# iammcy/BFLC-demo

Hardware: AMD Instinct MI355X
Metric: fl_round_wall_clock_ms (lower is better)
Workload: dtype bf16; 1 GPU; model=femnist_cnn, global_batch=4096, img=1x28x28x62cls, parallelism=fl_nodes1, clients=8, update_quota=4, aggregate_top_k=3, samples_per_client=3072, batch_size=1024, partition=dirichlet, byzantine_clients=0

## Files before the change

bflc_amd/models/__init__.py:

```python
from __future__ import annotations

from typing import Tuple

import torch

from bflc_amd.models.base import FlatModel
from bflc_amd.ops import functional as O


class LogReg(FlatModel):

    def specs(self):
        c = self.cfg
        return [("w", (c.n_features, c.n_class), "zeros"),
                ("b", (c.n_class,), "zeros")]

    def forward(self, x):
        return O.linear(x, self.p("w"), self.p("b"))


class MLP(FlatModel):

    HIDDEN = 128

    def specs(self):
        c = self.cfg
        return [("w1", (c.n_features, self.HIDDEN), "kaiming"),
                ("b1", (self.HIDDEN,), "zeros"),
                ("w2", (self.HIDDEN, c.n_class), "xavier"),
                ("b2", (c.n_class,), "zeros")]

    def forward(self, x):
        h = O.linear(x, self.p("w1"), self.p("b1"), relu=True)
        return O.linear(h, self.p("w2"), self.p("b2"))


class FemnistCNN(FlatModel):

    def specs(self):
        c = self.cfg
        return [("c1w", (32, 3, 3, 1), "kaiming"), ("c1b", (32,), "zeros"),
                ("c2w", (64, 3, 3, 32), "kaiming"), ("c2b", (64,), "zeros"),
                ("f1w", (64 * 7 * 7, 128), "kaiming"), ("f1b", (128,), "zeros"),
                ("f2w", (128, c.n_class), "xavier"), ("f2b", (c.n_class,), "zeros")]

    def forward(self, x):
        h = O.conv2d_relu_pool(x, self.p("c1w"), self.p("c1b"), 1, 1)
        h = O.conv2d_relu_pool(h, self.p("c2w"), self.p("c2b"), 1, 1)
        h = h.reshape(h.shape[0], -1)
        h = O.linear(h, self.p("f1w"), self.p("f1b"), relu=True)
        return O.linear(h, self.p("f2w"), self.p("f2b"))


def build_model(cfg, device, compute_dtype=None) -> FlatModel:
    name = cfg.model
    if getattr(cfg, "norm_groups", 0) > 0 and \
            name in ("logreg", "mlp", "femnist_cnn"):
        raise ValueError(
            f"norm_groups={cfg.norm_groups} set for model '{name}', which "
            "has no normalisation layers; it applies to resnet20/resnet50")
    if name == "logreg":
        m = LogReg(cfg, device, compute_dtype)
    elif name == "mlp":
        m = MLP(cfg, device, compute_dtype)
    elif name == "femnist_cnn":
        m = FemnistCNN(cfg, device, compute_dtype)
    elif name in ("resnet20", "resnet50"):
        from bflc_amd.models.resnet import ResNet
        m = ResNet(cfg, device, compute_dtype)
    else:
        raise ValueError(f"unknown model {name}")
    m.init_params(cfg.seed)
    return m


__all__ = ["FlatModel", "LogReg", "MLP", "FemnistCNN", "build_model"]
```

bflc_amd/ops/__init__.py:

```python
from bflc_amd.ops import functional
from bflc_amd.ops.functional import (accuracy, accuracy_t, adam_step_,
                                     axpy_, batchnorm2d, conv2d, conv2d_bn,
                                     conv2d_relu_pool,
                                     global_avgpool, add_relu,
                                     hip_available, hip_ops, linear,
                                     maxpool2d, relu, sgd_step_,
                                     sgdm_step_, grad_clip_coef_,
                                     softmax_cross_entropy, weighted_fedavg)

__all__ = [
    "functional", "linear", "conv2d", "conv2d_bn", "conv2d_relu_pool",
    "batchnorm2d", "relu",
    "add_relu", "maxpool2d", "global_avgpool", "softmax_cross_entropy",
    "accuracy", "accuracy_t", "axpy_", "sgd_step_", "adam_step_",
    "sgdm_step_", "grad_clip_coef_",
    "weighted_fedavg", "hip_ops", "hip_available",
]
```

bflc_amd/ops/functional.py:

```python
from __future__ import annotations

from typing import Optional

import torch
import torch.nn.functional as F

_hip = None
_hip_err: Optional[str] = None


def _load_hip():
    global _hip, _hip_err
    if _hip is not None or _hip_err is not None:
        return _hip
    try:
        from bflc_amd import _hip_ops
        _hip = _hip_ops
    except ImportError as e:
        _hip_err = str(e)
    return _hip


def hip_ops():
    m = _load_hip()
    if m is None:
        raise RuntimeError(
            "bflc_amd._hip_ops (gfx950 HIP kernels) is not built/importable "
            f"({_hip_err}); run `python -m bflc_amd.build`. GPU execution "
            "without the native kernels is disabled by design.")
    return m


def hip_available() -> bool:
    return _load_hip() is not None



class _LinearFn(torch.autograd.Function):

    @staticmethod
    def forward(ctx, x: torch.Tensor, w: torch.Tensor, b: torch.Tensor,
                relu: bool):
        ctx.relu = relu
        if x.is_cuda:
            y = hip_ops().linear_fwd(x, w, b, relu)
        else:
            y = torch.addmm(b, x, w)
            if relu:
                y = torch.relu(y)
        ctx.save_for_backward(x, w, y if relu else None)
        return y

    @staticmethod
    def backward(ctx, dy: torch.Tensor):
        x, w, y = ctx.saved_tensors
        dy = dy.contiguous()
        if ctx.relu:
            dy = hip_ops().relu_bwd(y, dy) if x.is_cuda \
                else dy * (y > 0).to(dy.dtype)
        want_dx = ctx.needs_input_grad[0]
        if x.is_cuda:
            dx, dw, db = hip_ops().linear_bwd(x, w, dy, want_dx)
            if not want_dx:
                dx = None
        else:
            dx = dy @ w.t() if want_dx else None
            dw = x.t() @ dy
            db = dy.sum(0)
        return dx, dw, db, None


def linear(x: torch.Tensor, w: torch.Tensor, b: torch.Tensor,
           relu: bool = False) -> torch.Tensor:
    return _LinearFn.apply(x, w, b, relu)


class _SoftmaxCEFn(torch.autograd.Function):

    @staticmethod
    def forward(ctx, logits: torch.Tensor, target: torch.Tensor):
        if logits.is_cuda:
            loss, probs = hip_ops().softmax_ce_fwd(logits, target)
        else:
            lse = torch.logsumexp(logits.float(), dim=1)
            picked = logits.float().gather(1, target.view(-1, 1)).squeeze(1)
            loss = (lse - picked).mean()
            probs = torch.softmax(logits.float(), dim=1)
        ctx.save_for_backward(probs, target)
        ctx.in_dtype = logits.dtype
        return loss

    @staticmethod
    def backward(ctx, gloss: torch.Tensor):
        probs, target = ctx.saved_tensors
        if probs.is_cuda:
            dlogits = hip_ops().softmax_ce_bwd(probs, target, gloss)
        else:
            n = probs.shape[0]
            dlogits = probs.clone()
            dlogits.scatter_add_(
                1, target.view(-1, 1),
                torch.full((n, 1), -1.0, dtype=probs.dtype))
            dlogits = dlogits * (gloss / n)
        return dlogits.to(ctx.in_dtype), None


def softmax_cross_entropy(logits: torch.Tensor,
                          target: torch.Tensor) -> torch.Tensor:
    return _SoftmaxCEFn.apply(logits, target)


class _ReluFn(torch.autograd.Function):
    @staticmethod
    def forward(ctx, x: torch.Tensor):
        if x.is_cuda:
            y = hip_ops().relu_fwd(x)
        else:
            y = torch.relu(x)
        ctx.save_for_backward(y)
        return y

    @staticmethod
    def backward(ctx, dy: torch.Tensor):
        (y,) = ctx.saved_tensors
        if y.is_cuda:
            return hip_ops().relu_bwd(y, dy.contiguous())
        return dy * (y > 0).to(dy.dtype)


def relu(x: torch.Tensor) -> torch.Tensor:
    return _ReluFn.apply(x)


class _Conv2dFn(torch.autograd.Function):

    @staticmethod
    def forward(ctx, x, w, b, stride: int, padding: int, relu: bool,
                want_col: bool):
        ctx.stride, ctx.padding = stride, padding
        ctx.has_bias = b is not None
        ctx.relu = relu
        if x.is_cuda:
            y, col = hip_ops().conv2d_fwd_col(
                x, w, b if b is not None else
                torch.zeros(w.shape[0], device=x.device, dtype=x.dtype),
                stride, padding, relu, want_col)
            ctx.save_for_backward(x, w, col, y if relu else None)
            return y
        y = F.conv2d(x.permute(0, 3, 1, 2), w.permute(0, 3, 1, 2), b,
                     stride=stride, padding=padding)
        y = y.permute(0, 2, 3, 1).contiguous()
        if relu:
            y = torch.relu(y)
        ctx.save_for_backward(x, w, None, y if relu else None)
        return y

    @staticmethod
    def backward(ctx, dy):
        x, w = ctx.saved_tensors[:2]
        dy = dy.contiguous()
        db_fused = None
        if ctx.relu:
            y = ctx.saved_tensors[3]
            if x.is_cuda and ctx.has_bias and w.shape[0] % 8 == 0:
                dy, db_fused = hip_ops().relu_bwd_colsum(y, dy)
            elif x.is_cuda:
                dy = hip_ops().relu_bwd(y, dy)
            else:
                dy = dy * (y > 0).to(dy.dtype)
        want_dx = ctx.needs_input_grad[0]
        if x.is_cuda:
            col = ctx.saved_tensors[2]
            if col.numel() == 0:
                col = None
            dx, dw, db = hip_ops().conv2d_bwd(
                x, w, dy, ctx.stride, ctx.padding, col,
                ctx.has_bias and db_fused is None, want_dx)
            if not want_dx:
                dx = None
            if db_fused is not None:
                db = db_fused
            elif not ctx.has_bias:
                db = None
        else:
            xn = x.permute(0, 3, 1, 2)
            wn = w.permute(0, 3, 1, 2)
            dyn = dy.permute(0, 3, 1, 2)
            dx = None
            if want_dx:
                dx = torch.nn.grad.conv2d_input(
                    xn.shape, wn, dyn, stride=ctx.stride,
                    padding=ctx.padding)
                dx = dx.permute(0, 2, 3, 1).contiguous()
            dw = torch.nn.grad.conv2d_weight(
                xn, wn.shape, dyn, stride=ctx.stride, padding=ctx.padding)
            dw = dw.permute(0, 2, 3, 1).contiguous()
            db = dy.sum(dim=(0, 1, 2))
        return dx, dw, (db if ctx.has_bias else None), None, None, None, \
            None


def conv2d(x, w, b=None, stride: int = 1, padding: int = 0,
           relu: bool = False) -> torch.Tensor:
    import os
    no_col = os.environ.get("BFLC_CONV_NO_COL", "1") == "1"
    want_col = (not no_col) and torch.is_grad_enabled() and \
        (x.requires_grad or w.requires_grad)
    return _Conv2dFn.apply(x, w, b, stride, padding, relu, want_col)


class _MaxPool2dFn(torch.autograd.Function):
    @staticmethod
    def forward(ctx, x, kernel: int, stride: int, want_idx: bool):
        if x.is_cuda:
            y, idx = hip_ops().maxpool2d_fwd(x, kernel, stride, want_idx)
        else:
            y, idx = F.max_pool2d(x.permute(0, 3, 1, 2), kernel, stride,
                                  return_indices=True)
            y = y.permute(0, 2, 3, 1).contiguous()
        ctx.save_for_backward(idx)
        ctx.in_shape = x.shape
        ctx.kernel, ctx.stride = kernel, stride
        return y

    @staticmethod
    def backward(ctx, dy):
        (idx,) = ctx.saved_tensors
        dy = dy.contiguous()
        if dy.is_cuda:
            dx = hip_ops().maxpool2d_bwd(dy, idx, list(ctx.in_shape),
                                         ctx.kernel, ctx.stride)
        else:
            dx = F.max_unpool2d(dy.permute(0, 3, 1, 2), idx, ctx.kernel,
                                ctx.stride,
                                output_size=ctx.in_shape[1:3])
            dx = dx.permute(0, 2, 3, 1).contiguous()
        return dx, None, None, None


def maxpool2d(x, kernel: int = 2, stride: Optional[int] = None) -> torch.Tensor:
    want_idx = torch.is_grad_enabled() and x.requires_grad
    return _MaxPool2dFn.apply(x, kernel, stride or kernel, want_idx)


class _ConvReluPoolFn(torch.autograd.Function):

    @staticmethod
    def forward(ctx, x, w, b, stride: int, padding: int,
                direct_wgrad: bool):
        ctx.stride, ctx.padding = stride, padding
        ctx.direct_wgrad = direct_wgrad
        ctx.has_bias = b is not None
        bias = b if b is not None else torch.zeros(
            w.shape[0], device=x.device, dtype=x.dtype)
        y, idx = hip_ops().conv2d_relu_pool_fwd_idx(x, w, bias, stride,
                                                    padding)
        ctx.save_for_backward(x, w, y, idx)
        return y

    @staticmethod
    def backward(ctx, dy):
        x, w, y, idx = ctx.saved_tensors
        want_dx = ctx.needs_input_grad[0]
        dx, dw, db = hip_ops().conv2d_relu_pool_bwd(
            x, w, y, idx, dy.contiguous(), ctx.stride, ctx.padding,
            ctx.has_bias, want_dx, ctx.direct_wgrad)
        return (dx if want_dx else None, dw,
                db if ctx.has_bias else None, None, None, None)


def conv2d_relu_pool(x, w, b=None, stride: int = 1,
                     padding: int = 0) -> torch.Tensor:
    import os
    if x.is_cuda and not torch.is_grad_enabled() and \
            os.environ.get("BFLC_FUSED_POOL", "1") == "1":
        bias = b if b is not None else torch.zeros(
            w.shape[0], device=x.device, dtype=x.dtype)
        return hip_ops().conv2d_relu_pool_fwd(x, w, bias, stride, padding)
    if x.is_cuda and torch.is_grad_enabled() and \
            os.environ.get("BFLC_FUSED_POOL_TRAIN", "1") != "0" and \
            hip_ops().conv2d_relu_pool_route(
                list(x.shape), list(w.shape), stride, padding) != "unfused":
        return _ConvReluPoolFn.apply(
            x, w, b, stride, padding,
            os.environ.get("BFLC_THIN_DIRECT_WGRAD", "0") == "1")
    return maxpool2d(conv2d(x, w, b, stride, padding, relu=True), 2)


class _BatchNormFn(torch.autograd.Function):

    @staticmethod
    def forward(ctx, x, gamma, beta, eps: float, relu: bool, residual):
        if x.is_cuda:
            y, mean, invstd = hip_ops().batchnorm_fwd(x, gamma, beta, eps,
                                                      relu, residual)
        else:
            xf = x.float()
            mean = xf.mean(dim=(0, 1, 2))
            var = xf.var(dim=(0, 1, 2), unbiased=False)
            invstd = (var + eps).rsqrt()
            y = (xf - mean) * invstd * gamma.float() + beta.float()
            if residual is not None:
                y = y + residual.float()
            if relu:
                y = torch.relu(y)
            y = y.to(x.dtype)
        ctx.relu = relu
        ctx.has_res = residual is not None
        if relu:
            ctx.save_for_backward(x, gamma, mean, invstd, y)
        else:
            ctx.save_for_backward(x, gamma, mean, invstd)
        return y

    @staticmethod
    def backward(ctx, dy):
        x, gamma, mean, invstd = ctx.saved_tensors[:4]
        yr = ctx.saved_tensors[4] if ctx.relu else None
        dy = dy.contiguous()
        dres = None
        if x.is_cuda:
            if ctx.has_res:
                dres = (hip_ops().add_relu_bwd(yr, dy) if yr is not None
                        else dy)
            dx, dgamma, dbeta = hip_ops().batchnorm_bwd(x, dy, mean, invstd,
                                                        gamma, yr)
        else:
            xf, dyf = x.float(), dy.float()
            if yr is not None:
                dyf = dyf * (yr.float() > 0)
            if ctx.has_res:
                dres = dyf.to(x.dtype)
            n = x.numel() / x.shape[-1]
            xhat = (xf - mean) * invstd
            sdy = dyf.sum(dim=(0, 1, 2))
            sdyx = (dyf * xhat).sum(dim=(0, 1, 2))
            dx = (gamma.float() * invstd) * (dyf - sdy / n - xhat * sdyx / n)
            dx = dx.to(x.dtype)
            dgamma = sdyx.to(x.dtype)
            dbeta = sdy.to(x.dtype)
        return dx, dgamma, dbeta, None, None, dres


class _ConvBNFn(torch.autograd.Function):

    @staticmethod
    def forward(ctx, x, w, gamma, beta, stride, padding, eps, relu,
                residual):
        h = hip_ops()
        ctx.stride, ctx.padding, ctx.relu = stride, padding, relu
        ctx.has_res = residual is not None
        yc, col, psum, psq = h.conv2d_fwd_bn(x, w, stride, padding)
        M = yc.numel() // yc.shape[-1]
        if psum.numel() > 0:
            mean, invstd = h.bn_stats_finalize(psum, psq, float(M), eps)
        else:
            mean, invstd = h.bn_stats(yc, eps)
        y = h.batchnorm_norm(yc, gamma, beta, mean, invstd, relu, residual)
        saved = [x, w, col, yc, gamma, mean, invstd]
        if relu:
            saved.append(y)
        ctx.save_for_backward(*saved)
        return y

    @staticmethod
    def backward(ctx, dy):
        h = hip_ops()
        x, w, col, yc, gamma, mean, invstd = ctx.saved_tensors[:7]
        yr = ctx.saved_tensors[7] if ctx.relu else None
        dy = dy.contiguous()
        dres = None
        if ctx.has_res:
            dres = h.add_relu_bwd(yr, dy) if yr is not None else dy
        dyc, dgamma, dbeta = h.batchnorm_bwd(yc, dy, mean, invstd, gamma,
                                             yr)
        want_dx = ctx.needs_input_grad[0]
        dx, dw, _db = h.conv2d_bwd(x, w, dyc, ctx.stride, ctx.padding,
                                   col if col.numel() > 0 else None,
                                   False, want_dx)
        if not want_dx:
            dx = None
        return (dx, dw, dgamma, dbeta, None, None, None, None, dres)


def conv2d_bn(x, w, gamma, beta, stride: int = 1, padding: int = 0,
              eps: float = 1e-5, relu: bool = True,
              residual=None) -> torch.Tensor:
    if not x.is_cuda:
        return batchnorm2d(conv2d(x, w, None, stride, padding), gamma,
                           beta, eps, relu, residual)
    return _ConvBNFn.apply(x, w, gamma, beta, stride, padding, eps, relu,
                           residual)


def batchnorm2d(x, gamma, beta, eps: float = 1e-5, relu: bool = False,
                residual=None) -> torch.Tensor:
    return _BatchNormFn.apply(x, gamma, beta, eps, relu, residual)


class _GroupNormFn(torch.autograd.Function):

    @staticmethod
    def forward(ctx, x, gamma, beta, groups: int, eps: float, relu: bool,
                residual):
        if x.is_cuda:
            y, mean, rstd = hip_ops().groupnorm_fwd(x, gamma, beta, groups,
                                                    eps, relu, residual)
        else:
            N, H, W, C = x.shape
            if groups <= 0 or C % groups:
                raise ValueError(f"groupnorm: C={C} is not divisible by "
                                 f"groups={groups}")
            xg = x.float().reshape(N, H * W, groups, C // groups)
            mean = xg.mean(dim=(1, 3))
            var = xg.var(dim=(1, 3), unbiased=False)
            rstd = (var + eps).rsqrt()
            xhat = ((xg - mean[:, None, :, None]) * rstd[:, None, :, None]) \
                .reshape(N, H, W, C)
            y = xhat * gamma.float() + beta.float()
            if residual is not None:
                y = y + residual.float()
            if relu:
                y = torch.relu(y)
            y = y.to(x.dtype)
        ctx.groups = groups
        ctx.relu = relu
        ctx.has_res = residual is not None
        if relu:
            ctx.save_for_backward(x, gamma, mean, rstd, y)
        else:
            ctx.save_for_backward(x, gamma, mean, rstd)
        return y

    @staticmethod
    def backward(ctx, dy):
        x, gamma, mean, rstd = ctx.saved_tensors[:4]
        yr = ctx.saved_tensors[4] if ctx.relu else None
        dy = dy.contiguous()
        dres = None
        G = ctx.groups
        if x.is_cuda:
            if ctx.has_res:
                dres = (hip_ops().add_relu_bwd(yr, dy) if yr is not None
                        else dy)
            dx, dgamma, dbeta = hip_ops().groupnorm_bwd(x, dy, mean, rstd,
                                                        gamma, G, yr)
        else:
            N, H, W, C = x.shape
            dyf = dy.float()
            if yr is not None:
                dyf = dyf * (yr.float() > 0)
            if ctx.has_res:
                dres = dyf.to(x.dtype)
            m = H * W * (C // G)
            xg = x.float().reshape(N, H * W, G, C // G)
            xhat = (xg - mean[:, None, :, None]) * rstd[:, None, :, None]
            d = (dyf * gamma.float()).reshape(N, H * W, G, C // G)
            sd = d.sum(dim=(1, 3), keepdim=True)
            sdx = (d * xhat).sum(dim=(1, 3), keepdim=True)
            dx = rstd[:, None, :, None] * (d - sd / m - xhat * sdx / m)
            dx = dx.reshape(N, H, W, C).to(x.dtype)
            xhat = xhat.reshape(N, H, W, C)
            dgamma = (dyf * xhat).sum(dim=(0, 1, 2)).to(x.dtype)
            dbeta = dyf.sum(dim=(0, 1, 2)).to(x.dtype)
        return dx, dgamma, dbeta, None, None, None, dres


def groupnorm2d(x, gamma, beta, groups: int, eps: float = 1e-5,
                relu: bool = False, residual=None) -> torch.Tensor:
    return _GroupNormFn.apply(x, gamma, beta, int(groups), eps, relu,
                              residual)


def conv2d_gn(x, w, gamma, beta, groups: int, stride: int = 1,
              padding: int = 0, eps: float = 1e-5, relu: bool = True,
              residual=None) -> torch.Tensor:
    return groupnorm2d(conv2d(x, w, None, stride, padding), gamma, beta,
                       groups, eps, relu, residual)


def groupnorm_route(H: int, W: int, C: int, groups: int) -> str:
    return hip_ops().groupnorm_route(H, W, C, groups)


class _GlobalAvgPoolFn(torch.autograd.Function):
    @staticmethod
    def forward(ctx, x):
        ctx.hw = (x.shape[1], x.shape[2])
        if x.is_cuda:
            return hip_ops().global_avgpool_fwd(x)
        return x.mean(dim=(1, 2))

    @staticmethod
    def backward(ctx, dy):
        h, w = ctx.hw
        dy = dy.contiguous()
        if dy.is_cuda:
            return hip_ops().global_avgpool_bwd(dy, h, w)
        return (dy / (h * w))[:, None, None, :].expand(-1, h, w, -1) \
            .contiguous()


def global_avgpool(x) -> torch.Tensor:
    return _GlobalAvgPoolFn.apply(x)


class _AddReluFn(torch.autograd.Function):

    @staticmethod
    def forward(ctx, a, b):
        if a.is_cuda:
            y = hip_ops().add_relu_fwd(a, b.contiguous())
        else:
            y = torch.relu(a + b)
        ctx.save_for_backward(y)
        return y

    @staticmethod
    def backward(ctx, dy):
        (y,) = ctx.saved_tensors
        dy = dy.contiguous()
        if y.is_cuda:
            da = hip_ops().add_relu_bwd(y, dy)
        else:
            da = dy * (y > 0).to(dy.dtype)
        return da, da


def add_relu(a, b) -> torch.Tensor:
    return _AddReluFn.apply(a, b)



def accuracy_t(logits: torch.Tensor, target: torch.Tensor) -> torch.Tensor:
    if logits.is_cuda:
        return hip_ops().accuracy_t(logits, target)
    return (logits.argmax(dim=1) == target).float().mean()


def accuracy(logits: torch.Tensor, target: torch.Tensor) -> float:
    return float(accuracy_t(logits, target))


def axpy_(y: torch.Tensor, alpha: float, x: torch.Tensor) -> torch.Tensor:
    if y.is_cuda:
        hip_ops().axpy_(y, x, float(alpha))
        return y
    return y.add_(x, alpha=alpha)


def score_load_(shadow: torch.Tensor, global_flat: torch.Tensor,
                delta: torch.Tensor, lr: float) -> None:
    if shadow.is_cuda:
        hip_ops().score_load_(shadow, global_flat, delta, float(lr))
    else:
        with torch.no_grad():
            shadow.copy_((global_flat - lr * delta).to(shadow.dtype))


def delta_extract_(out: torch.Tensor, global_flat: torch.Tensor,
                   w: torch.Tensor, lr: float) -> None:
    if out.is_cuda:
        hip_ops().delta_extract_(out, global_flat, w, float(lr))
    else:
        with torch.no_grad():
            torch.sub(global_flat, w, out=out)
            out.div_(lr)


def sgd_step_(flat_param: torch.Tensor, flat_grad: torch.Tensor,
              lr: float) -> None:
    if flat_param.is_cuda:
        hip_ops().sgd_step_(flat_param, flat_grad, float(lr))
    else:
        flat_param.add_(flat_grad, alpha=-lr)


def grad_sumsq_geom(n: int):
    return tuple(hip_ops().grad_sumsq_geom(int(n)))


def sgdm_step_geom(n: int):
    return tuple(hip_ops().sgdm_step_geom(int(n)))


def grad_clip_coef_(g: torch.Tensor, clip: float,
                    out: torch.Tensor) -> None:
    if not clip > 0:
        raise ValueError("clip must be > 0")
# ... 72 lines not shown
```

csrc/hip/bindings.cpp:

```cpp
#include <torch/extension.h>

#include <string>
#include <tuple>
#include <vector>

namespace bflc {

void axpy_(torch::Tensor y, torch::Tensor x, double alpha);
void sgd_step_(torch::Tensor p, torch::Tensor g, double lr);
void adam_step_(torch::Tensor p, torch::Tensor g, torch::Tensor m,
                torch::Tensor v, long step, double lr, double beta1,
                double beta2, double eps);
torch::Tensor weighted_fedavg(torch::Tensor deltas, torch::Tensor w);
void sgd_master_(torch::Tensor p, torch::Tensor shadow, torch::Tensor g,
                 double lr);
void adam_master_(torch::Tensor p, torch::Tensor shadow, torch::Tensor g,
                  torch::Tensor m, torch::Tensor v, long step, double lr,
                  double beta1, double beta2, double eps);
void adam_master_graph_(torch::Tensor p, torch::Tensor shadow,
                        torch::Tensor g, torch::Tensor m, torch::Tensor v,
                        torch::Tensor step, torch::Tensor bc, double lr,
                        double beta1, double beta2, double eps);
void refresh_shadow_(torch::Tensor p, torch::Tensor shadow);
void score_load_(torch::Tensor shadow, torch::Tensor global_flat,
                 torch::Tensor delta, double lr);
void delta_extract_(torch::Tensor out, torch::Tensor global_flat,
                    torch::Tensor w, double lr);
torch::Tensor relu_fwd(torch::Tensor x);
torch::Tensor relu_bwd(torch::Tensor y, torch::Tensor dy);
std::tuple<torch::Tensor, torch::Tensor> relu_bwd_colsum(
    const torch::Tensor& y, const torch::Tensor& dy);

std::tuple<long, long, long> grad_sumsq_geom_query(long n);
std::tuple<long, long, long> sgdm_step_geom_query(long n);
void grad_clip_coef_(torch::Tensor g, double clip, torch::Tensor out);
void sgdm_master_dev_(torch::Tensor p, c10::optional<torch::Tensor> shadow,
                      torch::Tensor g, torch::Tensor buf, torch::Tensor p0,
                      torch::Tensor lr_dev, torch::Tensor coef_dev,
                      double momentum, bool nesterov, double wd, double mu);

std::tuple<torch::Tensor, torch::Tensor> softmax_ce_fwd(torch::Tensor logits,
                                                        torch::Tensor target);
torch::Tensor softmax_ce_bwd(torch::Tensor probs, torch::Tensor target,
                             torch::Tensor gloss);

double accuracy(torch::Tensor logits, torch::Tensor target);
torch::Tensor accuracy_t(torch::Tensor logits, torch::Tensor target);

torch::Tensor linear_fwd(torch::Tensor x, torch::Tensor w, torch::Tensor b,
                         bool relu);
torch::Tensor gemm_raw(torch::Tensor A, torch::Tensor B, bool ta, bool tb);
using PlanRow = std::tuple<std::string, long, long, long, long>;
PlanRow gemm_plan_route(long M, long N, long K, bool ta, bool tb);
std::tuple<long, long, long, long> colsum_geom_query(long M, long N);
std::tuple<torch::Tensor, torch::Tensor, torch::Tensor> linear_bwd(
    torch::Tensor x, torch::Tensor w, torch::Tensor dy, bool want_dx);

std::tuple<torch::Tensor, torch::Tensor> conv2d_fwd_col(
    torch::Tensor x, torch::Tensor w, torch::Tensor b, long stride, long pad,
    bool relu, bool want_col);
std::tuple<torch::Tensor, torch::Tensor, torch::Tensor, torch::Tensor>
conv2d_fwd_bn(torch::Tensor x, torch::Tensor w, long stride, long pad);
std::tuple<torch::Tensor, torch::Tensor> bn_stats(torch::Tensor x,
                                                  double eps);
std::tuple<torch::Tensor, torch::Tensor> bn_stats_finalize(
    torch::Tensor psum, torch::Tensor psq, double count, double eps);
torch::Tensor batchnorm_norm(torch::Tensor x, torch::Tensor gamma,
                             torch::Tensor beta, torch::Tensor mean,
                             torch::Tensor invstd, bool relu,
                             c10::optional<torch::Tensor> residual);
torch::Tensor conv2d_fwd(torch::Tensor x, torch::Tensor w, torch::Tensor b,
                         long stride, long pad, bool relu);
std::tuple<torch::Tensor, torch::Tensor, torch::Tensor> conv2d_bwd(
    torch::Tensor x, torch::Tensor w, torch::Tensor dy, long stride,
    long pad, c10::optional<torch::Tensor> col_cache, bool want_db,
    bool want_dx);
std::tuple<torch::Tensor, torch::Tensor> maxpool2d_fwd(torch::Tensor x,
                                                       long kernel,
                                                       long stride,
                                                       bool want_idx);
torch::Tensor maxpool2d_bwd(torch::Tensor dy, torch::Tensor idx,
                            std::vector<long> in_shape, long kernel,
                            long stride);
torch::Tensor conv2d_relu_pool_fwd(torch::Tensor x, torch::Tensor w,
                                   torch::Tensor b, long stride, long pad,
                                   long max_blocks, std::string impl);
std::string conv_fwd_pool_impl(std::vector<long> x_shape,
                               std::vector<long> w_shape, long stride,
                               long pad);
long halo_conv_group_images_query(std::vector<long> x_shape,
                                  std::vector<long> w_shape, long stride,
                                  long pad);
std::string conv2d_relu_pool_route(std::vector<long> x_shape,
                                   std::vector<long> w_shape, long stride,
                                   long pad);
PlanRow conv_plan_route(const std::string& entry, std::vector<long> x_shape,
                        std::vector<long> w_shape, long stride, long pad);
std::tuple<torch::Tensor, torch::Tensor> conv2d_relu_pool_fwd_idx(
    torch::Tensor x, torch::Tensor w, torch::Tensor b, long stride,
    long pad, long max_blocks, std::string impl);
std::tuple<torch::Tensor, torch::Tensor> pool_relu_bwd_colsum(
    torch::Tensor y_pooled, torch::Tensor idx, torch::Tensor dy_pooled,
    std::vector<long> out_shape);
std::tuple<torch::Tensor, torch::Tensor> thin_conv_pool_wgrad(
    torch::Tensor x, torch::Tensor y_pooled, torch::Tensor idx,
    torch::Tensor dy_pooled, long stride, long pad);
std::tuple<torch::Tensor, torch::Tensor> thin_conv_pool_wgrad_fused(
    torch::Tensor x, torch::Tensor y_pooled, torch::Tensor idx,
    torch::Tensor dy_pooled, long stride, long pad);
std::string thin_pool_wgrad_impl(std::vector<long> x_shape,
                                 std::vector<long> w_shape, long stride,
                                 long pad, bool want_dx);
std::string conv2d_relu_pool_bwd_route(std::vector<long> x_shape,
                                       std::vector<long> w_shape,
                                       long stride, long pad, bool want_dx,
                                       bool allow_direct);
std::tuple<torch::Tensor, torch::Tensor, torch::Tensor> conv2d_relu_pool_bwd(
    torch::Tensor x, torch::Tensor w, torch::Tensor y_pooled,
    torch::Tensor idx, torch::Tensor dy_pooled, long stride, long pad,
    bool want_db, bool want_dx, bool allow_direct, std::string dgrad_impl,
    long max_blocks);
std::string pool_dgrad_impl(std::vector<long> x_shape,
                            std::vector<long> w_shape, long stride, long pad,
                            bool want_dx);
long halo_dgrad_group_images_query(std::vector<long> x_shape,
                                   std::vector<long> w_shape, long stride,
                                   long pad);
std::tuple<torch::Tensor, torch::Tensor> halo_pool_dgrad(
    torch::Tensor w, torch::Tensor y_pooled, torch::Tensor idx,
    torch::Tensor dy_pooled, long max_blocks, bool store_plane);

std::tuple<torch::Tensor, torch::Tensor, torch::Tensor> batchnorm_fwd(
    torch::Tensor x, torch::Tensor gamma, torch::Tensor beta, double eps,
    bool relu, c10::optional<torch::Tensor> residual);
std::tuple<torch::Tensor, torch::Tensor, torch::Tensor> batchnorm_bwd(
    torch::Tensor x, torch::Tensor dy, torch::Tensor mean,
    torch::Tensor invstd, torch::Tensor gamma,
    c10::optional<torch::Tensor> y_relu);
torch::Tensor global_avgpool_fwd(torch::Tensor x);
torch::Tensor global_avgpool_bwd(torch::Tensor dy, long H, long W);
torch::Tensor add_relu_fwd(torch::Tensor a, torch::Tensor b);
torch::Tensor add_relu_bwd(torch::Tensor y, torch::Tensor dy);

std::tuple<torch::Tensor, torch::Tensor, torch::Tensor> groupnorm_fwd(
    torch::Tensor x, torch::Tensor gamma, torch::Tensor beta, long groups,
    double eps, bool relu, c10::optional<torch::Tensor> residual);
std::tuple<torch::Tensor, torch::Tensor, torch::Tensor> groupnorm_bwd(
    torch::Tensor x, torch::Tensor dy, torch::Tensor mean, torch::Tensor rstd,
    torch::Tensor gamma, long groups, c10::optional<torch::Tensor> y_relu);
std::string groupnorm_route(long H, long W, long C, long groups);

}

PYBIND11_MODULE(TORCH_EXTENSION_NAME, m) {
  m.doc() = "bflc_amd hand-written gfx950 (CDNA4) HIP kernels";
  m.def("axpy_", &bflc::axpy_, "y += alpha*x (fp32, in place)");
  m.def("sgd_step_", &bflc::sgd_step_, "fused flat SGD");
  m.def("adam_step_", &bflc::adam_step_, "fused flat Adam");
  m.def("weighted_fedavg", &bflc::weighted_fedavg,
        "fixed-order weighted FedAvg reduce");
  m.def("sgd_master_", &bflc::sgd_master_,
        "fused fp32-master SGD + bf16 shadow refresh");
  m.def("adam_master_", &bflc::adam_master_);
  m.def("adam_master_graph_", &bflc::adam_master_graph_,
        "hipGraph-capturable Adam: device step counter + on-device bias "
        "corrections (tick kernel), fp32 master + bf16 shadow");
  m.def("refresh_shadow_", &bflc::refresh_shadow_, "shadow = bf16(master)");
  m.def("score_load_", &bflc::score_load_,
        "shadow = compute_dtype(global - lr*delta): one-pass scoring "
        "candidate load (replaces copy+axpy+set_flat)");
  m.def("delta_extract_", &bflc::delta_extract_,
        "out = (global - w)/lr: one-pass pseudo-gradient extraction");
  m.def("grad_sumsq_geom", &bflc::grad_sumsq_geom_query,
        "sum-of-squares geometry of an n-element gradient: (blocks, "
        "longest lane chain in elements, adds after the lane chain)",
        py::arg("n"));
  m.def("sgdm_step_geom", &bflc::sgdm_step_geom_query,
        "launch of sgdm_master_dev_ at n elements: (blocks, threads, "
        "elements per thread per grid-stride pass)",
        py::arg("n"));
  m.def("grad_clip_coef_", &bflc::grad_clip_coef_,
        "out[0] = min(1, clip / (||g||_2 + 1e-6)), 0 if the norm is not "
        "finite; out[1] = sum(g^2) when out has two elements",
        py::arg("g"), py::arg("clip"), py::arg("out"));
  m.def("sgdm_master_dev_", &bflc::sgdm_master_dev_,
        "fused SGD (momentum / nesterov / weight decay / FedProx / clip "
        "coefficient) on the fp32 master (+ bf16 shadow); lr and coef are "
        "device floats",
        py::arg("p"), py::arg("shadow"), py::arg("g"), py::arg("buf"),
        py::arg("p0"), py::arg("lr_dev"), py::arg("coef_dev"),
        py::arg("momentum"), py::arg("nesterov"), py::arg("wd"),
        py::arg("mu"));
  m.def("relu_fwd", &bflc::relu_fwd);
  m.def("relu_bwd", &bflc::relu_bwd);
  m.def("relu_bwd_colsum", &bflc::relu_bwd_colsum,
        "fused relu backward + bias-grad column sum: (dx, db)");
  m.def("softmax_ce_fwd", &bflc::softmax_ce_fwd,
        "fused softmax cross-entropy fwd (loss, probs)");
  m.def("softmax_ce_bwd", &bflc::softmax_ce_bwd);
  m.def("accuracy", &bflc::accuracy, "fused argmax-compare-reduce");
  m.def("accuracy_t", &bflc::accuracy_t,
        "accuracy as a device tensor (no host sync)");
  m.def("linear_fwd", &bflc::linear_fwd, "MFMA bf16 GEMM + bias (+relu)",
        py::arg("x"), py::arg("w"), py::arg("b"), py::arg("relu") = false);
  m.def("gemm_raw", &bflc::gemm_raw, "raw GEMM (bench/ablation)");
  m.def("gemm_plan_route", &bflc::gemm_plan_route,
        "plan gemm_raw takes: (thin | gemm8p | gemm256 | small, bm, bn, S, "
        "kslice)",
        py::arg("M"), py::arg("N"), py::arg("K"), py::arg("ta"),
        py::arg("tb"));
  m.def("conv_plan_route", &bflc::conv_plan_route,
        "plan of the implicit-GEMM conv entry fwd | fwd_pool | dgrad | "
        "wgrad: (none | gemm256 | small, bm, bn, S, kslice)",
        py::arg("entry"), py::arg("x_shape"), py::arg("w_shape"),
        py::arg("stride"), py::arg("pad"));
  m.def("colsum_geom", &bflc::colsum_geom_query,
        "colsum pass-1 geometry of an [M, N] matrix: (G, cblocks, rows, "
        "chunks)",
        py::arg("M"), py::arg("N"));
  m.def("linear_bwd", &bflc::linear_bwd,
        "(dx, dw, db) - dx empty unless want_dx", py::arg("x"),
        py::arg("w"), py::arg("dy"), py::arg("want_dx") = true);
  m.def("conv2d_fwd", &bflc::conv2d_fwd,
        "NHWC implicit-GEMM convolution (MFMA); inference entry, no col",
        py::arg("x"), py::arg("w"), py::arg("b"), py::arg("stride"),
        py::arg("pad"), py::arg("relu") = false);
  m.def("conv2d_fwd_col", &bflc::conv2d_fwd_col, "(y, col) - col for bwd",
        py::arg("x"), py::arg("w"), py::arg("b"), py::arg("stride"),
        py::arg("pad"), py::arg("relu") = false,
        py::arg("want_col") = true);
  m.def("conv2d_fwd_bn", &bflc::conv2d_fwd_bn,
        "(y, col, psum, psq) - conv with fused epilogue BN stats");
  m.def("bn_stats", &bflc::bn_stats, "(mean, invstd) of x [.., C]");
  m.def("bn_stats_finalize", &bflc::bn_stats_finalize,
        "(mean, invstd) from [chunks][C] partials");
  m.def("batchnorm_norm", &bflc::batchnorm_norm,
        py::arg("x"), py::arg("gamma"), py::arg("beta"), py::arg("mean"),
        py::arg("invstd"), py::arg("relu"),
        py::arg("residual") = py::none(),
        "normalization pass with known stats");
  m.def("conv2d_bwd", &bflc::conv2d_bwd,
        "(dx, dw, db) - db empty unless want_db, dx empty unless "
        "want_dx (first-layer convs need no input gradient)",
        py::arg("x"), py::arg("w"), py::arg("dy"), py::arg("stride"),
        py::arg("pad"), py::arg("col_cache") = py::none(),
        py::arg("want_db") = true, py::arg("want_dx") = true);
  m.def("maxpool2d_fwd", &bflc::maxpool2d_fwd, py::arg("x"),
        py::arg("kernel"), py::arg("stride"),
        py::arg("want_idx") = true);
  m.def("maxpool2d_bwd", &bflc::maxpool2d_bwd);
  m.def("conv2d_relu_pool_fwd", &bflc::conv2d_relu_pool_fwd,
        "grad-free conv + bias + ReLU + 2x2/2 maxpool, pooled in the conv "
        "epilogue where a fused route applies: [N, OH/2, OW/2, Kout]. "
        "max_blocks > 0 caps the halo kernel's grid; impl pins gemm256 | "
        "halo_mfma ('' = conv_fwd_pool_impl's answer)",
        py::arg("x"), py::arg("w"), py::arg("b"), py::arg("stride"),
        py::arg("pad"), py::arg("max_blocks") = 0, py::arg("impl") = "");
  m.def("conv_fwd_pool_impl", &bflc::conv_fwd_pool_impl,
        "what the gemm256_pool route launches: halo_mfma | gemm256",
        py::arg("x_shape"), py::arg("w_shape"), py::arg("stride"),
        py::arg("pad"));
  m.def("halo_conv_group_images", &bflc::halo_conv_group_images_query,
        "images per LDS group of the halo kernel (0: not its geometry)",
        py::arg("x_shape"), py::arg("w_shape"), py::arg("stride"),
        py::arg("pad"));
  m.def("conv2d_relu_pool_route", &bflc::conv2d_relu_pool_route,
        "route conv2d_relu_pool_fwd takes: gemm256_pool | thin_pool | "
        "unfused",
        py::arg("x_shape"), py::arg("w_shape"), py::arg("stride"),
        py::arg("pad"));
  m.def("conv2d_relu_pool_fwd_idx", &bflc::conv2d_relu_pool_fwd_idx,
        "training conv + bias + ReLU + 2x2/2 maxpool: (y_pooled, idx), "
        "same routes and options as conv2d_relu_pool_fwd",
        py::arg("x"), py::arg("w"), py::arg("b"), py::arg("stride"),
        py::arg("pad"), py::arg("max_blocks") = 0, py::arg("impl") = "");
  m.def("pool_relu_bwd_colsum", &bflc::pool_relu_bwd_colsum,
        "unpool + ReLU mask + bias grad in one pass: (dy_full_masked, db)",
        py::arg("y_pooled"), py::arg("idx"), py::arg("dy_pooled"),
        py::arg("out_shape"));
  m.def("thin_conv_pool_wgrad", &bflc::thin_conv_pool_wgrad,
        "direct first-layer (dw, db) from the pooled tensors",
        py::arg("x"), py::arg("y_pooled"), py::arg("idx"),
        py::arg("dy_pooled"), py::arg("stride"), py::arg("pad"));
  m.def("thin_conv_pool_wgrad_fused", &bflc::thin_conv_pool_wgrad_fused,
        "first-layer (dw, db) from the pooled tensors, bitwise the "
        "materialised unpool -> im2col -> split-K GEMM chain",
        py::arg("x"), py::arg("y_pooled"), py::arg("idx"),
        py::arg("dy_pooled"), py::arg("stride"), py::arg("pad"));
  m.def("thin_pool_wgrad_impl", &bflc::thin_pool_wgrad_impl,
        "what the unpool route runs for the thin first layer: "
        "fused_mfma | materialized",
        py::arg("x_shape"), py::arg("w_shape"), py::arg("stride"),
        py::arg("pad"), py::arg("want_dx"));
  m.def("conv2d_relu_pool_bwd_route", &bflc::conv2d_relu_pool_bwd_route,
        "route conv2d_relu_pool_bwd takes: thin_direct | unpool",
        py::arg("x_shape"), py::arg("w_shape"), py::arg("stride"),
        py::arg("pad"), py::arg("want_dx"), py::arg("allow_direct") = true);
  m.def("conv2d_relu_pool_bwd", &bflc::conv2d_relu_pool_bwd,
        "(dx, dw, db) of the fused conv + ReLU + pool from its saved "
        "(x, w, y_pooled, idx). dgrad_impl pins halo_mfma | implicit_gemm "
        "('' = pool_dgrad_impl's answer); max_blocks > 0 caps the halo "
        "kernel's grid",
        py::arg("x"), py::arg("w"), py::arg("y_pooled"), py::arg("idx"),
        py::arg("dy_pooled"), py::arg("stride"), py::arg("pad"),
        py::arg("want_db") = true, py::arg("want_dx") = true,
        py::arg("allow_direct") = true, py::arg("dgrad_impl") = "",
        py::arg("max_blocks") = 0);
  m.def("pool_dgrad_impl", &bflc::pool_dgrad_impl,
        "data gradient the unpool route runs: halo_mfma | implicit_gemm",
        py::arg("x_shape"), py::arg("w_shape"), py::arg("stride"),
        py::arg("pad"), py::arg("want_dx"));
  m.def("halo_dgrad_group_images", &bflc::halo_dgrad_group_images_query,
        "images per LDS group of the halo dgrad kernel (0: not its "
        "geometry)",
        py::arg("x_shape"), py::arg("w_shape"), py::arg("stride"),
        py::arg("pad"));
  m.def("halo_pool_dgrad", &bflc::halo_pool_dgrad,
        "the halo dgrad kernel on its geometry alone: (dx, masked "
        "full-resolution dy plane) from w and the pooled (y, idx, dy); "
        "store_plane = false skips the plane store (0-size plane)",
        py::arg("w"), py::arg("y_pooled"), py::arg("idx"),
        py::arg("dy_pooled"), py::arg("max_blocks") = 0,
        py::arg("store_plane") = true);
  m.def("batchnorm_fwd", &bflc::batchnorm_fwd,
        py::arg("x"), py::arg("gamma"), py::arg("beta"), py::arg("eps"),
        py::arg("relu"), py::arg("residual") = py::none(),
        "(y, mean, invstd) — batch-stats BN, optional fused relu");
  m.def("batchnorm_bwd", &bflc::batchnorm_bwd, "(dx, dgamma, dbeta)",
        py::arg("x"), py::arg("dy"), py::arg("mean"), py::arg("invstd"),
        py::arg("gamma"), py::arg("y_relu") = py::none());
  m.def("global_avgpool_fwd", &bflc::global_avgpool_fwd);
  m.def("global_avgpool_bwd", &bflc::global_avgpool_bwd);
  m.def("add_relu_fwd", &bflc::add_relu_fwd, "fused residual add + relu");
  m.def("add_relu_bwd", &bflc::add_relu_bwd);
  m.def("groupnorm_fwd", &bflc::groupnorm_fwd,
        py::arg("x"), py::arg("gamma"), py::arg("beta"), py::arg("groups"),
        py::arg("eps"), py::arg("relu"), py::arg("residual") = py::none(),
        "(y, mean [N,G], rstd [N,G]) — per-sample GroupNorm, optional "
        "fused residual add + relu");
  m.def("groupnorm_bwd", &bflc::groupnorm_bwd, "(dx, dgamma, dbeta)",
        py::arg("x"), py::arg("dy"), py::arg("mean"), py::arg("rstd"),
        py::arg("gamma"), py::arg("groups"), py::arg("y_relu") = py::none());
  m.def("groupnorm_route", &bflc::groupnorm_route,
        "route groupnorm_fwd/bwd take: slab | split (from H, W, C, groups "
        "only — never N)",
        py::arg("H"), py::arg("W"), py::arg("C"), py::arg("groups"));
}
```

csrc/hip/conv2d.hip:

```cpp

#include "common.h"
#include "gemm_api.h"

namespace bflc {

namespace {

typedef __attribute__((ext_vector_type(8))) __bf16 bf16x8_t;
typedef __attribute__((ext_vector_type(8))) unsigned short u16x8_t;
typedef __attribute__((ext_vector_type(8))) int i32x8_t;
typedef __attribute__((ext_vector_type(4))) float f32x4_t;

__global__ void im2col_nhwc_vec_kernel(const bf16* __restrict__ x,
                                       bf16* __restrict__ col, ConvShape sh,
                                       long total_g) {
  const int c8g = sh.C / 8;
  const int rs = sh.R * sh.S;
  long g = (long)blockIdx.x * blockDim.x + threadIdx.x;
  const long stride = (long)gridDim.x * blockDim.x;
  for (; g < total_g; g += stride) {
    const int c8 = (int)(g % c8g) * 8;
    const int k = (int)((g / c8g) % rs);
    const long m = g / ((long)c8g * rs);
    const int s = k % sh.S, r = k / sh.S;
// ... 654 lines not shown
    for (int t = 0; t < Q; ++t) {
      if (wq == t && my0 < nsteps) {
        if (my0 > 0) acc = accs[frag][lane];
#pragma unroll
        for (int i = 0; i < CH; ++i)
          if (my0 + i < nsteps)
            acc = __builtin_amdgcn_mfma_f32_16x16x32_bf16(
                __builtin_bit_cast(bf16x8_t, av[i]),
                __builtin_bit_cast(bf16x8_t, bv[i]), acc, 0, 0, 0);
        accs[frag][lane] = acc;
      }
      __syncthreads();
    }
  }
  if (wq != 0) return;
  acc = accs[frag][lane];

  if (l15 < 9) {
#pragma unroll
    for (int r = 0; r < 4; ++r) {
      const int row = frag * 16 + l4 * 4 + r;
      if (row >= Kout) continue;
      if (part)
        part[((long)blockIdx.x * Kout + row) * 9 + l15] = acc[r];
      else
        dw[row * 9 + l15] = f2b(acc[r] + 0.f);
    }
  }
}

inline int ew_grid(long n) {
  return (int)std::min<long>((n + 255) / 256, 16384);
}

ConvShape make_shape(const torch::Tensor& x, const torch::Tensor& w,
                     long stride, long pad) {
  ConvShape sh;
  sh.N = (int)x.size(0); sh.H = (int)x.size(1);
  sh.W = (int)x.size(2); sh.C = (int)x.size(3);
  sh.Kout = (int)w.size(0); sh.R = (int)w.size(1); sh.S = (int)w.size(2);
  sh.stride = (int)stride; sh.pad = (int)pad;
  sh.OH = (sh.H + 2 * sh.pad - sh.R) / sh.stride + 1;
  sh.OW = (sh.W + 2 * sh.pad - sh.S) / sh.stride + 1;
  TORCH_CHECK(w.size(3) == sh.C, "conv channel mismatch (NHWC x, KRSC w)");
  return sh;
}

torch::Tensor im2col(const torch::Tensor& x, const ConvShape& sh) {
  if (sh.C % 8 == 0) {
    auto col = torch::empty({sh.M(), sh.RSC()}, x.options());
    const long total_g = sh.M() * sh.R * sh.S * (sh.C / 8);
    hipLaunchKernelGGL(im2col_nhwc_vec_kernel, dim3(ew_grid(total_g)),
                       dim3(256), 0, cur_stream(),
                       (const bf16*)x.data_ptr(), (bf16*)col.data_ptr(), sh,
                       total_g);
    HIP_CHECK(hipGetLastError());
    return col;
  }
  const long rscp = (sh.RSC() + 7) / 8 * 8;
  auto col = torch::empty({sh.M(), rscp}, x.options());
  if (rscp <= 32) {
    const long total_m = sh.M();
    hipLaunchKernelGGL(im2col_nhwc_rowvec_kernel, dim3(ew_grid(total_m)),
                       dim3(256), 0, cur_stream(),
                       (const bf16*)x.data_ptr(), (bf16*)col.data_ptr(), sh,
                       rscp, total_m);
  } else {
    const long total_g = sh.M() * (rscp / 8);
    hipLaunchKernelGGL(im2col_nhwc_gran_kernel, dim3(ew_grid(total_g)),
                       dim3(256), 0, cur_stream(),
                       (const bf16*)x.data_ptr(), (bf16*)col.data_ptr(), sh,
                       rscp, total_g);
  }
  HIP_CHECK(hipGetLastError());
  return col;
}

torch::Tensor pad_w2(const torch::Tensor& w2, long kp) {
  if (kp == w2.size(1)) return w2;
  auto out = torch::zeros({w2.size(0), kp}, w2.options());
  out.slice(1, 0, w2.size(1)).copy_(w2);
  return out;
}

bool is_1x1_s1(const ConvShape& sh) {
  return sh.R == 1 && sh.S == 1 && sh.stride == 1 && sh.pad == 0;
}

int env_gate(const char* name, int dflt) {
  const char* e = getenv(name);
  return e ? atoi(e) : dflt;
}
int wgrad_implicit_max_kout() {
  static int v = env_gate("BFLC_WGRAD_IMPLICIT_MAX_KOUT", 64);
  return v;
}
int dgrad_implicit_max_c() {
  static int v = env_gate("BFLC_DGRAD_IMPLICIT_MAX_C", 128);
  return v;
}

}

std::tuple<torch::Tensor, torch::Tensor> conv2d_fwd_col(
    torch::Tensor x, torch::Tensor w, torch::Tensor b, long stride,
    long pad, bool relu, bool want_col) {
  CHECK_GPU(x); CHECK_CONTIG(x); CHECK_CONTIG(w);
  TORCH_CHECK(x.scalar_type() == at::kBFloat16, "conv: bf16 only");
  auto sh = make_shape(x, w, stride, pad);
  auto w2 = w.view({(long)sh.Kout, sh.RSC()});
  auto bc = b.contiguous();
  auto y = torch::empty({(long)sh.N, (long)sh.OH, (long)sh.OW,
                         (long)sh.Kout}, x.options());
  if (is_1x1_s1(sh)) {
    auto col = x.view({sh.M(), (long)sh.C});
    gemm_bf16_raw(col, w2, y, sh.M(), sh.Kout, sh.RSC(), false, true, &bc,
                  relu, EpStore::kPlain, 0);
    return {y, col};
  }
  if (gemm_conv_fwd_raw(x, w2, y, sh, &bc, relu))
    return {y, torch::empty({0}, x.options())};
  const long kp = (sh.RSC() + 7) / 8 * 8;
  if (!want_col && sh.RSC() <= 16 && kp <= 32) {
    auto w2p = pad_w2(w2, kp);
    if (gemm_thin_conv_raw(x, w2p, y, sh, &bc, relu))
      return {y, torch::empty({0}, x.options())};
  }
  auto col = im2col(x, sh);
  TORCH_CHECK(col.size(1) == kp);
  gemm_bf16_raw(col, pad_w2(w2, kp), y, sh.M(), sh.Kout, kp, false, true,
                &bc, relu, EpStore::kPlain, 0);
  return {y, col};
}

torch::Tensor conv2d_fwd(torch::Tensor x, torch::Tensor w, torch::Tensor b,
                         long stride, long pad, bool relu) {
  return std::get<0>(conv2d_fwd_col(x, w, b, stride, pad, relu, false));
}

std::tuple<torch::Tensor, torch::Tensor, torch::Tensor, torch::Tensor>
conv2d_fwd_bn(torch::Tensor x, torch::Tensor w, long stride, long pad) {
  CHECK_GPU(x); CHECK_CONTIG(x); CHECK_CONTIG(w);
  auto sh = make_shape(x, w, stride, pad);
  auto w2 = w.view({(long)sh.Kout, sh.RSC()});
  auto y = torch::empty({(long)sh.N, (long)sh.OH, (long)sh.OW,
                         (long)sh.Kout}, x.options());
  std::pair<torch::Tensor, torch::Tensor> stats;
  auto none = torch::empty({0}, x.options());
  if (is_1x1_s1(sh)) {
    auto col = x.view({sh.M(), (long)sh.C});
    gemm_bf16_raw(col, w2, y, sh.M(), sh.Kout, sh.RSC(), false, true,
                  nullptr, false, EpStore::kPlain, 0, &stats);
    return {y, col, stats.first.defined() ? stats.first : none,
            stats.second.defined() ? stats.second : none};
  }
  if (gemm_conv_fwd_raw(x, w2, y, sh, nullptr, false, &stats))
    return {y, none, stats.first.defined() ? stats.first : none,
            stats.second.defined() ? stats.second : none};
  auto col = im2col(x, sh);
  const long kp = col.size(1);
  gemm_bf16_raw(col, pad_w2(w2, kp), y, sh.M(), sh.Kout, kp, false, true,
                nullptr, false, EpStore::kPlain, 0, &stats);
  return {y, col, stats.first.defined() ? stats.first : none,
          stats.second.defined() ? stats.second : none};
}

namespace {

torch::Tensor conv_dgrad(const torch::Tensor& x, const torch::Tensor& w,
                         const torch::Tensor& dy2, const ConvShape& sh,
                         bool want_dx) {
  auto w2 = w.view({(long)sh.Kout, sh.RSC()});
  torch::Tensor dx;
  bool dgrad_done = !want_dx;
  if (!want_dx) {
    dx = torch::empty({0}, x.options());
  } else if (is_1x1_s1(sh)) {
    auto wT = transpose_bf16(w2);
    dx = torch::empty_like(x);
    auto dxv = dx.view({sh.M(), (long)sh.C});
    gemm_bf16_raw(dy2, wT, dxv, sh.M(), sh.RSC(), sh.Kout, false, true,
                  nullptr, false, EpStore::kPlain, 0);
    dgrad_done = true;
  } else if (sh.Kout % 8 == 0 && sh.C <= dgrad_implicit_max_c() &&
             sh.C >= 8 && sh.stride == 1) {
    auto wrot2 = w.permute({3, 1, 2, 0}).contiguous()
                     .view({(long)sh.C, (long)sh.R * sh.S * sh.Kout});
    dx = torch::empty_like(x);
    auto dxv = dx.view({(long)sh.N * sh.H * sh.W, (long)sh.C});
    dgrad_done = gemm_conv_dgrad_raw(dy2, wrot2, dxv, sh);
  }
  if (!dgrad_done) {
    auto wT = transpose_bf16(w2);
    auto dcol = torch::empty({sh.M(), sh.RSC()}, x.options());
    gemm_bf16_raw(dy2, wT, dcol, sh.M(), sh.RSC(), sh.Kout, false, true,
                  nullptr, false, EpStore::kPlain, 0);
    dx = torch::empty_like(x);
    if (sh.C % 8 == 0) {
      const long total_g = (long)sh.N * sh.H * sh.W * (sh.C / 8);
      hipLaunchKernelGGL(col2im_nhwc_vec_kernel, dim3(ew_grid(total_g)),
                         dim3(256), 0, cur_stream(),
                         (const bf16*)dcol.data_ptr(),
                         (bf16*)dx.data_ptr(), sh, total_g);
    } else {
      const long total = dx.numel();
      hipLaunchKernelGGL(col2im_nhwc_kernel, dim3(ew_grid(total)), dim3(256),
                         0, cur_stream(), (const bf16*)dcol.data_ptr(),
                         (bf16*)dx.data_ptr(), sh, total);
    }
    HIP_CHECK(hipGetLastError());
  }
  return dx;
}

torch::Tensor conv_wgrad(const torch::Tensor& x, const torch::Tensor& w,
                         const torch::Tensor& dy2, const ConvShape& sh,
                         const c10::optional<torch::Tensor>& col_cache) {
  auto w2 = w.view({(long)sh.Kout, sh.RSC()});
  auto dw = torch::empty_like(w2);
  bool wgrad_done = false;
  if (!is_1x1_s1(sh) && sh.Kout <= wgrad_implicit_max_kout() &&
      !(col_cache.has_value() && col_cache->numel() > 0))
    wgrad_done = gemm_conv_wgrad_raw(dy2, x, dw, sh);
  if (!wgrad_done) {
    auto col = (col_cache.has_value() && col_cache->numel() > 0)
                   ? *col_cache
                   : (is_1x1_s1(sh) ? x.view({sh.M(), (long)sh.C})
                                    : im2col(x, sh));
    const long kp = col.size(1);
    if (kp == sh.RSC()) {
      gemm_bf16_raw(dy2, col, dw, sh.Kout, sh.RSC(), sh.M(), true, false,
                    nullptr, false, EpStore::kPlain, 0);
    } else {
      auto dwp = torch::empty({(long)sh.Kout, kp}, dw.options());
      gemm_bf16_raw(dy2, col, dwp, sh.Kout, kp, sh.M(), true, false,
                    nullptr, false, EpStore::kPlain, 0);
      dw.copy_(dwp.slice(1, 0, sh.RSC()));
    }
  }
  return dw.view(w.sizes());
}

}

std::tuple<torch::Tensor, torch::Tensor, torch::Tensor> conv2d_bwd(
    torch::Tensor x, torch::Tensor w, torch::Tensor dy, long stride,
    long pad, c10::optional<torch::Tensor> col_cache, bool want_db,
    bool want_dx) {
  CHECK_GPU(x); CHECK_CONTIG(x); CHECK_CONTIG(w); CHECK_CONTIG(dy);
  auto sh = make_shape(x, w, stride, pad);
  auto dy2 = dy.view({sh.M(), (long)sh.Kout});
  auto dx = conv_dgrad(x, w, dy2, sh, want_dx);
  auto dw = conv_wgrad(x, w, dy2, sh, col_cache);

  auto db = want_db ? colsum_bf16(dy2)
                    : torch::empty({0}, dy.options());
  return {dx, dw, db};
}

std::tuple<torch::Tensor, torch::Tensor> maxpool2d_fwd(torch::Tensor x,
                                                       long kernel,
                                                       long stride,
                                                       bool want_idx) {
  CHECK_GPU(x); CHECK_CONTIG(x);
  ConvShape sh;
  sh.N = (int)x.size(0); sh.H = (int)x.size(1);
  sh.W = (int)x.size(2); sh.C = (int)x.size(3);
  sh.R = sh.S = (int)kernel; sh.stride = (int)stride; sh.pad = 0;
  sh.Kout = sh.C;
  sh.OH = (sh.H - sh.R) / sh.stride + 1;
  sh.OW = (sh.W - sh.S) / sh.stride + 1;
  auto y = torch::empty({(long)sh.N, (long)sh.OH, (long)sh.OW, (long)sh.C},
                        x.options());
  TORCH_CHECK(sh.R * sh.S <= 255, "maxpool window too large for u8 idx");
  const bool skip_idx = !want_idx && sh.C % 8 == 0;
  auto idx = skip_idx
                 ? torch::empty({0}, y.options().dtype(at::kByte))
                 : torch::empty_like(y, y.options().dtype(at::kByte));
  if (sh.C % 8 == 0) {
    const long total_g = sh.M() * (sh.C / 8);
    hipLaunchKernelGGL(maxpool_nhwc_vec_fwd, dim3(ew_grid(total_g)),
                       dim3(256), 0, cur_stream(),
                       (const bf16*)x.data_ptr(), (bf16*)y.data_ptr(),
                       skip_idx ? nullptr : idx.data_ptr<uint8_t>(), sh,
                       total_g);
  } else {
    const long total = y.numel();
    hipLaunchKernelGGL(maxpool_nhwc_fwd, dim3(ew_grid(total)), dim3(256), 0,
                       cur_stream(), (const bf16*)x.data_ptr(),
                       (bf16*)y.data_ptr(), idx.data_ptr<uint8_t>(), sh,
                       total);
  }
  HIP_CHECK(hipGetLastError());
  return {y, idx};
}

namespace {

enum class PoolRoute { kUnfused, kGemm256, kThin };

PoolRoute pool_route(const ConvShape& sh) {
  if (is_1x1_s1(sh)) return PoolRoute::kUnfused;
  if (gemm_conv_fwd_pool_eligible(sh)) return PoolRoute::kGemm256;
  const long kp = (sh.RSC() + 7) / 8 * 8;
  if (sh.RSC() <= 16 && gemm_thin_conv_pool_eligible(sh, kp))
    return PoolRoute::kThin;
  return PoolRoute::kUnfused;
}

ConvShape make_shape_dims(std::vector<long> xs, std::vector<long> ws,
                          long stride, long pad) {
  TORCH_CHECK(xs.size() == 4 && ws.size() == 4, "NHWC x, KRSC w");
  ConvShape sh;
  sh.N = (int)xs[0]; sh.H = (int)xs[1]; sh.W = (int)xs[2]; sh.C = (int)xs[3];
  sh.Kout = (int)ws[0]; sh.R = (int)ws[1]; sh.S = (int)ws[2];
  sh.stride = (int)stride; sh.pad = (int)pad;
  sh.OH = (sh.H + 2 * sh.pad - sh.R) / sh.stride + 1;
  sh.OW = (sh.W + 2 * sh.pad - sh.S) / sh.stride + 1;
  return sh;
}

}

PlanRow conv_plan_route(const std::string& entry, std::vector<long> x_shape,
                        std::vector<long> w_shape, long stride, long pad) {
  const ConvEntry e = entry == "fwd"        ? ConvEntry::kFwd
                      : entry == "fwd_pool" ? ConvEntry::kFwdPool
                      : entry == "dgrad"    ? ConvEntry::kDgrad
                                            : ConvEntry::kWgrad;
  TORCH_CHECK(e != ConvEntry::kWgrad || entry == "wgrad",
              "conv_plan_route: entry is fwd | fwd_pool | dgrad | wgrad");
  return plan_row(
      gemm_conv_plan(e, make_shape_dims(x_shape, w_shape, stride, pad)));
}

std::string conv2d_relu_pool_route(std::vector<long> x_shape,
                                   std::vector<long> w_shape, long stride,
                                   long pad) {
  switch (pool_route(make_shape_dims(x_shape, w_shape, stride, pad))) {
    case PoolRoute::kGemm256: return "gemm256_pool";
    case PoolRoute::kThin: return "thin_pool";
    default: return "unfused";
  }
}

namespace {

std::tuple<torch::Tensor, torch::Tensor> relu_pool_fwd_impl(
    const torch::Tensor& x, const torch::Tensor& w, const torch::Tensor& b,
    long stride, long pad, bool want_idx, long max_blocks = 0,
    const std::string& impl = "") {
  CHECK_GPU(x); CHECK_CONTIG(x); CHECK_CONTIG(w);
  TORCH_CHECK(x.scalar_type() == at::kBFloat16, "conv: bf16 only");
  auto sh = make_shape(x, w, stride, pad);
  TORCH_CHECK(impl.empty() || impl == "gemm256" || impl == "halo_mfma",
              "conv2d_relu_pool: impl is '' | gemm256 | halo_mfma");
  const HaloMode halo = impl.empty()        ? HaloMode::kAuto
                        : impl == "gemm256" ? HaloMode::kOff
                                            : HaloMode::kForce;
  TORCH_CHECK(halo != HaloMode::kForce || halo_conv_geometry_ok(sh),
              "conv2d_relu_pool: shape outside the halo kernel's geometry");
  const PoolRoute route =
      halo == HaloMode::kForce ? PoolRoute::kGemm256 : pool_route(sh);
  if (route != PoolRoute::kUnfused) {
    auto w2 = w.view({(long)sh.Kout, sh.RSC()});
    auto bc = b.contiguous();
    auto y = torch::empty({(long)sh.N, (long)sh.OH / 2, (long)sh.OW / 2,
                           (long)sh.Kout}, x.options());
    auto idx = want_idx
                   ? torch::empty_like(y, y.options().dtype(at::kByte))
                   : torch::empty({0}, y.options().dtype(at::kByte));
    uint8_t* ip = want_idx ? idx.data_ptr<uint8_t>() : nullptr;
    const bool done =
        route == PoolRoute::kGemm256
            ? gemm_conv_fwd_pool_raw(x, w2, y, sh, &bc, true, ip, halo,
                                     (int)max_blocks)
            : gemm_thin_conv_pool_raw(
                  x, pad_w2(w2, (sh.RSC() + 7) / 8 * 8), y, sh, &bc, true,
                  ip);
    TORCH_CHECK(done, "conv2d_relu_pool: route query and launcher disagree");
    return {y, idx};
  }
  auto y = conv2d_fwd(x, w, b, stride, pad, true);
  return maxpool2d_fwd(y, 2, 2, want_idx);
}

bool thin_wgrad_eligible(const ConvShape& sh) {
  return sh.R == 3 && sh.S == 3 && sh.C == 1 && sh.stride == 1 &&
         sh.OH > 0 && sh.OW > 0 && sh.OH % 2 == 0 && sh.OW % 2 == 0 &&
         sh.Kout <= 64 && sh.Kout % 8 == 0;
}

void check_pooled(const torch::Tensor& y, const torch::Tensor& idx,
                  const torch::Tensor& dy) {
  CHECK_GPU(y); CHECK_GPU(idx); CHECK_GPU(dy);
  CHECK_CONTIG(y); CHECK_CONTIG(idx); CHECK_CONTIG(dy);
  TORCH_CHECK(y.scalar_type() == at::kBFloat16 &&
              dy.scalar_type() == at::kBFloat16 &&
              idx.scalar_type() == at::kByte,
              "pooled backward: bf16 y/dy and u8 idx");
  TORCH_CHECK(y.dim() == 4 && y.sizes() == dy.sizes() &&
              y.sizes() == idx.sizes(),
              "pooled backward: y, idx, dy must share one NHWC shape");
}

bool thin_fused_wgrad_gate() {
  static const bool v = env_gate("BFLC_THIN_FUSED_WGRAD", 1) != 0;
  return v;
}

struct ThinFusedPlan {
  bool ok = false;
  long S = 1, kslice = 0;
  int tbl_pairs = 0;
  long lds = 0;
  int cshift = 0;
};

ThinFusedPlan thin_fused_plan(const ConvShape& sh) {
  ThinFusedPlan t;
  if (!thin_wgrad_eligible(sh) || sh.N <= 0) return t;
  const long Mpix = sh.M();
  const long kp = (sh.RSC() + 7) / 8 * 8;
  const GemmPlan p = gemm_dense_plan(sh.Kout, kp, Mpix, true, false);
  const long lim = 1L << 31;
  if (p.path != GemmPath::kSmall || kp != 16 || Mpix * sh.Kout >= lim ||
      (long)sh.N * sh.H * sh.W >= lim || (long)sh.N * (sh.OH + 2) >= lim)
    return t;
  t.S = p.S;
  t.kslice = p.kslice;
  int rows_max = 0;
  for (long s = 0; s < p.S; ++s) {
    int P0, rows;
    thin_wgrad_window(sh, s * p.kslice,
                      std::min(Mpix, (s + 1) * p.kslice), &P0, &rows);
    rows_max = std::max(rows_max, rows);
  }
  const long xelems = (long)(rows_max + 2) * (sh.OW + 2) + 4;
  const long pairs = (p.kslice / 32 + 1) * 16;
  t.tbl_pairs = (int)pairs;
  t.lds = pairs * 8 + (xelems + 1) / 2 * 4;
  while (t.cshift < 6 && (1 << t.cshift) < sh.OW + 2) ++t.cshift;
  t.ok = t.lds <= kThinFusedMaxLds && xelems <= 32768;
  return t;
}

torch::Tensor pool_relu_bwd_db(const torch::Tensor& y_pooled,
                               const torch::Tensor& idx,
                               const torch::Tensor& dy_pooled,
                               const ConvShape& sh) {
  const long Mpix = sh.M();
  const long N = sh.Kout;
  TORCH_CHECK(Mpix * N < (1L << 31), "pool_relu_bwd_db: 32-bit indices");
  auto db = torch::empty({N}, dy_pooled.options());
  const ColsumGeom g = colsum_geom(Mpix, N);
  auto cpart = torch::empty({g.chunks, N},
                            dy_pooled.options().dtype(at::kFloat));
  hipLaunchKernelGGL(pool_relu_bwd_colsum_part_kernel<false>,
                     dim3(g.cblocks, g.chunks), dim3(256), 0, cur_stream(),
                     (const bf16*)y_pooled.data_ptr(),
                     idx.data_ptr<uint8_t>(),
                     (const bf16*)dy_pooled.data_ptr(), (bf16*)nullptr, Mpix,
                     N, sh.OH, sh.OW, g.G, g.rows, cpart.data_ptr<float>());
  HIP_CHECK(hipGetLastError());
  colsum_finalize(cpart, db);
  return db;
}

}

torch::Tensor conv2d_relu_pool_fwd(torch::Tensor x, torch::Tensor w,
                                   torch::Tensor b, long stride, long pad,
                                   long max_blocks, std::string impl) {
  return std::get<0>(
      relu_pool_fwd_impl(x, w, b, stride, pad, false, max_blocks, impl));
}

std::string conv_fwd_pool_impl(std::vector<long> x_shape,
                               std::vector<long> w_shape, long stride,
                               long pad) {
  const auto sh = make_shape_dims(x_shape, w_shape, stride, pad);
  return pool_route(sh) == PoolRoute::kGemm256 && halo_conv_gate(sh)
             ? "halo_mfma"
             : "gemm256";
}

long halo_conv_group_images_query(std::vector<long> x_shape,
                                  std::vector<long> w_shape, long stride,
                                  long pad) {
  return halo_conv_group_images(
      make_shape_dims(x_shape, w_shape, stride, pad));
}

std::tuple<torch::Tensor, torch::Tensor> conv2d_relu_pool_fwd_idx(
    torch::Tensor x, torch::Tensor w, torch::Tensor b, long stride,
    long pad, long max_blocks, std::string impl) {
  return relu_pool_fwd_impl(x, w, b, stride, pad, true, max_blocks, impl);
}

std::tuple<torch::Tensor, torch::Tensor> pool_relu_bwd_colsum(
    torch::Tensor y_pooled, torch::Tensor idx, torch::Tensor dy_pooled,
    std::vector<long> out_shape) {
  check_pooled(y_pooled, idx, dy_pooled);
  const long n = y_pooled.size(0), PH = y_pooled.size(1),
             PW = y_pooled.size(2), N = y_pooled.size(3);
  TORCH_CHECK(N % 8 == 0, "pool_relu_bwd_colsum: C % 8 required");
  TORCH_CHECK(out_shape.size() == 4 && out_shape[0] == n &&
              out_shape[1] == 2 * PH && out_shape[2] == 2 * PW &&
              out_shape[3] == N,
              "pool_relu_bwd_colsum: out_shape must be [N, 2*PH, 2*PW, C]");
  const long M = n * PH * PW * 4;
  auto dx = torch::empty({n, 2 * PH, 2 * PW, N}, dy_pooled.options());
  auto db = torch::empty({N}, dy_pooled.options());
  const ColsumGeom g = colsum_geom(M, N);
  auto part = torch::empty({g.chunks, N},
                           dy_pooled.options().dtype(at::kFloat));
  if (M > 0) {
    hipLaunchKernelGGL(pool_relu_bwd_colsum_part_kernel<true>,
                       dim3(g.cblocks, g.chunks), dim3(256), 0, cur_stream(),
                       (const bf16*)y_pooled.data_ptr(),
                       idx.data_ptr<uint8_t>(),
                       (const bf16*)dy_pooled.data_ptr(),
                       (bf16*)dx.data_ptr(), M, N, (int)(2 * PH),
                       (int)(2 * PW), g.G, g.rows, part.data_ptr<float>());
    HIP_CHECK(hipGetLastError());
  }
  colsum_finalize(part, db);
  return {dx, db};
}

std::tuple<torch::Tensor, torch::Tensor> thin_conv_pool_wgrad(
    torch::Tensor x, torch::Tensor y_pooled, torch::Tensor idx,
    torch::Tensor dy_pooled, long stride, long pad) {
  CHECK_GPU(x); CHECK_CONTIG(x);
  TORCH_CHECK(x.scalar_type() == at::kBFloat16 && x.dim() == 4,
              "thin_conv_pool_wgrad: bf16 NHWC x");
  check_pooled(y_pooled, idx, dy_pooled);
  const auto sh = make_shape_dims(
      x.sizes().vec(), {y_pooled.size(3), 3, 3, x.size(3)}, stride, pad);
  TORCH_CHECK(thin_wgrad_eligible(sh),
              "thin_conv_pool_wgrad: 3x3, C == 1, stride 1, even OH/OW, "
              "Kout % 8 == 0 and Kout <= 64 only");
  TORCH_CHECK(y_pooled.size(0) == sh.N && y_pooled.size(1) == sh.OH / 2 &&
              y_pooled.size(2) == sh.OW / 2,
              "thin_conv_pool_wgrad: pooled shape does not match x");
  const long MP = sh.M() / 4;
  const int N = sh.Kout;
  const int G = N / 8, PL = 256 / G;
  const long rows = std::max<long>(PL, (MP + 511) / 512);
  const int chunks = (int)std::max<long>(1, (MP + rows - 1) / rows);
  auto part = torch::empty({(long)chunks, (long)N, (long)kWgradAcc},
                           x.options().dtype(at::kFloat));
  auto dw = torch::empty({(long)N, 3, 3, 1}, x.options());
  auto db = torch::empty({(long)N}, x.options());
  hipLaunchKernelGGL(thin_conv_pool_wgrad_part_kernel, dim3(chunks),
                     dim3(256), 0, cur_stream(), (const bf16*)x.data_ptr(),
                     (const bf16*)y_pooled.data_ptr(),
                     idx.data_ptr<uint8_t>(),
                     (const bf16*)dy_pooled.data_ptr(), sh, MP, G, rows,
                     part.data_ptr<float>());
  HIP_CHECK(hipGetLastError());
  hipLaunchKernelGGL(thin_conv_pool_wgrad_final_kernel,
                     dim3(ceil_div((long)N * kWgradAcc, 4)), dim3(256), 0,
                     cur_stream(), part.data_ptr<float>(), chunks, N,
                     (bf16*)dw.data_ptr(), (bf16*)db.data_ptr());
  HIP_CHECK(hipGetLastError());
  return {dw, db};
}

std::tuple<torch::Tensor, torch::Tensor> thin_conv_pool_wgrad_fused(
    torch::Tensor x, torch::Tensor y_pooled, torch::Tensor idx,
    torch::Tensor dy_pooled, long stride, long pad) {
  CHECK_GPU(x); CHECK_CONTIG(x);
  TORCH_CHECK(x.scalar_type() == at::kBFloat16 && x.dim() == 4,
              "thin_conv_pool_wgrad_fused: bf16 NHWC x");
  check_pooled(y_pooled, idx, dy_pooled);
  const auto sh = make_shape_dims(
      x.sizes().vec(), {y_pooled.size(3), 3, 3, x.size(3)}, stride, pad);
  const ThinFusedPlan t = thin_fused_plan(sh);
  TORCH_CHECK(t.ok,
              "thin_conv_pool_wgrad_fused: 3x3, C == 1, stride 1, even "
              "OH/OW, Kout % 8 == 0 and Kout <= 64, on the small-tile "
              "split-K plan, only");
  TORCH_CHECK(y_pooled.size(0) == sh.N && y_pooled.size(1) == sh.OH / 2 &&
              y_pooled.size(2) == sh.OW / 2,
              "thin_conv_pool_wgrad_fused: pooled shape does not match x");
  const long Mpix = sh.M();
  const int N = sh.Kout;
  auto dw = torch::empty({(long)N, 3, 3, 1}, x.options());
  torch::Tensor db;

  torch::Tensor part;
  if (t.S > 1)
    part = torch::empty({t.S, (long)N, 9}, x.options().dtype(at::kFloat));
  const int frags = (N + 15) / 16;
  auto* kern = frags <= 2 ? thin_pool_wgrad_mfma_kernel<4>
                          : thin_pool_wgrad_mfma_kernel<2>;
  hipLaunchKernelGGL(kern, dim3((unsigned)t.S),
                     dim3(frags * (frags <= 2 ? 4 : 2) * 64), (size_t)t.lds,
                     cur_stream(), (const unsigned short*)x.data_ptr(),
                     (const unsigned short*)y_pooled.data_ptr(),
                     idx.data_ptr<uint8_t>(),
                     (const unsigned short*)dy_pooled.data_ptr(), sh, Mpix,
                     t.kslice, t.cshift, t.tbl_pairs,
                     t.S > 1 ? part.data_ptr<float>() : nullptr,
                     (bf16*)dw.data_ptr());
  HIP_CHECK(hipGetLastError());
  if (t.S > 1) {
    auto dw2 = dw.view({(long)N, 9});
    splitk_reduce_plain(part, dw2);
  }

  db = pool_relu_bwd_db(y_pooled, idx, dy_pooled, sh);
  return {dw, db};
}

std::string thin_pool_wgrad_impl(std::vector<long> x_shape,
                                 std::vector<long> w_shape, long stride,
                                 long pad, bool want_dx) {
  const auto sh = make_shape_dims(x_shape, w_shape, stride, pad);
  return !want_dx && thin_fused_wgrad_gate() && thin_fused_plan(sh).ok
             ? "fused_mfma"
             : "materialized";
}

std::string conv2d_relu_pool_bwd_route(std::vector<long> x_shape,
                                       std::vector<long> w_shape,
                                       long stride, long pad, bool want_dx,
                                       bool allow_direct) {
  const auto sh = make_shape_dims(x_shape, w_shape, stride, pad);
  return allow_direct && !want_dx && thin_wgrad_eligible(sh) ? "thin_direct"
                                                             : "unpool";
}

namespace {

std::tuple<torch::Tensor, torch::Tensor> halo_pool_dgrad_impl(
    const torch::Tensor& x_like, const torch::Tensor& w,
    const torch::Tensor& y_pooled, const torch::Tensor& idx,
    const torch::Tensor& dy_pooled, const ConvShape& sh, long max_blocks,
    bool store_plane = true) {
  auto dyf = store_plane
                 ? torch::empty({(long)sh.N, (long)sh.OH, (long)sh.OW,
                                 (long)sh.Kout}, dy_pooled.options())
                 : torch::empty({0}, dy_pooled.options());
  auto dx = torch::empty({(long)sh.N, (long)sh.H, (long)sh.W, (long)sh.C},
                         x_like.options());
  halo_pool_dgrad_launch(w, y_pooled, idx, dy_pooled,
                         store_plane ? &dyf : nullptr, dx, sh,
                         (int)max_blocks);
  return {dx, dyf};
}

}

std::string pool_dgrad_impl(std::vector<long> x_shape,
                            std::vector<long> w_shape, long stride, long pad,
                            bool want_dx) {
  const auto sh = make_shape_dims(x_shape, w_shape, stride, pad);
  return want_dx && halo_dgrad_gate(sh) ? "halo_mfma" : "implicit_gemm";
}

long halo_dgrad_group_images_query(std::vector<long> x_shape,
                                   std::vector<long> w_shape, long stride,
                                   long pad) {
  return halo_dgrad_group_images(
      make_shape_dims(x_shape, w_shape, stride, pad));
}

std::tuple<torch::Tensor, torch::Tensor> halo_pool_dgrad(
    torch::Tensor w, torch::Tensor y_pooled, torch::Tensor idx,
    torch::Tensor dy_pooled, long max_blocks, bool store_plane) {
  CHECK_GPU(w); CHECK_CONTIG(w);
  TORCH_CHECK(w.scalar_type() == at::kBFloat16 && w.dim() == 4,
              "halo_pool_dgrad: bf16 KRSC w");
  check_pooled(y_pooled, idx, dy_pooled);
  const auto sh = make_shape_dims(
      {y_pooled.size(0), 2 * y_pooled.size(1), 2 * y_pooled.size(2),
       w.size(3)},
      w.sizes().vec(), 1, 1);
  TORCH_CHECK(y_pooled.size(3) == sh.Kout && halo_dgrad_geometry_ok(sh),
              "halo_pool_dgrad: shape outside the halo kernel's geometry");
  return halo_pool_dgrad_impl(dy_pooled, w, y_pooled, idx, dy_pooled, sh,
                              max_blocks, store_plane);
}

std::tuple<torch::Tensor, torch::Tensor, torch::Tensor> conv2d_relu_pool_bwd(
    torch::Tensor x, torch::Tensor w, torch::Tensor y_pooled,
    torch::Tensor idx, torch::Tensor dy_pooled, long stride, long pad,
    bool want_db, bool want_dx, bool allow_direct, std::string dgrad_impl,
    long max_blocks) {
  CHECK_GPU(x); CHECK_CONTIG(x); CHECK_CONTIG(w);
  const auto sh = make_shape(x, w, stride, pad);
  TORCH_CHECK(sh.OH % 2 == 0 && sh.OW % 2 == 0 &&
              y_pooled.dim() == 4 && y_pooled.size(0) == sh.N &&
              y_pooled.size(1) == sh.OH / 2 &&
              y_pooled.size(2) == sh.OW / 2 && y_pooled.size(3) == sh.Kout,
              "conv2d_relu_pool_bwd: pooled shape does not match the conv");
  TORCH_CHECK(dgrad_impl.empty() || dgrad_impl == "halo_mfma" ||
                  dgrad_impl == "implicit_gemm",
              "conv2d_relu_pool_bwd: dgrad_impl is '' | halo_mfma | "
              "implicit_gemm");
  const bool force_halo = dgrad_impl == "halo_mfma";
  TORCH_CHECK(!force_halo || (want_dx && halo_dgrad_geometry_ok(sh) &&
                              sh.M() * sh.Kout < (1L << 31)),
              "conv2d_relu_pool_bwd: shape outside the halo dgrad kernel's "
              "geometry");
  auto none = torch::empty({0}, x.options());
  if (allow_direct && !want_dx && thin_wgrad_eligible(sh)) {
    auto [dw, db] = thin_conv_pool_wgrad(x, y_pooled, idx, dy_pooled,
                                         stride, pad);
    return {none, dw.view(w.sizes()), want_db ? db : none};
  }
  if (!want_dx && thin_fused_wgrad_gate() && thin_fused_plan(sh).ok) {
    auto [dw, db] = thin_conv_pool_wgrad_fused(x, y_pooled, idx, dy_pooled,
                                               stride, pad);
    return {none, dw.view(w.sizes()), want_db ? db : none};
  }
  if (force_halo ||
      (dgrad_impl.empty() && want_dx && halo_dgrad_gate(sh))) {
    check_pooled(y_pooled, idx, dy_pooled);
    auto db = want_db ? pool_relu_bwd_db(y_pooled, idx, dy_pooled, sh) : none;
    auto [dx, dyf] = halo_pool_dgrad_impl(x, w, y_pooled, idx, dy_pooled, sh,
                                          max_blocks);
    auto dy2 = dyf.view({sh.M(), (long)sh.Kout});
    auto dw = conv_wgrad(x, w, dy2, sh, c10::nullopt);
    return {dx, dw, db};
  }
  auto [dyf, db] = pool_relu_bwd_colsum(
      y_pooled, idx, dy_pooled,
      {(long)sh.N, (long)sh.OH, (long)sh.OW, (long)sh.Kout});
  auto [dx, dw, db_unused] =
      conv2d_bwd(x, w, dyf, stride, pad, c10::nullopt, false, want_dx);
  (void)db_unused;
  return {dx, dw, want_db ? db : none};
}

torch::Tensor maxpool2d_bwd(torch::Tensor dy, torch::Tensor idx,
                            std::vector<long> in_shape, long kernel,
                            long stride) {
  CHECK_GPU(dy); CHECK_CONTIG(dy); CHECK_CONTIG(idx);
  TORCH_CHECK(idx.numel() == dy.numel(),
              "maxpool2d_bwd: argmax mask missing/size-mismatched (the "
              "forward ran with want_idx=false?)");
  ConvShape sh;
  sh.N = (int)in_shape[0]; sh.H = (int)in_shape[1];
  sh.W = (int)in_shape[2]; sh.C = (int)in_shape[3];
  sh.R = sh.S = (int)kernel; sh.stride = (int)stride; sh.pad = 0;
  sh.Kout = sh.C;
  sh.OH = (int)dy.size(1); sh.OW = (int)dy.size(2);
  auto dx = torch::empty({(long)sh.N, (long)sh.H, (long)sh.W, (long)sh.C},
                         dy.options());
  if (sh.C % 8 == 0) {
    const long total_g = (long)sh.N * sh.H * sh.W * (sh.C / 8);
    hipLaunchKernelGGL(maxpool_nhwc_vec_bwd, dim3(ew_grid(total_g)),
                       dim3(256), 0, cur_stream(),
                       (const bf16*)dy.data_ptr(), idx.data_ptr<uint8_t>(),
                       (bf16*)dx.data_ptr(), sh, total_g);
  } else {
    const long total = dx.numel();
    hipLaunchKernelGGL(maxpool_nhwc_bwd, dim3(ew_grid(total)), dim3(256), 0,
                       cur_stream(), (const bf16*)dy.data_ptr(),
                       idx.data_ptr<uint8_t>(), (bf16*)dx.data_ptr(), sh,
                       total);
  }
  HIP_CHECK(hipGetLastError());
  return dx;
}

}
```

csrc/hip/gemm_api.h:

```cpp
#pragma once

#include <torch/extension.h>

#include <string>
#include <tuple>

#include "gemm_plan.h"

namespace bflc {

#if defined(__HIPCC__) || defined(__HIP__)
#define BFLC_HD __host__ __device__
#else
#define BFLC_HD
#endif

struct ConvShape {
  int N, C, H, W, Kout, R, S, stride, pad, OH, OW;
  BFLC_HD long M() const { return (long)N * OH * OW; }
  BFLC_HD long RSC() const { return (long)R * S * C; }
};

enum class EpStore : int {
  kPlain = 0,
  kConvNCHW = 1,
};

void gemm_bf16_raw(const torch::Tensor& A, const torch::Tensor& B,
                   torch::Tensor& C, long M, long N, long K, bool ta, bool tb,
                   const torch::Tensor* bias, bool relu, EpStore store,
                   long ohw,
                   std::pair<torch::Tensor, torch::Tensor>* bn_stats
                   = nullptr);

using PlanRow = std::tuple<std::string, long, long, long, long>;
inline PlanRow plan_row(const GemmPlan& p) {
  return {gemm_path_name(p.path), p.bm, p.bn, p.S, p.kslice};
}
PlanRow gemm_plan_route(long M, long N, long K, bool ta, bool tb);
GemmPlan gemm_dense_plan(long M, long N, long K, bool ta, bool tb);
void splitk_reduce_plain(const torch::Tensor& part, torch::Tensor& out);

enum class ConvEntry { kFwd, kFwdPool, kDgrad, kWgrad };
GemmPlan gemm_conv_plan(ConvEntry e, const ConvShape& sh);

bool gemm_thin_conv_raw(const torch::Tensor& x, const torch::Tensor& w2p,
                        torch::Tensor& y, const ConvShape& sh,
                        const torch::Tensor* bias, bool relu);

bool gemm_conv_fwd_raw(const torch::Tensor& x, const torch::Tensor& w2,
                       torch::Tensor& y, const ConvShape& sh,
                       const torch::Tensor* bias, bool relu,
                       std::pair<torch::Tensor, torch::Tensor>* bn_stats
                       = nullptr);

bool gemm_conv_fwd_pool_eligible(const ConvShape& sh);
enum class HaloMode { kAuto, kOff, kForce };
bool gemm_conv_fwd_pool_raw(const torch::Tensor& x, const torch::Tensor& w2,
                            torch::Tensor& y, const ConvShape& sh,
                            const torch::Tensor* bias, bool relu,
                            uint8_t* idx = nullptr,
                            HaloMode halo = HaloMode::kAuto,
                            int max_blocks = 0);

bool halo_conv_geometry_ok(const ConvShape& sh);
int halo_conv_group_images(const ConvShape& sh);
bool halo_conv_gate(const ConvShape& sh);
void halo_conv_fwd_pool_launch(const torch::Tensor& x,
                               const torch::Tensor& w2, torch::Tensor& y,
                               const ConvShape& sh, const torch::Tensor* bias,
                               bool relu, uint8_t* idx, int max_blocks);
bool halo_dgrad_geometry_ok(const ConvShape& sh);
int halo_dgrad_group_images(const ConvShape& sh);
bool halo_dgrad_gate(const ConvShape& sh);
void halo_pool_dgrad_launch(const torch::Tensor& w,
                            const torch::Tensor& y_pooled,
                            const torch::Tensor& idx,
                            const torch::Tensor& dy_pooled,
                            torch::Tensor* dyf, torch::Tensor& dx,
                            const ConvShape& sh, int max_blocks);
bool gemm_thin_conv_pool_eligible(const ConvShape& sh, long KT);
bool gemm_thin_conv_pool_raw(const torch::Tensor& x,
                             const torch::Tensor& w2p, torch::Tensor& y,
                             const ConvShape& sh, const torch::Tensor* bias,
                             bool relu, uint8_t* idx = nullptr);

bool gemm_conv_dgrad_raw(const torch::Tensor& dy, const torch::Tensor& wrot2,
                         torch::Tensor& dx, const ConvShape& sh);

bool gemm_conv_wgrad_raw(const torch::Tensor& dy2, const torch::Tensor& x,
                         torch::Tensor& dw, const ConvShape& sh);

torch::Tensor colsum_bf16(const torch::Tensor& X);
void colsum_finalize(const torch::Tensor& part, torch::Tensor& out);
std::tuple<torch::Tensor, torch::Tensor> relu_bwd_colsum(
    const torch::Tensor& y, const torch::Tensor& dy);

torch::Tensor transpose_bf16(const torch::Tensor& X);

}
```

csrc/hip/gemm_bf16.hip:

```cpp

#include "common.h"
#include "gemm_api.h"

namespace bflc {

namespace {

typedef __attribute__((ext_vector_type(8))) __bf16 bf16x8_t;
typedef __attribute__((ext_vector_type(8))) unsigned short u16x8_t;
typedef __attribute__((ext_vector_type(2))) unsigned short u16x2_t;
typedef __attribute__((ext_vector_type(4))) float f32x4_t;

constexpr int BK = 32;
constexpr int BKP = BK + 8;

template <int BM, int BN, int WR, int WC, bool TA, bool TB,
          int CMODE = 0>
__launch_bounds__(WR * WC * 64)
__global__ void gemm_kernel(const bf16* __restrict__ A,
                            const bf16* __restrict__ B,
                            bf16* __restrict__ C, float* __restrict__ Cpart,
                            const bf16* __restrict__ bias, long M, long N,
                            long K, long kslice, int relu, int store_mode,
                            long ohw, int vecA, int vecB, ConvShape csh,
                            float* __restrict__ bn_psum = nullptr,
                            float* __restrict__ bn_psq = nullptr) {
  constexpr int THREADS = WR * WC * 64;
  constexpr int FM = BM / WR / 16;
  constexpr int FN = BN / WC / 16;

  __shared__ bf16 As[BM][BKP];
  __shared__ bf16 Bs[BN][BKP];
  auto swz = [](int row, int k) { return k ^ (row & 24); };

  const int ntn = (int)((N + BN - 1) / BN);
  const int ntm = (int)((M + BM - 1) / BM);
  const int nwg = ntm * ntn;
  int bid = blockIdx.x;
  {
    const int nxcd = 8;
    const int q = nwg / nxcd, r = nwg % nxcd;
    const int xcd = bid % nxcd, idx = bid / nxcd;
    bid = (xcd < r ? xcd * (q + 1) : r * (q + 1) + (xcd - r) * q) + idx;
  }
  const long tile_m = (long)(bid / ntn) * BM;
  const long tile_n = (long)(bid % ntn) * BN;

  const long k_begin = (long)blockIdx.y * kslice;
  const long k_end = min(K, k_begin + kslice);

  const int tid = threadIdx.x;
  const int wave = tid / 64, lane = tid % 64;
  const int wm0 = (wave / WC) * (BM / WR);
  const int wn0 = (wave % WC) * (BN / WC);
  const int l15 = lane & 15, l4 = lane >> 4;

  f32x4_t acc[FM][FN] = {};

  constexpr int AGI =
      (CMODE == 1 || CMODE == 2)
          ? ((BM * BK / 8) + THREADS - 1) / THREADS : 1;
  long cv_nbase[AGI];
  int cv_i0[AGI], cv_j0[AGI];
  bool cv_mok[AGI];
  int st_c8[AGI], st_rr[AGI], st_ss[AGI];
  if (CMODE == 1 || CMODE == 2) {
    constexpr int GROUPS = (BM * BK) / 8;
#pragma unroll
    for (int i = 0; i < AGI; ++i) {
      const int g = tid + i * THREADS;
      const int m = g / (BK / 8);
      const int k8 = (g % (BK / 8)) * 8;
      const long gm = tile_m + m;
      cv_mok[i] = g < GROUPS && gm < M;
      const long gmc = cv_mok[i] ? gm : 0;
      if (CMODE == 1) {
        const int ow = (int)(gmc % csh.OW);
        const int oh = (int)((gmc / csh.OW) % csh.OH);
        const int nn = (int)(gmc / ((long)csh.OW * csh.OH));
        cv_i0[i] = oh * csh.stride - csh.pad;
        cv_j0[i] = ow * csh.stride - csh.pad;
        cv_nbase[i] = (long)nn * csh.H;
      } else {
        const int iw = (int)(gmc % csh.W);
        const int ih = (int)((gmc / csh.W) % csh.H);
        const int nn = (int)(gmc / ((long)csh.W * csh.H));
        cv_i0[i] = ih + csh.pad;
        cv_j0[i] = iw + csh.pad;
        cv_nbase[i] = (long)nn * csh.OH;
      }
      const int inner = CMODE == 1 ? csh.C : csh.Kout;
      const long gk0 = k_begin + k8;
      const int rs = (int)(gk0 / inner);
      st_c8[i] = (int)(gk0 - (long)rs * inner);
      st_rr[i] = rs / csh.S;
      st_ss[i] = rs - st_rr[i] * csh.S;
    }
  }

  constexpr int BGI =
      CMODE == 3 ? ((BN * BK / 8) + THREADS - 1) / THREADS
      : (CMODE == 4 ? ((BN * BK / 16) + THREADS - 1) / THREADS : 1);
  int cv3_rr[BGI], cv3_ss[BGI], cv3_c8[BGI];
  int st3_ow[BGI], st3_oh[BGI];
  long st3_nb[BGI];
  if (CMODE == 3 || CMODE == 4) {
#pragma unroll
    for (int i = 0; i < BGI; ++i) {
      const int g = tid + i * THREADS;
      const int n8 = (g % (BN / 8)) * 8;
      const long gn = tile_n + n8;
      const long gnc = gn + 8 <= N ? gn : 0;
      const int rs = (int)(gnc / csh.C);
      cv3_c8[i] = (int)(gnc - (long)rs * csh.C);
      cv3_rr[i] = rs / csh.S;
      cv3_ss[i] = rs - cv3_rr[i] * csh.S;
      const int k = (CMODE == 4 ? 2 : 1) * (g / (BN / 8));
      const long gm0 = k_begin + k;
      st3_ow[i] = (int)(gm0 % csh.OW);
      st3_oh[i] = (int)((gm0 / csh.OW) % csh.OH);
      st3_nb[i] = (long)(gm0 / ((long)csh.OW * csh.OH)) * csh.H;
    }
  }

  const bf16 zero = f2b(0.f);
  for (long k0 = k_begin; k0 < k_end; k0 += BK) {
    if (CMODE == 1 || CMODE == 2) {
      constexpr int GROUPS = (BM * BK) / 8;
#pragma unroll
      for (int i = 0; i < AGI; ++i) {
        const int g = tid + i * THREADS;
        if (GROUPS % THREADS != 0 && g >= GROUPS) break;
        const int m = g / (BK / 8), k8 = (g % (BK / 8)) * 8;
        const long gk = k0 + k8;
        bool ok = cv_mok[i] && gk < k_end;
        long src = 0;
        if (ok && CMODE == 1) {
          const int ih = cv_i0[i] + st_rr[i];
          const int iw = cv_j0[i] + st_ss[i];
          ok = ih >= 0 && ih < csh.H && iw >= 0 && iw < csh.W;
          src = ((cv_nbase[i] + ih) * csh.W + iw) * csh.C + st_c8[i];
        } else if (ok) {
          const int oh_num = cv_i0[i] - st_rr[i];
          const int ow_num = cv_j0[i] - st_ss[i];
          const int oh = oh_num / csh.stride;
          const int ow = ow_num / csh.stride;
          ok = oh_num >= 0 && ow_num >= 0 &&
               oh_num % csh.stride == 0 && ow_num % csh.stride == 0 &&
               oh < csh.OH && ow < csh.OW;
          src = ((cv_nbase[i] + oh) * csh.OW + ow) * csh.Kout + st_c8[i];
        }
        if (ok) {
          *reinterpret_cast<bf16x8_t*>(&As[m][swz(m, k8)]) =
              *reinterpret_cast<const bf16x8_t*>(&A[src]);
        } else {
          u16x8_t z = {};
          *reinterpret_cast<bf16x8_t*>(&As[m][swz(m, k8)]) =
              *reinterpret_cast<const bf16x8_t*>(&z);
        }
        {
          const int inner = CMODE == 1 ? csh.C : csh.Kout;
          int c8n = st_c8[i] + BK;
          while (c8n >= inner) {
            c8n -= inner;
            if (++st_ss[i] == csh.S) { st_ss[i] = 0; ++st_rr[i]; }
          }
          st_c8[i] = c8n;
        }
      }
    } else if (vecA) {
      constexpr int GROUPS = (BM * BK) / 8;
#pragma unroll
      for (int i = 0; i < (GROUPS + THREADS - 1) / THREADS; ++i) {
        const int g = tid + i * THREADS;
        if (GROUPS % THREADS != 0 && g >= GROUPS) break;
        if (!TA) {
          const int m = g / (BK / 8), k8 = (g % (BK / 8)) * 8;
          const long gm = tile_m + m, gk = k0 + k8;
          if (gm < M && gk + 8 <= k_end) {
            *reinterpret_cast<bf16x8_t*>(&As[m][swz(m, k8)]) =
                *reinterpret_cast<const bf16x8_t*>(&A[gm * K + gk]);
          } else {
#pragma unroll
            for (int j = 0; j < 8; ++j)
              As[m][swz(m, k8) + j] = (gm < M && gk + j < k_end)
                                  ? A[gm * K + gk + j] : zero;
          }
        } else {
          const int k = g / (BM / 8), m8 = (g % (BM / 8)) * 8;
          const long gm = tile_m + m8, gk = k0 + k;
          if (gk < k_end && gm + 8 <= M) {
            const u16x8_t v =
                *reinterpret_cast<const u16x8_t*>(&A[gk * M + gm]);
#pragma unroll
            for (int j = 0; j < 8; ++j)
              *reinterpret_cast<unsigned short*>(
                  &As[m8 + j][swz(m8 + j, k)]) = v[j];
          } else {
#pragma unroll
            for (int j = 0; j < 8; ++j)
              As[m8 + j][swz(m8 + j, k)] =
                  (gk < k_end && gm + j < M) ? A[gk * M + gm + j] : zero;
          }
        }
      }
    } else {
#pragma unroll
      for (int i = 0; i < (BM * BK) / THREADS; ++i) {
        int idx = tid + i * THREADS;
        int m = idx / BK, k = idx % BK;
        long gm = tile_m + m, gk = k0 + k;
        As[m][swz(m, k)] = (gm < M && gk < k_end)
                       ? (TA ? A[gk * M + gm] : A[gm * K + gk]) : zero;
      }
    }
    if (CMODE == 4) {
      constexpr int GROUPS = (BN * BK) / 16;
#pragma unroll
      for (int i = 0; i < BGI; ++i) {
        const int g = tid + i * THREADS;
        if (GROUPS % THREADS != 0 && g >= GROUPS) break;
        const int k2 = g / (BN / 8), n8 = (g % (BN / 8)) * 8;
        const int k = 2 * k2;
        const long gn = tile_n + n8;
        const long gm0 = k0 + k;
        const bool okn = gn + 8 <= N;
        u16x8_t v0 = {}, v1 = {};
        if (okn && gm0 < k_end) {
          const int ih = st3_oh[i] * csh.stride - csh.pad + cv3_rr[i];
          const int iw = st3_ow[i] * csh.stride - csh.pad + cv3_ss[i];
          if (ih >= 0 && ih < csh.H && iw >= 0 && iw < csh.W)
            v0 = *reinterpret_cast<const u16x8_t*>(
                &B[((st3_nb[i] + ih) * csh.W + iw) * csh.C + cv3_c8[i]]);
        }
        if (okn && gm0 + 1 < k_end) {
          int ow1 = st3_ow[i] + 1, oh1 = st3_oh[i];
          long nb1 = st3_nb[i];
          if (ow1 == csh.OW) {
            ow1 = 0;
            if (++oh1 == csh.OH) { oh1 = 0; nb1 += csh.H; }
          }
          const int ih = oh1 * csh.stride - csh.pad + cv3_rr[i];
          const int iw = ow1 * csh.stride - csh.pad + cv3_ss[i];
          if (ih >= 0 && ih < csh.H && iw >= 0 && iw < csh.W)
            v1 = *reinterpret_cast<const u16x8_t*>(
                &B[((nb1 + ih) * csh.W + iw) * csh.C + cv3_c8[i]]);
        }
#pragma unroll
        for (int j = 0; j < 8; ++j) {
          u16x2_t w2v;
          w2v[0] = v0[j];
          w2v[1] = v1[j];
          *reinterpret_cast<u16x2_t*>(
              &Bs[n8 + j][swz(n8 + j, k)]) = w2v;
        }
        {
          int ow = st3_ow[i] + BK;
          while (ow >= csh.OW) {
            ow -= csh.OW;
            if (++st3_oh[i] == csh.OH) { st3_oh[i] = 0; st3_nb[i] += csh.H; }
          }
          st3_ow[i] = ow;
        }
      }
    } else if (CMODE == 3) {
      constexpr int GROUPS = (BN * BK) / 8;
#pragma unroll
      for (int i = 0; i < (GROUPS + THREADS - 1) / THREADS; ++i) {
        const int g = tid + i * THREADS;
        if (GROUPS % THREADS != 0 && g >= GROUPS) break;
        const int k = g / (BN / 8), n8 = (g % (BN / 8)) * 8;
        const long gn = tile_n + n8;
        const long gm = k0 + k;
        bool ok = gm < k_end && gn + 8 <= N;
        u16x8_t v = {};
        if (ok) {
          const int ih = st3_oh[i] * csh.stride - csh.pad + cv3_rr[i];
          const int iw = st3_ow[i] * csh.stride - csh.pad + cv3_ss[i];
          if (ih >= 0 && ih < csh.H && iw >= 0 && iw < csh.W)
            v = *reinterpret_cast<const u16x8_t*>(
                &B[((st3_nb[i] + ih) * csh.W + iw) * csh.C + cv3_c8[i]]);
        }
#pragma unroll
        for (int j = 0; j < 8; ++j)
          *reinterpret_cast<unsigned short*>(
              &Bs[n8 + j][swz(n8 + j, k)]) = v[j];
        {
          int ow = st3_ow[i] + BK;
          while (ow >= csh.OW) {
            ow -= csh.OW;
            if (++st3_oh[i] == csh.OH) { st3_oh[i] = 0; st3_nb[i] += csh.H; }
          }
          st3_ow[i] = ow;
        }
      }
    } else if (vecB) {
      constexpr int GROUPS = (BN * BK) / 8;
#pragma unroll
      for (int i = 0; i < (GROUPS + THREADS - 1) / THREADS; ++i) {
        const int g = tid + i * THREADS;
        if (GROUPS % THREADS != 0 && g >= GROUPS) break;
        if (TB) {
          const int n = g / (BK / 8), k8 = (g % (BK / 8)) * 8;
          const long gn = tile_n + n, gk = k0 + k8;
          if (gn < N && gk + 8 <= k_end) {
// ... 843 lines not shown
      }
      if (bias) v += b2f(bias[col]);
      if (relu) v = fmaxf(v, 0.f);
      const float f = b2f(f2b(v));
      if (f > best) { best = f; bi = r; }
    }
    C[o] = f2b(best);
    if (idx) idx[o] = (uint8_t)bi;
  }
}

void launch_splitk_reduce_pool(const float* part, long S, long M, long N,
                               bf16* c, const bf16* bias, int relu,
                               uint8_t* idx) {
  const long totalp = M * N / 4;
  const int blocks = (int)std::min<long>((totalp + 255) / 256, 16384);
  hipLaunchKernelGGL(splitk_reduce_pool_kernel, dim3(blocks), dim3(256), 0,
                     cur_stream(), part, (int)S, M, N, c, bias, relu,
                     splitk_reduce_is_vec(M, N) ? 1 : 0, idx);
  HIP_CHECK(hipGetLastError());
}

void launch_splitk_reduce(const float* part, long S, long M, long N,
                          bf16* c, const bf16* bias, int relu,
                          EpStore store, long ohw) {
  const long total = M * N;
  if (store == EpStore::kPlain && splitk_reduce_is_vec(M, N)) {
    const long total4 = total / 4;
    const int blocks = (int)std::min<long>((total4 + 255) / 256, 16384);
    hipLaunchKernelGGL(splitk_reduce_vec_kernel, dim3(blocks), dim3(256),
                       0, cur_stream(), part, (int)S, M, N, c, bias, relu);
  } else {
    const int blocks = (int)std::min<long>((total + 31) / 32, 16384);
    hipLaunchKernelGGL(splitk_reduce_kernel, dim3(blocks), dim3(256), 0,
                       cur_stream(), part, (int)S, M, N, c, bias, relu,
                       (int)store, ohw);
  }
  HIP_CHECK(hipGetLastError());
}

__global__ void colsum_part_vec_kernel(const bf16* __restrict__ X, long M,
                                       long N, int G, long chunk_rows,
                                       float* __restrict__ part) {
  const int gi = threadIdx.x % G, rl = threadIdx.x / G;
  const int RL = (int)blockDim.x / G;
  const long c8 = ((long)blockIdx.x * G + gi) * 8;
  const long r0 = (long)blockIdx.y * chunk_rows;
  const long r1 = min(M, r0 + chunk_rows);
  float sj[8] = {};
  if (c8 < N)
    for (long m = r0 + rl; m < r1; m += RL) {
      const bf16x8_t v = *reinterpret_cast<const bf16x8_t*>(&X[m * N + c8]);
#pragma unroll
      for (int j = 0; j < 8; ++j) sj[j] += b2f(v[j]);
    }
  __shared__ float rs[256][8];
#pragma unroll
  for (int j = 0; j < 8; ++j) rs[threadIdx.x][j] = sj[j];
  __syncthreads();
  for (int h = RL >> 1; h > 0; h >>= 1) {
    if (rl < h) {
#pragma unroll
      for (int j = 0; j < 8; ++j)
        rs[rl * G + gi][j] += rs[(rl + h) * G + gi][j];
    }
    __syncthreads();
  }
  if (rl == 0 && c8 < N) {
#pragma unroll
    for (int j = 0; j < 8; ++j)
      part[(long)blockIdx.y * N + c8 + j] = rs[gi][j];
  }
}

__global__ void relu_bwd_colsum_part_vec_kernel(
    const bf16* __restrict__ y, const bf16* __restrict__ dy,
    bf16* __restrict__ dx, long M, long N, int G, long chunk_rows,
    float* __restrict__ part) {
  const int gi = threadIdx.x % G, rl = threadIdx.x / G;
  const int RL = (int)blockDim.x / G;
  const long c8 = ((long)blockIdx.x * G + gi) * 8;
  const long r0 = (long)blockIdx.y * chunk_rows;
  const long r1 = min(M, r0 + chunk_rows);
  float sj[8] = {};
  if (c8 < N)
    for (long m = r0 + rl; m < r1; m += RL) {
      const bf16x8_t yv =
          *reinterpret_cast<const bf16x8_t*>(&y[m * N + c8]);
      bf16x8_t gv = *reinterpret_cast<const bf16x8_t*>(&dy[m * N + c8]);
#pragma unroll
      for (int j = 0; j < 8; ++j) {
        if (!(b2f(yv[j]) > 0.f)) gv[j] = f2b(0.f);
        sj[j] += b2f(gv[j]);
      }
      *reinterpret_cast<bf16x8_t*>(&dx[m * N + c8]) = gv;
    }
  __shared__ float rs[256][8];
#pragma unroll
  for (int j = 0; j < 8; ++j) rs[threadIdx.x][j] = sj[j];
  __syncthreads();
  for (int h = RL >> 1; h > 0; h >>= 1) {
    if (rl < h) {
#pragma unroll
      for (int j = 0; j < 8; ++j)
        rs[rl * G + gi][j] += rs[(rl + h) * G + gi][j];
    }
    __syncthreads();
  }
  if (rl == 0 && c8 < N) {
#pragma unroll
    for (int j = 0; j < 8; ++j)
      part[(long)blockIdx.y * N + c8 + j] = rs[gi][j];
  }
}

__global__ void colsum_part_kernel(const bf16* __restrict__ X, long M, long N,
                                   long chunk_rows,
                                   float* __restrict__ part) {
  const long col = (long)blockIdx.x * 32 + (threadIdx.x & 31);
  const int rlane = threadIdx.x >> 5;
  const int chunk = blockIdx.y;
  const long r0 = (long)chunk * chunk_rows;
  const long r1 = min(M, r0 + chunk_rows);
  float acc = 0.f;
  if (col < N)
    for (long m = r0 + rlane; m < r1; m += 8) acc += b2f(X[m * N + col]);
  __shared__ float red[8][33];
  red[rlane][threadIdx.x & 31] = acc;
  __syncthreads();
  if (rlane == 0 && col < N) {
    float t = 0.f;
#pragma unroll
    for (int r = 0; r < 8; ++r) t += red[r][threadIdx.x & 31];
    part[(long)chunk * N + col] = t;
  }
}

__global__ void colsum_final_vec_kernel(const float* __restrict__ part,
                                        int chunks, long N, int G,
                                        bf16* __restrict__ out) {
  const int gi = threadIdx.x % G, kl = threadIdx.x / G;
  const int KL = (int)blockDim.x / G;
  const long c4 = ((long)blockIdx.x * G + gi) * 4;
  float sj[4] = {};
  if (c4 < N)
    for (int k = kl; k < chunks; k += KL) {
      const float4 a =
          *reinterpret_cast<const float4*>(&part[(long)k * N + c4]);
      sj[0] += a.x; sj[1] += a.y; sj[2] += a.z; sj[3] += a.w;
    }
  __shared__ float rs[256][4];
#pragma unroll
  for (int j = 0; j < 4; ++j) rs[threadIdx.x][j] = sj[j];
  __syncthreads();
  for (int h = KL >> 1; h > 0; h >>= 1) {
    if (kl < h) {
#pragma unroll
      for (int j = 0; j < 4; ++j)
        rs[kl * G + gi][j] += rs[(kl + h) * G + gi][j];
    }
    __syncthreads();
  }
  if (kl == 0 && c4 < N) {
#pragma unroll
    for (int j = 0; j < 4; ++j) out[c4 + j] = f2b(rs[gi][j]);
  }
}

__global__ void colsum_final_kernel(const float* __restrict__ part,
                                    int chunks, long N,
                                    bf16* __restrict__ out) {
  const int clane = threadIdx.x >> 5;
  const int elane = threadIdx.x & 31;
  const long col = (long)blockIdx.x * 32 + elane;
  float acc = 0.f;
  if (col < N)
    for (int c = clane; c < chunks; c += 8) acc += part[(long)c * N + col];
  __shared__ float red[8][33];
  red[clane][elane] = acc;
  __syncthreads();
  if (clane == 0 && col < N) {
    float v = 0.f;
#pragma unroll
    for (int r = 0; r < 8; ++r) v += red[r][elane];
    out[col] = f2b(v);
  }
}

typedef __attribute__((ext_vector_type(8))) float f32x8v_t;
typedef __attribute__((ext_vector_type(2))) float f32x2v_t;
typedef uint8_t u8x8_t __attribute__((ext_vector_type(8)));

template <int KT>
__global__ __launch_bounds__(256) void gemm_thin_kernel(
    const bf16* __restrict__ A, const bf16* __restrict__ B,
    bf16* __restrict__ C, const bf16* __restrict__ bias, long M, int N,
    int relu) {
  __shared__ float Bl[32 * 64];
  __shared__ float bl[64];
  for (int i = threadIdx.x; i < N * KT; i += blockDim.x)
    Bl[(i % KT) * 64 + i / KT] = b2f(B[i]);
  for (int i = threadIdx.x; i < N; i += blockDim.x)
    bl[i] = bias ? b2f(bias[i]) : 0.f;
  __syncthreads();
  long m = (long)blockIdx.x * blockDim.x + threadIdx.x;
  const long stride = (long)gridDim.x * blockDim.x;
  for (; m < M; m += stride) {
    f32x2v_t a2[KT];
    const bf16* arow = &A[m * KT];
#pragma unroll
    for (int k8 = 0; k8 < KT; k8 += 8) {
      const bf16x8_t v = *reinterpret_cast<const bf16x8_t*>(&arow[k8]);
#pragma unroll
      for (int j = 0; j < 8; ++j) {
        const float f = b2f(v[j]);
        a2[k8 + j] = f32x2v_t{f, f};
      }
    }
    for (int n8 = 0; n8 < N; n8 += 8) {
      f32x8v_t acc = *reinterpret_cast<const f32x8v_t*>(&bl[n8]);
      f32x2v_t* acc2 = reinterpret_cast<f32x2v_t*>(&acc);
#pragma unroll
      for (int k = 0; k < KT; ++k) {
        const f32x8v_t bv =
            *reinterpret_cast<const f32x8v_t*>(&Bl[k * 64 + n8]);
        const f32x2v_t* bv2 = reinterpret_cast<const f32x2v_t*>(&bv);
#pragma unroll
        for (int p = 0; p < 4; ++p) acc2[p] += bv2[p] * a2[k];
      }
      bf16x8_t out;
#pragma unroll
      for (int j = 0; j < 8; ++j) {
        float v = acc[j];
        if (relu && v < 0.f) v = 0.f;
        out[j] = f2b(v);
      }
      *reinterpret_cast<bf16x8_t*>(&C[m * N + n8]) = out;
    }
  }
}

template <int KT>
__global__ __launch_bounds__(256) void gemm_thin_conv_kernel(
    const bf16* __restrict__ X, const bf16* __restrict__ B,
    bf16* __restrict__ C, const bf16* __restrict__ bias, ConvShape sh,
    long M, int N, int relu) {
  __shared__ float Bl[32 * 64];
  __shared__ float bl[64];
  for (int i = threadIdx.x; i < N * KT; i += blockDim.x)
    Bl[(i % KT) * 64 + i / KT] = b2f(B[i]);
  for (int i = threadIdx.x; i < N; i += blockDim.x)
    bl[i] = bias ? b2f(bias[i]) : 0.f;
  __syncthreads();
  const int OW = sh.OW, OHW = sh.OH * sh.OW;
  long m = (long)blockIdx.x * blockDim.x + threadIdx.x;
  const long stride = (long)gridDim.x * blockDim.x;
  for (; m < M; m += stride) {
    const int n = (int)(m / OHW);
    const int rem = (int)(m % OHW);
    const int oh = rem / OW, ow = rem % OW;
    const int ih0 = oh * sh.stride - sh.pad;
    const int iw0 = ow * sh.stride - sh.pad;
    f32x2v_t a2[KT];
#pragma unroll
    for (int t = 0; t < KT; ++t) a2[t] = f32x2v_t{0.f, 0.f};
    int t = 0;
    for (int r = 0; r < sh.R; ++r) {
      const int ih = ih0 + r;
      const bool okh = ih >= 0 && ih < sh.H;
      for (int s = 0; s < sh.S; ++s) {
        const int iw = iw0 + s;
        const bool ok = okh && iw >= 0 && iw < sh.W;
        const long base =
            (((long)n * sh.H + ih) * sh.W + iw) * sh.C;
        for (int c = 0; c < sh.C; ++c, ++t) {
          const float f = ok ? b2f(X[base + c]) : 0.f;
          a2[t] = f32x2v_t{f, f};
        }
      }
    }
    for (int n8 = 0; n8 < N; n8 += 8) {
      f32x8v_t acc = *reinterpret_cast<const f32x8v_t*>(&bl[n8]);
      f32x2v_t* acc2 = reinterpret_cast<f32x2v_t*>(&acc);
#pragma unroll
      for (int k = 0; k < KT; ++k) {
        const f32x8v_t bv =
            *reinterpret_cast<const f32x8v_t*>(&Bl[k * 64 + n8]);
        const f32x2v_t* bv2 = reinterpret_cast<const f32x2v_t*>(&bv);
#pragma unroll
        for (int p = 0; p < 4; ++p) acc2[p] += bv2[p] * a2[k];
      }
      bf16x8_t out;
#pragma unroll
      for (int j = 0; j < 8; ++j) {
        float v = acc[j];
        if (relu && v < 0.f) v = 0.f;
        out[j] = f2b(v);
      }
      *reinterpret_cast<bf16x8_t*>(&C[m * N + n8]) = out;
    }
  }
}

template <int KT, bool IDX>
__global__ __launch_bounds__(256) void gemm_thin_conv_pool_kernel(
    const bf16* __restrict__ X, const bf16* __restrict__ B,
    bf16* __restrict__ C, uint8_t* __restrict__ idx,
    const bf16* __restrict__ bias, ConvShape sh, long MP, int N, int relu) {
  __shared__ float Bl[32 * 64];
  __shared__ float bl[64];
  for (int i = threadIdx.x; i < N * KT; i += blockDim.x)
    Bl[(i % KT) * 64 + i / KT] = b2f(B[i]);
  for (int i = threadIdx.x; i < N; i += blockDim.x)
    bl[i] = bias ? b2f(bias[i]) : 0.f;
  __syncthreads();
  const int PW = sh.OW >> 1, PHW = (sh.OH >> 1) * PW;
  long mp = (long)blockIdx.x * blockDim.x + threadIdx.x;
  const long stride = (long)gridDim.x * blockDim.x;
  for (; mp < MP; mp += stride) {
    const int n = (int)(mp / PHW);
    const int rem = (int)(mp % PHW);
    const int ih0 = (rem / PW) * 2 - sh.pad;
    const int iw0 = (rem % PW) * 2 - sh.pad;
    f32x2v_t pd[4][4];
#pragma unroll
    for (int r = 0; r < 4; ++r) {
      const int ih = ih0 + r;
      const bool okh = ih >= 0 && ih < sh.H;
#pragma unroll
      for (int s = 0; s < 4; ++s) {
        const int iw = iw0 + s;
        const bool ok = okh && iw >= 0 && iw < sh.W;
        const float f =
            ok ? b2f(X[((long)n * sh.H + ih) * sh.W + iw]) : 0.f;
        pd[r][s] = f32x2v_t{f, f};
      }
    }
    const f32x2v_t zero2 = {0.f, 0.f};
    for (int n8 = 0; n8 < N; n8 += 8) {
      f32x8v_t acc[4];
#pragma unroll
      for (int q = 0; q < 4; ++q)
        acc[q] = *reinterpret_cast<const f32x8v_t*>(&bl[n8]);
#pragma unroll
      for (int k = 0; k < KT; ++k) {
        const f32x8v_t bv =
            *reinterpret_cast<const f32x8v_t*>(&Bl[k * 64 + n8]);
        const f32x2v_t* bv2 = reinterpret_cast<const f32x2v_t*>(&bv);
#pragma unroll
        for (int q = 0; q < 4; ++q) {
          const f32x2v_t a =
              k < 9 ? pd[(q >> 1) + k / 3][(q & 1) + k % 3] : zero2;
          f32x2v_t* acc2 = reinterpret_cast<f32x2v_t*>(&acc[q]);
#pragma unroll
          for (int p = 0; p < 4; ++p) acc2[p] += bv2[p] * a;
        }
      }
      float best[8];
      int bi[8];
#pragma unroll
      for (int j = 0; j < 8; ++j) { best[j] = -INFINITY; bi[j] = 0; }
#pragma unroll
      for (int q = 0; q < 4; ++q) {
#pragma unroll
        for (int j = 0; j < 8; ++j) {
          float v = acc[q][j];
          if (relu && v < 0.f) v = 0.f;
          const float f = b2f(f2b(v));
          if (f > best[j]) {
            best[j] = f;
            if (IDX) bi[j] = q;
          }
        }
      }
      bf16x8_t out;
#pragma unroll
      for (int j = 0; j < 8; ++j) out[j] = f2b(best[j]);
      *reinterpret_cast<bf16x8_t*>(&C[mp * N + n8]) = out;
      if (IDX) {
        u8x8_t oidx;
#pragma unroll
        for (int j = 0; j < 8; ++j) oidx[j] = (uint8_t)bi[j];
        *reinterpret_cast<u8x8_t*>(&idx[mp * N + n8]) = oidx;
      }
    }
  }
}

static_assert(BK == kSmallBK && BK2 == kDbufBK,
              "gemm_plan.h slices K in the kernels' steps");

template <int V>
using ic = std::integral_constant<int, V>;

template <class F>
void dispatch_bool(bool b, F&& f) {
  if (b) f(std::true_type{});
  else f(std::false_type{});
}

template <class F>
void dispatch_thin(long K, F&& f) {
  switch (K) {
    case 8: f(ic<8>{}); break;
    case 16: f(ic<16>{}); break;
    case 24: f(ic<24>{}); break;
    default: f(ic<32>{}); break;
  }
}

template <class F>
void dispatch_small(const GemmPlan& p, F&& f) {
  switch (p.bm * 1000 + p.bn) {
    case 128128: f(ic<128>{}, ic<128>{}, ic<2>{}, ic<2>{}); break;
    case 128064: f(ic<128>{}, ic<64>{}, ic<2>{}, ic<2>{}); break;
    case 128032: f(ic<128>{}, ic<32>{}, ic<2>{}, ic<2>{}); break;
    case  64128: f(ic<64>{}, ic<128>{}, ic<2>{}, ic<2>{}); break;
    case  64064: f(ic<64>{}, ic<64>{}, ic<2>{}, ic<2>{}); break;
    case  64032: f(ic<64>{}, ic<32>{}, ic<2>{}, ic<2>{}); break;
    case  32128: f(ic<32>{}, ic<128>{}, ic<1>{}, ic<4>{}); break;
    case  32064: f(ic<32>{}, ic<64>{}, ic<1>{}, ic<4>{}); break;
    case  32032: f(ic<32>{}, ic<32>{}, ic<2>{}, ic<1>{}); break;
    default: TORCH_CHECK(false, "no tile config for ", p.bm, "x", p.bn);
  }
}

template <class F>
void dispatch_dbuf(const GemmPlan& p, F&& f) {
  switch (p.bm * 1000 + p.bn) {
    case 256256: f(ic<256>{}, ic<256>{}); break;
    case 256128: f(ic<256>{}, ic<128>{}); break;
    case 256064: f(ic<256>{}, ic<64>{}); break;
    case 128256: f(ic<128>{}, ic<256>{}); break;
    case 128128: f(ic<128>{}, ic<128>{}); break;
    case 128064: f(ic<128>{}, ic<64>{}); break;
    case  64256: f(ic<64>{}, ic<256>{}); break;
    case  64128: f(ic<64>{}, ic<128>{}); break;
    case  64064: f(ic<64>{}, ic<64>{}); break;
    default: TORCH_CHECK(false, "no dbuf tile config for ", p.bm, "x", p.bn);
  }
}

struct SplitKPart {
  torch::Tensor buf;
  float* ptr = nullptr;
};

SplitKPart alloc_splitk_part(const GemmPlan& p, long M, long N,
                             const torch::Tensor& like) {
  SplitKPart part;
  if (p.S > 1) {
    part.buf = torch::empty({p.S, M, N}, like.options().dtype(at::kFloat));
    part.ptr = part.buf.data_ptr<float>();
  }
  return part;
}

struct BnStatsPtrs {
  float* sum = nullptr;
  float* sq = nullptr;
};

BnStatsPtrs alloc_bn_stats(std::pair<torch::Tensor, torch::Tensor>* out,
                           bool want, const GemmPlan& p, long M, long N,
                           const torch::Tensor& like) {
  BnStatsPtrs st;
  if (out && want) {
    const long chunks = (M + p.bm - 1) / p.bm;
    const auto opt = like.options().dtype(at::kFloat);
    out->first = torch::empty({chunks, N}, opt);
    out->second = torch::empty({chunks, N}, opt);
    st.sum = out->first.data_ptr<float>();
    st.sq = out->second.data_ptr<float>();
  }
  return st;
}

int wgrad_small_gate() {
  static const int v = [] {
    const char* e = getenv("BFLC_WGRAD_SMALL");
    return e ? atoi(e) : 0;
  }();
  return v;
}

bool narrow_dbuf_gate() {
  static const bool v = [] {
    const char* e = getenv("BFLC_NARROW_DBUF");
    return e && e[0] == '1';
  }();
  return v;
}

struct GemmDims { long M, N, K; };

GemmDims conv_gemm_dims(ConvEntry e, const ConvShape& sh) {
  if (e == ConvEntry::kWgrad) return {sh.Kout, sh.RSC(), sh.M()};
  if (e == ConvEntry::kDgrad)
    return {(long)sh.N * sh.H * sh.W, sh.C, (long)sh.R * sh.S * sh.Kout};
  return {sh.M(), sh.Kout, sh.RSC()};
}

void launch_colsum_final(const float* part, int chunks, long N, bf16* out) {
  if (N % 4 == 0) {
    const int G4 = colsum_final_g4(N);
    hipLaunchKernelGGL(colsum_final_vec_kernel,
                       dim3(ceil_div(N / 4, (long)G4)), dim3(256), 0,
                       cur_stream(), part, chunks, N, G4, out);
  } else {
    hipLaunchKernelGGL(colsum_final_kernel, dim3(ceil_div(N, 32)),
                       dim3(256), 0, cur_stream(), part, chunks, N, out);
  }
  HIP_CHECK(hipGetLastError());
}

}

bool gemm_thin_conv_pool_eligible(const ConvShape& sh, long KT) {
  return sh.R == 3 && sh.S == 3 && sh.C == 1 && sh.stride == 1 &&
         sh.OH % 2 == 0 && sh.OW % 2 == 0 && KT == 16 &&
         sh.Kout <= 64 && sh.Kout % 8 == 0 && sh.M() >= 65536;
}

bool gemm_thin_conv_pool_raw(const torch::Tensor& x,
                             const torch::Tensor& w2p, torch::Tensor& y,
                             const ConvShape& sh, const torch::Tensor* bias,
                             bool relu, uint8_t* idx) {
  const long KT = w2p.size(1);
  if (!gemm_thin_conv_pool_eligible(sh, KT)) return false;
  const long MP = sh.M() / 4;
  const bf16* bs = bias ? (const bf16*)bias->data_ptr() : nullptr;
  const int blocks = (int)std::min<long>((MP + 255) / 256, 16384);
  dispatch_bool(idx != nullptr, [&](auto want_idx) {
    hipLaunchKernelGGL(
        (gemm_thin_conv_pool_kernel<16, decltype(want_idx)::value>),
        dim3(blocks), dim3(256), 0, cur_stream(), (const bf16*)x.data_ptr(),
        (const bf16*)w2p.data_ptr(), (bf16*)y.data_ptr(), idx, bs, sh, MP,
        (int)sh.Kout, relu ? 1 : 0);
  });
  HIP_CHECK(hipGetLastError());
  return true;
}

bool gemm_thin_conv_raw(const torch::Tensor& x, const torch::Tensor& w2p,
                        torch::Tensor& y, const ConvShape& sh,
                        const torch::Tensor* bias, bool relu) {
  const long M = sh.M();
  const long KT = w2p.size(1);
  const long N = sh.Kout;
  if (KT > 32 || KT % 8 != 0 || N > 64 || N % 8 != 0 || M < 65536)
    return false;
  const bf16* bs = bias ? (const bf16*)bias->data_ptr() : nullptr;
  const int blocks = (int)std::min<long>((M + 255) / 256, 16384);
  dispatch_thin(KT, [&](auto kt) {
    hipLaunchKernelGGL((gemm_thin_conv_kernel<decltype(kt)::value>),
                       dim3(blocks), dim3(256), 0, cur_stream(),
                       (const bf16*)x.data_ptr(),
                       (const bf16*)w2p.data_ptr(), (bf16*)y.data_ptr(),
                       bs, sh, M, (int)N, relu ? 1 : 0);
  });
  HIP_CHECK(hipGetLastError());
  return true;
}

torch::Tensor transpose_bf16(const torch::Tensor& X) {
  const long R = X.size(0), C = X.size(1);
  auto out = torch::empty({C, R}, X.options());
  dim3 grid((unsigned)ceil_div(C, 64), (unsigned)ceil_div(R, 64));
  hipLaunchKernelGGL(transpose_bf16_kernel, grid, dim3(256), 0, cur_stream(),
                     (const bf16*)X.data_ptr(), (bf16*)out.data_ptr(), R, C);
  HIP_CHECK(hipGetLastError());
  return out;
}

void gemm_bf16_raw(const torch::Tensor& A, const torch::Tensor& B,
                   torch::Tensor& C, long M, long N, long K, bool ta, bool tb,
                   const torch::Tensor* bias, bool relu, EpStore store,
                   long ohw,
                   std::pair<torch::Tensor, torch::Tensor>* bn_stats) {
  TORCH_CHECK(A.scalar_type() == at::kBFloat16 &&
              B.scalar_type() == at::kBFloat16, "gemm: bf16 only");
  CHECK_GPU(A); CHECK_GPU(B); CHECK_CONTIG(A); CHECK_CONTIG(B);
  const bf16* a = (const bf16*)A.data_ptr();
  const bf16* b = (const bf16*)B.data_ptr();
  bf16* c = (bf16*)C.data_ptr();
  const bf16* bs = bias ? (const bf16*)bias->data_ptr() : nullptr;
  const int relu_i = relu ? 1 : 0, sm = (int)store;

  const GemmPlan p =
      plan_dense(M, N, K, ta, tb, store == EpStore::kPlain,
                 bn_stats != nullptr, wgrad_small_gate());
  if (p.path == GemmPath::kThin) {
    dispatch_thin(K, [&](auto kt) {
      hipLaunchKernelGGL((gemm_thin_kernel<decltype(kt)::value>),
                         dim3((unsigned)p.tiles), dim3(256), 0, cur_stream(),
                         a, b, c, bs, M, (int)N, relu_i);
    });
    HIP_CHECK(hipGetLastError());
    return;
  }

  const SplitKPart part = alloc_splitk_part(p, M, N, A);
  const dim3 grid((unsigned)p.tiles, (unsigned)p.S);
  if (p.path == GemmPath::kSmall) {
    const int vecA = ta ? (M % 8 == 0) : (K % 8 == 0);
    const int vecB = tb ? (K % 8 == 0) : (N % 8 == 0);
    dispatch_small(p, [&](auto bm, auto bn, auto wr, auto wc) {
      constexpr int BMv = decltype(bm)::value, BNv = decltype(bn)::value;
      constexpr int WRv = decltype(wr)::value, WCv = decltype(wc)::value;
      dispatch_bool(ta, [&](auto tav) {
        dispatch_bool(tb, [&](auto tbv) {
          hipLaunchKernelGGL(
              (gemm_kernel<BMv, BNv, WRv, WCv, decltype(tav)::value,
                           decltype(tbv)::value>),
              grid, dim3(WRv * WCv * 64), 0, cur_stream(), a, b, c, part.ptr,
              bs, M, N, K, p.kslice, relu_i, sm, ohw, vecA, vecB,
              ConvShape{});
        });
      });
    });
  } else {
    torch::Tensor At, Bt;
    if (ta) { At = transpose_bf16(A); a = (const bf16*)At.data_ptr(); }
    if (!tb) { Bt = transpose_bf16(B); b = (const bf16*)Bt.data_ptr(); }
    const BnStatsPtrs st = alloc_bn_stats(
        bn_stats, p.S == 1 && store == EpStore::kPlain, p, M, N, A);
    if (p.path == GemmPath::kGemm8p)
      hipLaunchKernelGGL(gemm8p_kernel, grid, dim3(512), 0, cur_stream(), a,
                         b, c, part.ptr, bs, M, N, K, p.kslice, relu_i,
                         st.sum, st.sq);
    else
      dispatch_dbuf(p, [&](auto bm, auto bn) {
        hipLaunchKernelGGL(
            (gemm256_kernel<decltype(bm)::value, decltype(bn)::value>), grid,
            dim3(512), 0, cur_stream(), a, b, c, part.ptr, bs, M, N, K,
            p.kslice, relu_i, sm, ohw, ConvShape{}, st.sum, st.sq);
      });
  }
  HIP_CHECK(hipGetLastError());
  if (p.S > 1)
    launch_splitk_reduce(part.ptr, p.S, M, N, c, bs, relu_i, store, ohw);
}

PlanRow gemm_plan_route(long M, long N, long K, bool ta, bool tb) {
  return plan_row(plan_dense(M, N, K, ta, tb, true, false,
                             wgrad_small_gate()));
}

GemmPlan gemm_dense_plan(long M, long N, long K, bool ta, bool tb) {
  return plan_dense(M, N, K, ta, tb, true, false, wgrad_small_gate());
}

void splitk_reduce_plain(const torch::Tensor& part, torch::Tensor& out) {
  launch_splitk_reduce(part.data_ptr<float>(), part.size(0), part.size(1),
                       part.size(2), (bf16*)out.data_ptr(), nullptr, 0,
                       EpStore::kPlain, 0);
}

std::tuple<long, long, long, long> colsum_geom_query(long M, long N) {
  const ColsumGeom g = colsum_geom(M, N);
  return {g.G, g.cblocks, g.rows, g.chunks};
}

torch::Tensor colsum_bf16(const torch::Tensor& X) {
  CHECK_GPU(X); CHECK_CONTIG(X);
  long M = X.size(0), N = X.size(1);
  auto out = torch::empty({N}, X.options());
  const ColsumGeom g = colsum_geom(M, N);
  auto part = torch::empty({g.chunks, N}, X.options().dtype(at::kFloat));
  if (N % 8 == 0) {
    hipLaunchKernelGGL(colsum_part_vec_kernel, dim3(g.cblocks, g.chunks),
                       dim3(256), 0, cur_stream(),
                       (const bf16*)X.data_ptr(), M, N, g.G, g.rows,
                       part.data_ptr<float>());
  } else {
    hipLaunchKernelGGL(colsum_part_kernel, dim3(g.cblocks, g.chunks),
                       dim3(256), 0, cur_stream(),
                       (const bf16*)X.data_ptr(), M, N, g.rows,
                       part.data_ptr<float>());
  }
  HIP_CHECK(hipGetLastError());
  launch_colsum_final(part.data_ptr<float>(), g.chunks, N,
                      (bf16*)out.data_ptr());
  return out;
}

void colsum_finalize(const torch::Tensor& part, torch::Tensor& out) {
  launch_colsum_final(part.data_ptr<float>(), (int)part.size(0),
                      part.size(1), (bf16*)out.data_ptr());
}

std::tuple<torch::Tensor, torch::Tensor> relu_bwd_colsum(
    const torch::Tensor& y, const torch::Tensor& dy) {
  CHECK_GPU(y); CHECK_GPU(dy); CHECK_CONTIG(y); CHECK_CONTIG(dy);
  const long N = dy.size(-1);
  const long M = dy.numel() / N;
  TORCH_CHECK(N % 8 == 0, "relu_bwd_colsum: N % 8 required");
  TORCH_CHECK(y.numel() == dy.numel());
  auto dx = torch::empty_like(dy);
  auto out = torch::empty({N}, dy.options());
  const ColsumGeom g = colsum_geom(M, N);
  auto part = torch::empty({g.chunks, N}, dy.options().dtype(at::kFloat));
  hipLaunchKernelGGL(relu_bwd_colsum_part_vec_kernel,
                     dim3(g.cblocks, g.chunks), dim3(256), 0, cur_stream(),
                     (const bf16*)y.data_ptr(), (const bf16*)dy.data_ptr(),
                     (bf16*)dx.data_ptr(), M, N, g.G, g.rows,
                     part.data_ptr<float>());
  HIP_CHECK(hipGetLastError());
  launch_colsum_final(part.data_ptr<float>(), g.chunks, N,
                      (bf16*)out.data_ptr());
  return {dx, out};
}

GemmPlan gemm_conv_plan(ConvEntry e, const ConvShape& sh) {
  const GemmDims d = conv_gemm_dims(e, sh);
  if (e == ConvEntry::kWgrad)
    return sh.C % 8 == 0 ? plan_small(d.M, d.N, d.K) : GemmPlan{};
  const int inner = e == ConvEntry::kDgrad ? sh.Kout : sh.C;
  if (inner % 8 != 0 || d.M < 48) return {};
  if (e == ConvEntry::kFwdPool &&
      (d.N % 64 != 0 || d.N < 64 || sh.OH % 2 != 0 || sh.OW % 2 != 0))
    return {};
  return plan_conv(d.M, d.N, d.K, narrow_dbuf_gate());
}

namespace {

template <int CMODE>
bool conv_implicit_gemm(const torch::Tensor& x, const torch::Tensor& w2,
                        torch::Tensor& y, const ConvShape& sh,
                        const torch::Tensor* bias, bool relu,
                        std::pair<torch::Tensor, torch::Tensor>* bn_stats
                        = nullptr, bool pool = false,
                        uint8_t* pool_idx = nullptr,
                        HaloMode halo = HaloMode::kAuto,
                        int max_blocks = 0) {
  const ConvEntry e = CMODE == 2 ? ConvEntry::kDgrad
                                 : (pool ? ConvEntry::kFwdPool
                                         : ConvEntry::kFwd);
  const GemmPlan p = gemm_conv_plan(e, sh);
  if (p.path == GemmPath::kNone || (pool && bn_stats)) return false;
  if constexpr (CMODE == 1) {
    if (pool && halo != HaloMode::kOff && halo_conv_gate(sh)) {
      halo_conv_fwd_pool_launch(x, w2, y, sh, bias, relu, pool_idx,
                                max_blocks);
      return true;
    }
  }
  const GemmDims d = conv_gemm_dims(e, sh);
  const long M = d.M, N = d.N, K = d.K;
  const bf16* a = (const bf16*)x.data_ptr();
  const bf16* b = (const bf16*)w2.data_ptr();
  bf16* c = (bf16*)y.data_ptr();
  const bf16* bs = bias ? (const bf16*)bias->data_ptr() : nullptr;
  const int relu_i = relu ? 1 : 0, plain = (int)EpStore::kPlain;
  const SplitKPart part = alloc_splitk_part(p, M, N, x);
  const dim3 grid((unsigned)p.tiles, (unsigned)p.S);
  const BnStatsPtrs st =
      alloc_bn_stats(bn_stats, CMODE == 1 && p.S == 1, p, M, N, x);
  if (p.path == GemmPath::kSmall) {
    dispatch_small(p, [&](auto bm, auto bn, auto wr, auto wc) {
      constexpr int BMv = decltype(bm)::value, BNv = decltype(bn)::value;
      constexpr int WRv = decltype(wr)::value, WCv = decltype(wc)::value;
      hipLaunchKernelGGL(
          (gemm_kernel<BMv, BNv, WRv, WCv, false, true, CMODE>), grid,
          dim3(WRv * WCv * 64), 0, cur_stream(), a, b, c, part.ptr, bs, M,
          N, K, p.kslice, relu_i, plain, 0, 0, 1, sh, st.sum, st.sq);
    });
  } else if (p.bn == 32) {
    auto launchn = [&](auto bm) {
      hipLaunchKernelGGL((gemm256_kernel<decltype(bm)::value, 32, CMODE>),
                         grid, dim3(512), 0, cur_stream(), a, b, c, part.ptr,
                         bs, M, N, K, p.kslice, relu_i, plain, 0, sh,
                         st.sum, st.sq);
    };
    if (p.bm == 128) launchn(ic<128>{});
    else launchn(ic<64>{});
  } else {
    dispatch_dbuf(p, [&](auto bm, auto bn) {
      constexpr int BMv = decltype(bm)::value, BNv = decltype(bn)::value;
      if constexpr (CMODE == 1) {
        if (pool && pool_idx && p.S == 1) {
          hipLaunchKernelGGL((gemm256_kernel<BMv, BNv, 1, 2>), grid,
                             dim3(512), 0, cur_stream(), a, b, c, part.ptr,
                             bs, M, N, K, p.kslice, relu_i, plain, 0, sh,
                             st.sum, st.sq, pool_idx);
          return;
        }
        if (pool) {
          hipLaunchKernelGGL((gemm256_kernel<BMv, BNv, 1, 1>), grid,
                             dim3(512), 0, cur_stream(), a, b, c, part.ptr,
                             bs, M, N, K, p.kslice, relu_i, plain, 0, sh,
                             st.sum, st.sq);
          return;
        }
      }
      hipLaunchKernelGGL((gemm256_kernel<BMv, BNv, CMODE>), grid, dim3(512),
                         0, cur_stream(), a, b, c, part.ptr, bs, M, N, K,
                         p.kslice, relu_i, plain, 0, sh, st.sum, st.sq);
    });
  }
  HIP_CHECK(hipGetLastError());
  if (p.S > 1 && pool)
    launch_splitk_reduce_pool(part.ptr, p.S, M, N, c, bs, relu_i, pool_idx);
  else if (p.S > 1)
    launch_splitk_reduce(part.ptr, p.S, M, N, c, bs, relu_i,
                         EpStore::kPlain, 0);
  return true;
}

}

bool gemm_conv_fwd_raw(const torch::Tensor& x, const torch::Tensor& w2,
                       torch::Tensor& y, const ConvShape& sh,
                       const torch::Tensor* bias, bool relu,
                       std::pair<torch::Tensor, torch::Tensor>* bn_stats) {
  return conv_implicit_gemm<1>(x, w2, y, sh, bias, relu, bn_stats);
}

bool gemm_conv_fwd_pool_eligible(const ConvShape& sh) {
  return gemm_conv_plan(ConvEntry::kFwdPool, sh).path != GemmPath::kNone;
}

bool gemm_conv_fwd_pool_raw(const torch::Tensor& x, const torch::Tensor& w2,
                            torch::Tensor& y, const ConvShape& sh,
                            const torch::Tensor* bias, bool relu,
                            uint8_t* idx, HaloMode halo, int max_blocks) {
  if (halo == HaloMode::kForce) {
    halo_conv_fwd_pool_launch(x, w2, y, sh, bias, relu, idx, max_blocks);
    return true;
  }
  return conv_implicit_gemm<1>(x, w2, y, sh, bias, relu, nullptr, true, idx,
                               halo, max_blocks);
}

bool gemm_conv_dgrad_raw(const torch::Tensor& dy, const torch::Tensor& wrot2,
                         torch::Tensor& dx, const ConvShape& sh) {
  return conv_implicit_gemm<2>(dy, wrot2, dx, sh, nullptr, false);
}

// ... 77 lines not shown
```

csrc/hip/halo_conv.hip:

```cpp
#include "common.h"
#include "gemm_api.h"

#include <cstdlib>

namespace bflc {

namespace {

typedef __attribute__((ext_vector_type(8))) __bf16 bf16x8_t;
typedef __attribute__((ext_vector_type(4))) unsigned int u32x4_t;
typedef __attribute__((ext_vector_type(4))) float f32x4_t;

constexpr int kHaloThreads = 256;
constexpr int kHaloWC = 1;
constexpr int kHaloPF = 8;
constexpr int kHaloMinBlocks = 2;
constexpr long kHaloLdsBudget = 80 * 1024;

struct Magic { unsigned long long m; };
inline Magic make_magic(unsigned d) { return {0xFFFFFFFFull / d + 1}; }
__device__ __forceinline__ unsigned mdiv(unsigned n, Magic g) {
  return (unsigned)(((unsigned long long)n * g.m) >> 32);
}

struct HaloParams {
  int N, H, W, PH, PW;
  int G;
  int pitch;
  int img_lds;
  int hw4;
  int phw;
  Magic m_hw4, m_w, m_phw, m_pw;
};

template <int POOLV>
__launch_bounds__(kHaloThreads, kHaloMinBlocks * (kHaloThreads / 256))
__global__ void halo_conv_pool_kernel(const unsigned char* __restrict__ x,
                                      const bf16* __restrict__ w2,
                                      const bf16* __restrict__ bias,
                                      bf16* __restrict__ y,
                                      uint8_t* __restrict__ pool_idx,
                                      int relu, HaloParams p) {
  extern __shared__ __align__(16) unsigned char smem[];
  constexpr int WR = kHaloThreads / 64 / kHaloWC;
  constexpr int FN = 4 / kHaloWC;
  constexpr int WN = FN * 16;
  constexpr int KOUT = 64, KW = 9 * 32;

  const int tid = threadIdx.x;
  const int lane = tid & 63;
  const int l15 = lane & 15, l4 = lane >> 4;
  const int wave = __builtin_amdgcn_readfirstlane(tid >> 6);
  const int wr = wave / kHaloWC, wc = wave % kHaloWC;

  const int buf_bytes = p.G * p.img_lds;
  const int ngroups = (p.N + p.G - 1) / p.G;

  {
    const u32x4_t z = {0u, 0u, 0u, 0u};
    for (int o = tid * 16; o < 2 * buf_bytes; o += kHaloThreads * 16)
      *reinterpret_cast<u32x4_t*>(smem + o) = z;
  }

  bf16x8_t bfr[9][FN];
#pragma unroll
  for (int t = 0; t < 9; ++t)
#pragma unroll
    for (int fn = 0; fn < FN; ++fn)
      bfr[t][fn] = *reinterpret_cast<const bf16x8_t*>(
          &w2[(long)(wc * WN + fn * 16 + l15) * KW + t * 32 + l4 * 8]);
  float bv[FN];
#pragma unroll
  for (int fn = 0; fn < FN; ++fn)
    bv[fn] = bias ? b2f(bias[wc * WN + fn * 16 + l15]) : 0.f;

  int st_off[kHaloPF];
#pragma unroll
  for (int i = 0; i < kHaloPF; ++i) {
    const unsigned gi = tid + i * kHaloThreads;
    const unsigned img = mdiv(gi, p.m_hw4);
    const unsigned rem = gi - img * p.hw4;
    const unsigned pix = rem >> 2, ch = rem & 3;
    const unsigned py = mdiv(pix, p.m_w), px = pix - py * p.W;
    st_off[i] = (int)(img * p.img_lds + (py + 1) * p.pitch + (px + 1) * 64 +
                      ch * 16);
  }
  u32x4_t pf[kHaloPF];
  auto fetch = [&](int g) __attribute__((always_inline)) {
    const int gc = min(p.G, p.N - g * p.G);
    const int ngr = gc * p.hw4;
    const unsigned char* src = x + (long)g * p.G * p.hw4 * 16;
#pragma unroll
    for (int i = 0; i < kHaloPF; ++i) {
      const int gi = tid + i * kHaloThreads;
      if (gi < ngr)
        pf[i] = *reinterpret_cast<const u32x4_t*>(src + (long)gi * 16);
    }
    return ngr;
  };
  auto stage = [&](int buf, int ngr) __attribute__((always_inline)) {
#pragma unroll
    for (int i = 0; i < kHaloPF; ++i) {
      const int gi = tid + i * kHaloThreads;
      if (gi < ngr)
        *reinterpret_cast<u32x4_t*>(smem + buf * buf_bytes + st_off[i]) =
            pf[i];
    }
  };

  int g = blockIdx.x;
  if (g >= ngroups) return;
  {
    const int ngr = fetch(g);
    __syncthreads();
    stage(0, ngr);
  }
  __syncthreads();

  int cur = 0;
  for (; g < ngroups; g += gridDim.x) {
    const int gnext = g + gridDim.x;
    const bool has_next = gnext < ngroups;
    int ngr_next = 0;
    if (has_next) ngr_next = fetch(gnext);

    const int gc = min(p.G, p.N - g * p.G);
    const int npp = gc * p.phw;
    const int ntiles = (npp + 3) >> 2;
    const long pp0 = (long)g * p.G * p.phw;
    const unsigned char* lbuf = smem + cur * buf_bytes;

    for (int mt = wr; mt < ntiles; mt += WR) {
      const int pp = mt * 4 + (l15 >> 2);
      const int q = l15 & 3;
      const unsigned ppc = pp < npp ? pp : 0;
      const unsigned img = mdiv(ppc, p.m_phw);
      const unsigned rem = ppc - img * p.phw;
      const unsigned ph = mdiv(rem, p.m_pw), pw = rem - ph * p.PW;
      const unsigned char* a0 = lbuf + img * p.img_lds +
                                (2 * ph + (q >> 1)) * p.pitch +
                                (2 * pw + (q & 1)) * 64 + l4 * 16;
      const unsigned char* a1 = a0 + p.pitch;
      const unsigned char* a2 = a1 + p.pitch;

      f32x4_t acc[FN] = {};
#pragma unroll
      for (int t = 0; t < 9; ++t) {
        const int r = t / 3, s = t - r * 3;
        const unsigned char* ar = r == 0 ? a0 : (r == 1 ? a1 : a2);
        const bf16x8_t af =
            *reinterpret_cast<const bf16x8_t*>(ar + s * 64);
#pragma unroll
        for (int fn = 0; fn < FN; ++fn)
          acc[fn] = __builtin_amdgcn_mfma_f32_16x16x32_bf16(
              af, bfr[t][fn], acc[fn], 0, 0, 0);
      }
      {
        const u32x4_t zu = {0u, 0u, 0u, 0u};
        const bf16x8_t z = *reinterpret_cast<const bf16x8_t*>(&zu);
#pragma unroll
        for (int fn = 0; fn < FN; ++fn)
          acc[fn] = __builtin_amdgcn_mfma_f32_16x16x32_bf16(
              z, z, acc[fn], 0, 0, 0);
      }

      const int opp = mt * 4 + l4;
      if (opp < npp) {
#pragma unroll
        for (int fn = 0; fn < FN; ++fn) {
          const int col = wc * WN + fn * 16 + l15;
          float best = -INFINITY;
          int bi = 0;
#pragma unroll
          for (int r = 0; r < 4; ++r) {
            float v = acc[fn][r] + bv[fn];
            if (relu) v = fmaxf(v, 0.f);
            const float f = b2f(f2b(v));
            if (f > best) {
              best = f;
              if (POOLV == 2) bi = r;
            }
          }
          y[(pp0 + opp) * KOUT + col] = f2b(best);
          if (POOLV == 2) pool_idx[(pp0 + opp) * KOUT + col] = (uint8_t)bi;
        }
      }
    }

    if (has_next) stage(cur ^ 1, ngr_next);
    __syncthreads();
    cur ^= 1;
  }
}

bool halo_conv_env_gate() {
  static const bool v = [] {
    const char* e = getenv("BFLC_HALO_CONV");
    return (e ? atoi(e) : 1) != 0;
  }();
  return v;
}

struct HaloGeom {
  bool ok = false;
  int G = 0, pitch = 0, img_lds = 0;
};

HaloGeom halo_geom(const ConvShape& sh) {
  HaloGeom g;
  if (sh.C != 32 || sh.R != 3 || sh.S != 3 || sh.stride != 1 ||
      sh.pad != 1 || sh.Kout != 64 || sh.N <= 0 || sh.OH <= 0 ||
      sh.OW <= 0 || sh.OH % 2 != 0 || sh.OW % 2 != 0)
    return g;
  g.pitch = (sh.W + 2) * 64 + 32;
  const long img = (long)(sh.H + 2) * g.pitch;
  const long by_lds = kHaloLdsBudget / (2 * img);
  const long by_pf =
      (long)kHaloPF * kHaloThreads / ((long)sh.H * sh.W * 4);
  const long G = std::min(by_lds, by_pf);
  if (G < 1) return g;
  g.G = (int)G;
  g.img_lds = (int)img;
  g.ok = true;
  return g;
}

constexpr int kDgPF = 2;
constexpr int kDgWPitch = 72;
constexpr long kDgWBytes = 9L * 32 * kDgWPitch * 2;

struct DgradParams {
  int N, H, W, PW;
  int G;
  int WP;
  int img_pix;
  int hw;
  int pgr;
  Magic m_pgr8, m_pw, m_hw, m_w;
};

typedef __attribute__((ext_vector_type(8))) unsigned short u16x8_t;
typedef __attribute__((ext_vector_type(2))) unsigned int u32x2_t;

__device__ __forceinline__ int dg_lds_off(int pix, int slot) {
  return pix * 128 + ((slot ^ ((pix >> 1) & 7)) << 4);
}

template <bool PLANE>
__launch_bounds__(kHaloThreads, kHaloMinBlocks * (kHaloThreads / 256))
__global__ void halo_pool_dgrad_kernel(const bf16* __restrict__ w,
                                       const unsigned char* __restrict__ yp,
                                       const unsigned char* __restrict__ idx,
                                       const unsigned char* __restrict__ dyp,
                                       unsigned char* __restrict__ dyf,
                                       bf16* __restrict__ dx, DgradParams p) {
  extern __shared__ __align__(16) unsigned char smem[];
  constexpr int WR = kHaloThreads / 64;
  constexpr int FN = 2, C = 32;

  const int tid = threadIdx.x;
  const int lane = tid & 63;
  const int l15 = lane & 15, l4 = lane >> 4;
  const int wave = __builtin_amdgcn_readfirstlane(tid >> 6);

  const int buf_bytes = p.G * p.img_pix * 128;
  const int ngroups = (p.N + p.G - 1) / p.G;
  int g = blockIdx.x;
  if (g >= ngroups) return;

  int st_pix[kDgPF], st_gl[kDgPF];
#pragma unroll
  for (int i = 0; i < kDgPF; ++i) {
    const unsigned gi = tid + i * kHaloThreads;
    const unsigned pp = gi >> 3;
    const unsigned img = mdiv(pp, p.m_pgr8);
    const unsigned rem = pp - img * (p.pgr >> 3);
    const unsigned ph = mdiv(rem, p.m_pw), pw = rem - ph * p.PW;
    st_pix[i] = (int)(img * p.img_pix + (2 * ph + 1) * p.WP + 2 * pw + 1);
    st_gl[i] = (int)((img * p.hw + 2 * ph * p.W + 2 * pw) * 8 + (gi & 7));
  }
  u32x4_t pf_dy[kDgPF], pf_y[kDgPF];
  u32x2_t pf_ix[kDgPF];
  auto fetch = [&](int gg) __attribute__((always_inline)) {
    const int gc = min(p.G, p.N - gg * p.G);
    const int ngr = gc * p.pgr;
    const long base = (long)gg * p.G * p.pgr;
#pragma unroll
    for (int i = 0; i < kDgPF; ++i) {
      const int gi = tid + i * kHaloThreads;
      if (gi < ngr) {
        pf_dy[i] =
            *reinterpret_cast<const u32x4_t*>(dyp + (base + gi) * 16);
        pf_y[i] = *reinterpret_cast<const u32x4_t*>(yp + (base + gi) * 16);
        pf_ix[i] = *reinterpret_cast<const u32x2_t*>(idx + (base + gi) * 8);
      }
    }
    return ngr;
  };
  auto stage = [&](int buf, int gg, int ngr) __attribute__((always_inline)) {
    unsigned char* lbuf = smem + buf * buf_bytes;
    unsigned char* gbase = dyf + (long)gg * p.G * p.hw * 128;
    const bf16 zero = f2b(0.f);
#pragma unroll
    for (int i = 0; i < kDgPF; ++i) {
      const int gi = tid + i * kHaloThreads;
      if (gi < ngr) {
        const bf16x8_t dv = __builtin_bit_cast(bf16x8_t, pf_dy[i]);
        const bf16x8_t yv = __builtin_bit_cast(bf16x8_t, pf_y[i]);
        const unsigned long long iv =
            __builtin_bit_cast(unsigned long long, pf_ix[i]);
        const int slot = gi & 7;
#pragma unroll
        for (int q = 0; q < 4; ++q) {
          bf16x8_t gv;
#pragma unroll
          for (int j = 0; j < 8; ++j) {
            float a = 0.f;
            if ((int)((iv >> (8 * j)) & 0xff) == q) a += b2f(dv[j]);
            gv[j] = f2b(a);
            if (!(b2f(yv[j]) > 0.f)) gv[j] = zero;
          }
          const int pix = st_pix[i] + (q >> 1) * p.WP + (q & 1);
          *reinterpret_cast<bf16x8_t*>(lbuf + dg_lds_off(pix, slot)) = gv;
          if (PLANE) {
            const long go = st_gl[i] + ((q >> 1) * p.W + (q & 1)) * 8;
            *reinterpret_cast<bf16x8_t*>(gbase + go * 16) = gv;
          }
        }
      }
    }
  };

  int ngr0 = fetch(g);

  {
    unsigned short* wt = reinterpret_cast<unsigned short*>(smem);
    const unsigned short* wg = reinterpret_cast<const unsigned short*>(w);
    const int kout = lane;
    u16x8_t wv[9];
#pragma unroll
    for (int i = 0; i < 9; ++i) {
      const int q = wave + i * WR;
      wv[i] = *reinterpret_cast<const u16x8_t*>(&wg[kout * 288 + q * 8]);
    }
#pragma unroll
    for (int i = 0; i < 9; ++i) {
      const int q = wave + i * WR;
#pragma unroll
      for (int j = 0; j < 8; ++j) wt[(q * 8 + j) * kDgWPitch + kout] = wv[i][j];
    }
  }
  __syncthreads();
  bf16x8_t bfr[9][2][FN];
  {
    const unsigned short* wt = reinterpret_cast<const unsigned short*>(smem);
#pragma unroll
    for (int t = 0; t < 9; ++t)
#pragma unroll
      for (int h = 0; h < 2; ++h)
#pragma unroll
        for (int fn = 0; fn < FN; ++fn)
          bfr[t][h][fn] = *reinterpret_cast<const bf16x8_t*>(
              &wt[(t * 32 + fn * 16 + l15) * kDgWPitch + h * 32 + l4 * 8]);
  }
  __syncthreads();

  {
    const u32x4_t z = {0u, 0u, 0u, 0u};
    for (int o = tid * 16; o < 2 * buf_bytes; o += kHaloThreads * 16)
      *reinterpret_cast<u32x4_t*>(smem + o) = z;
  }
  __syncthreads();
  stage(0, g, ngr0);
  __syncthreads();

  int cur = 0;
  for (; g < ngroups; g += gridDim.x) {
    const int gnext = g + gridDim.x;
    const bool has_next = gnext < ngroups;
    int ngr_next = 0;
    if (has_next) ngr_next = fetch(gnext);

    const int gc = min(p.G, p.N - g * p.G);
    const int npix = gc * p.hw;
    const int ntiles = (npix + 15) >> 4;
    const long m0 = (long)g * p.G * p.hw;
    const unsigned char* lbuf = smem + cur * buf_bytes;

    for (int mt = wave; mt < ntiles; mt += WR) {
      const int m = mt * 16 + l15;
      const unsigned mc = m < npix ? m : 0;
      const unsigned img = mdiv(mc, p.m_hw);
      const unsigned rem = mc - img * p.hw;
      const unsigned ih = mdiv(rem, p.m_w), iw = rem - ih * p.W;
      const int pix0 =
          (int)(img * p.img_pix + (ih + 2) * p.WP + iw + 2);

      f32x4_t acc[FN] = {};
#pragma unroll
      for (int t = 0; t < 9; ++t) {
        const int r = t / 3, s = t - r * 3;
        const int off = dg_lds_off(pix0 - r * p.WP - s, l4);
#pragma unroll
        for (int h = 0; h < 2; ++h) {
          const bf16x8_t af =
              *reinterpret_cast<const bf16x8_t*>(lbuf + (off ^ (h << 6)));
#pragma unroll
          for (int fn = 0; fn < FN; ++fn)
            acc[fn] = __builtin_amdgcn_mfma_f32_16x16x32_bf16(
                af, bfr[t][h][fn], acc[fn], 0, 0, 0);
        }
      }

#pragma unroll
      for (int r = 0; r < 4; ++r) {
        const int row = mt * 16 + l4 * 4 + r;
        if (row < npix) {
#pragma unroll
          for (int fn = 0; fn < FN; ++fn)
            dx[(m0 + row) * C + fn * 16 + l15] = f2b(acc[fn][r] + 0.f);
        }
      }
    }

    if (has_next) stage(cur ^ 1, gnext, ngr_next);
    __syncthreads();
    cur ^= 1;
  }
}

bool halo_dgrad_env_gate() {
  static const bool v = [] {
    const char* e = getenv("BFLC_HALO_DGRAD");
    return (e ? atoi(e) : 1) != 0;
  }();
  return v;
}

struct DgradGeom {
  bool ok = false;
  int G = 0;
  long img_lds = 0;
};

DgradGeom dgrad_geom(const ConvShape& sh) {
  DgradGeom g;
  if (sh.C != 32 || sh.R != 3 || sh.S != 3 || sh.stride != 1 ||
      sh.pad != 1 || sh.Kout != 64 || sh.N <= 0 || sh.OH <= 0 ||
      sh.OW <= 0 || sh.OH % 2 != 0 || sh.OW % 2 != 0)
    return g;
  g.img_lds = (long)(sh.OH + 2) * (sh.OW + 2) * 128;
  const long by_lds = kHaloLdsBudget / (2 * g.img_lds);
  const long by_pf =
      (long)kDgPF * kHaloThreads / ((long)(sh.OH / 2) * (sh.OW / 2) * 8);
  const long G = std::min(by_lds, by_pf);
  if (G < 1) return g;
  g.G = (int)G;
  g.ok = true;
  return g;
}

}

bool halo_dgrad_geometry_ok(const ConvShape& sh) { return dgrad_geom(sh).ok; }

int halo_dgrad_group_images(const ConvShape& sh) { return dgrad_geom(sh).G; }

bool halo_dgrad_gate(const ConvShape& sh) {
  if (!halo_dgrad_env_gate() || !dgrad_geom(sh).ok) return false;
  if (sh.M() * sh.Kout >= (1L << 31)) return false;
  const GemmPlan p = gemm_conv_plan(ConvEntry::kDgrad, sh);
  return p.path != GemmPath::kNone && p.S == 1;
}

void halo_pool_dgrad_launch(const torch::Tensor& w,
                            const torch::Tensor& y_pooled,
                            const torch::Tensor& idx,
                            const torch::Tensor& dy_pooled,
                            torch::Tensor* dyf, torch::Tensor& dx,
                            const ConvShape& sh, int max_blocks) {
  const DgradGeom g = dgrad_geom(sh);
  TORCH_CHECK(g.ok, "halo dgrad: shape outside the kernel's geometry");
  TORCH_CHECK((long)sh.N * sh.OH * sh.OW < (1L << 31), "halo dgrad: N");
  DgradParams p;
  p.N = sh.N; p.H = sh.OH; p.W = sh.OW; p.PW = sh.OW / 2;
  p.G = g.G;
  p.WP = sh.OW + 2;
  p.img_pix = (sh.OH + 2) * (sh.OW + 2);
  p.hw = sh.OH * sh.OW;
  p.pgr = (sh.OH / 2) * (sh.OW / 2) * 8;
  p.m_pgr8 = make_magic((unsigned)(p.pgr / 8));
  p.m_pw = make_magic((unsigned)p.PW);
  p.m_hw = make_magic((unsigned)p.hw);
  p.m_w = make_magic((unsigned)p.W);
  const size_t lds =
      (size_t)std::max<long>(2L * g.G * g.img_lds, kDgWBytes);
  const int groups = (sh.N + g.G - 1) / g.G;
  int blocks = std::min(groups, kHaloMinBlocks * kNumCU);
  if (max_blocks > 0) blocks = std::min(blocks, max_blocks);
  static const bool attr_set = [] {
    HIP_CHECK(hipFuncSetAttribute(
        (const void*)halo_pool_dgrad_kernel<true>,
        hipFuncAttributeMaxDynamicSharedMemorySize, (int)kHaloLdsBudget));
    HIP_CHECK(hipFuncSetAttribute(
        (const void*)halo_pool_dgrad_kernel<false>,
        hipFuncAttributeMaxDynamicSharedMemorySize, (int)kHaloLdsBudget));
    return true;
  }();
  (void)attr_set;
  auto* kern = dyf ? halo_pool_dgrad_kernel<true>
                   : halo_pool_dgrad_kernel<false>;
  hipLaunchKernelGGL(kern, dim3((unsigned)blocks),
                     dim3(kHaloThreads), lds, cur_stream(),
                     (const bf16*)w.data_ptr(),
                     (const unsigned char*)y_pooled.data_ptr(),
                     (const unsigned char*)idx.data_ptr(),
                     (const unsigned char*)dy_pooled.data_ptr(),
                     dyf ? (unsigned char*)dyf->data_ptr() : nullptr,
                     (bf16*)dx.data_ptr(), p);
  HIP_CHECK(hipGetLastError());
}

bool halo_conv_geometry_ok(const ConvShape& sh) { return halo_geom(sh).ok; }

int halo_conv_group_images(const ConvShape& sh) { return halo_geom(sh).G; }

bool halo_conv_gate(const ConvShape& sh) {
  if (!halo_conv_env_gate() || !halo_geom(sh).ok) return false;
  const GemmPlan p = gemm_conv_plan(ConvEntry::kFwdPool, sh);
  return p.path == GemmPath::kGemm256 && p.S == 1;
}

void halo_conv_fwd_pool_launch(const torch::Tensor& x,
                               const torch::Tensor& w2, torch::Tensor& y,
                               const ConvShape& sh, const torch::Tensor* bias,
                               bool relu, uint8_t* idx, int max_blocks) {
  const HaloGeom g = halo_geom(sh);
  TORCH_CHECK(g.ok, "halo conv: shape outside the kernel's geometry");
  TORCH_CHECK((long)sh.N * sh.H * sh.W * 64 < (1L << 40), "halo conv: N");
  HaloParams p;
  p.N = sh.N; p.H = sh.H; p.W = sh.W;
  p.PH = sh.OH / 2; p.PW = sh.OW / 2;
  p.G = g.G; p.pitch = g.pitch; p.img_lds = g.img_lds;
  p.hw4 = sh.H * sh.W * 4;
  p.phw = p.PH * p.PW;
  p.m_hw4 = make_magic((unsigned)p.hw4);
  p.m_w = make_magic((unsigned)p.W);
  p.m_phw = make_magic((unsigned)p.phw);
  p.m_pw = make_magic((unsigned)p.PW);
  const size_t lds = (size_t)2 * g.G * g.img_lds;
  const int groups = (sh.N + g.G - 1) / g.G;
  int blocks = std::min(groups, kHaloMinBlocks * kNumCU);
  if (max_blocks > 0) blocks = std::min(blocks, max_blocks);
  auto* kern = idx ? halo_conv_pool_kernel<2> : halo_conv_pool_kernel<1>;
  static const bool attr_set = [] {
    HIP_CHECK(hipFuncSetAttribute(
        (const void*)halo_conv_pool_kernel<1>,
        hipFuncAttributeMaxDynamicSharedMemorySize, (int)kHaloLdsBudget));
    HIP_CHECK(hipFuncSetAttribute(
        (const void*)halo_conv_pool_kernel<2>,
        hipFuncAttributeMaxDynamicSharedMemorySize, (int)kHaloLdsBudget));
    return true;
  }();
  (void)attr_set;
  hipLaunchKernelGGL(kern, dim3((unsigned)blocks), dim3(kHaloThreads), lds,
                     cur_stream(), (const unsigned char*)x.data_ptr(),
                     (const bf16*)w2.data_ptr(),
                     bias ? (const bf16*)bias->data_ptr() : nullptr,
                     (bf16*)y.data_ptr(), idx, relu ? 1 : 0, p);
  HIP_CHECK(hipGetLastError());
}

}
```

Baseline: 5.065 ms/round.

## Fuse both conv-ReLU-pool layers of FemnistCNN into one halo stack kernel

```diff
diff --git a/bflc_amd/models/__init__.py b/bflc_amd/models/__init__.py
--- a/bflc_amd/models/__init__.py
+++ b/bflc_amd/models/__init__.py
@@ -45,8 +45,8 @@
                 ("f2w", (128, c.n_class), "xavier"), ("f2b", (c.n_class,), "zeros")]
 
     def forward(self, x):
-        h = O.conv2d_relu_pool(x, self.p("c1w"), self.p("c1b"), 1, 1)
-        h = O.conv2d_relu_pool(h, self.p("c2w"), self.p("c2b"), 1, 1)
+        h = O.conv_relu_pool_stack(x, self.p("c1w"), self.p("c1b"),
+                                   self.p("c2w"), self.p("c2b"))
         h = h.reshape(h.shape[0], -1)
         h = O.linear(h, self.p("f1w"), self.p("f1b"), relu=True)
         return O.linear(h, self.p("f2w"), self.p("f2b"))
diff --git a/bflc_amd/ops/__init__.py b/bflc_amd/ops/__init__.py
--- a/bflc_amd/ops/__init__.py
+++ b/bflc_amd/ops/__init__.py
@@ -2,6 +2,7 @@
 from bflc_amd.ops.functional import (accuracy, accuracy_t, adam_step_,
                                      axpy_, batchnorm2d, conv2d, conv2d_bn,
                                      conv2d_relu_pool,
+                                     conv_relu_pool_stack,
                                      global_avgpool, add_relu,
                                      hip_available, hip_ops, linear,
                                      maxpool2d, relu, sgd_step_,
@@ -10,7 +11,7 @@
 
 __all__ = [
     "functional", "linear", "conv2d", "conv2d_bn", "conv2d_relu_pool",
-    "batchnorm2d", "relu",
+    "conv_relu_pool_stack", "batchnorm2d", "relu",
     "add_relu", "maxpool2d", "global_avgpool", "softmax_cross_entropy",
     "accuracy", "accuracy_t", "axpy_", "sgd_step_", "adam_step_",
     "sgdm_step_", "grad_clip_coef_",
diff --git a/bflc_amd/ops/functional.py b/bflc_amd/ops/functional.py
--- a/bflc_amd/ops/functional.py
+++ b/bflc_amd/ops/functional.py
@@ -285,6 +285,18 @@
             x, w, b, stride, padding,
             os.environ.get("BFLC_THIN_DIRECT_WGRAD", "0") == "1")
     return maxpool2d(conv2d(x, w, b, stride, padding, relu=True), 2)
+
+
+def conv_relu_pool_stack(x, w1, b1, w2, b2) -> torch.Tensor:
+    import os
+    if x.is_cuda and not torch.is_grad_enabled() and \
+            os.environ.get("BFLC_FUSED_POOL", "1") == "1" and \
+            b1 is not None and b2 is not None and \
+            hip_ops().conv_relu_pool_stack_route(
+                list(x.shape), list(w1.shape), list(w2.shape)) == "halo_stack":
+        return hip_ops().conv_relu_pool_stack_fwd(x, w1, b1, w2, b2, 0, "")
+    h = conv2d_relu_pool(x, w1, b1, 1, 1)
+    return conv2d_relu_pool(h, w2, b2, 1, 1)
 
 
 class _BatchNormFn(torch.autograd.Function):
diff --git a/csrc/hip/bindings.cpp b/csrc/hip/bindings.cpp
--- a/csrc/hip/bindings.cpp
+++ b/csrc/hip/bindings.cpp
@@ -88,6 +88,16 @@
 std::string conv_fwd_pool_impl(std::vector<long> x_shape,
                                std::vector<long> w_shape, long stride,
                                long pad);
+torch::Tensor conv_relu_pool_stack_fwd(torch::Tensor x, torch::Tensor w1,
+                                       torch::Tensor b1, torch::Tensor w2,
+                                       torch::Tensor b2, long max_blocks,
+                                       std::string impl);
+std::string conv_relu_pool_stack_route(std::vector<long> x_shape,
+                                       std::vector<long> w1_shape,
+                                       std::vector<long> w2_shape);
+long halo_stack_group_images_query(std::vector<long> x_shape,
+                                   std::vector<long> w1_shape,
+                                   std::vector<long> w2_shape);
 long halo_conv_group_images_query(std::vector<long> x_shape,
                                   std::vector<long> w_shape, long stride,
                                   long pad);
@@ -264,6 +274,19 @@
         "images per LDS group of the halo kernel (0: not its geometry)",
         py::arg("x_shape"), py::arg("w_shape"), py::arg("stride"),
         py::arg("pad"));
+  m.def("conv_relu_pool_stack_fwd", &bflc::conv_relu_pool_stack_fwd,
+        "grad-free conv3x3 + ReLU + pool twice (stride 1, pad 1): "
+        "[N, H/4, W/4, Kout2]. impl pins two_call | halo_stack (geometry "
+        "only; '' = conv_relu_pool_stack_route's answer); max_blocks > 0 "
+        "caps the halo kernels' grids",
+        py::arg("x"), py::arg("w1"), py::arg("b1"), py::arg("w2"),
+        py::arg("b2"), py::arg("max_blocks") = 0, py::arg("impl") = "");
+  m.def("conv_relu_pool_stack_route", &bflc::conv_relu_pool_stack_route,
+        "what conv_relu_pool_stack_fwd runs: halo_stack | two_call",
+        py::arg("x_shape"), py::arg("w1_shape"), py::arg("w2_shape"));
+  m.def("halo_stack_group_images", &bflc::halo_stack_group_images_query,
+        "images per LDS group of the stack kernel (0: not its geometry)",
+        py::arg("x_shape"), py::arg("w1_shape"), py::arg("w2_shape"));
   m.def("conv2d_relu_pool_route", &bflc::conv2d_relu_pool_route,
         "route conv2d_relu_pool_fwd takes: gemm256_pool | thin_pool | "
         "unfused",
diff --git a/csrc/hip/conv2d.hip b/csrc/hip/conv2d.hip
--- a/csrc/hip/conv2d.hip
+++ b/csrc/hip/conv2d.hip
@@ -980,9 +980,7 @@
 PoolRoute pool_route(const ConvShape& sh) {
   if (is_1x1_s1(sh)) return PoolRoute::kUnfused;
   if (gemm_conv_fwd_pool_eligible(sh)) return PoolRoute::kGemm256;
-  const long kp = (sh.RSC() + 7) / 8 * 8;
-  if (sh.RSC() <= 16 && gemm_thin_conv_pool_eligible(sh, kp))
-    return PoolRoute::kThin;
+  if (gemm_thin_conv_pool_eligible(sh)) return PoolRoute::kThin;
   return PoolRoute::kUnfused;
 }
 
@@ -1053,9 +1051,7 @@
         route == PoolRoute::kGemm256
             ? gemm_conv_fwd_pool_raw(x, w2, y, sh, &bc, true, ip, halo,
                                      (int)max_blocks)
-            : gemm_thin_conv_pool_raw(
-                  x, pad_w2(w2, (sh.RSC() + 7) / 8 * 8), y, sh, &bc, true,
-                  ip);
+            : gemm_thin_conv_pool_raw(x, w2, y, sh, &bc, true, ip);
     TORCH_CHECK(done, "conv2d_relu_pool: route query and launcher disagree");
     return {y, idx};
   }
@@ -1168,6 +1164,80 @@
                                   long pad) {
   return halo_conv_group_images(
       make_shape_dims(x_shape, w_shape, stride, pad));
+}
+
+namespace {
+
+struct StackShapes { ConvShape sh1, sh2; };
+
+StackShapes stack_shapes(const std::vector<long>& xs,
+                         const std::vector<long>& w1s,
+                         const std::vector<long>& w2s) {
+  StackShapes s;
+  s.sh1 = make_shape_dims(xs, w1s, 1, 1);
+  s.sh2 = make_shape_dims({xs[0], s.sh1.OH / 2, s.sh1.OW / 2, w1s[0]}, w2s,
+                          1, 1);
+  return s;
+}
+
+bool stack_gate(const StackShapes& s) {
+  return pool_route(s.sh1) == PoolRoute::kThin &&
+         pool_route(s.sh2) == PoolRoute::kGemm256 &&
+         halo_stack_gate(s.sh1, s.sh2);
+}
+
+}
+
+std::string conv_relu_pool_stack_route(std::vector<long> x_shape,
+                                       std::vector<long> w1_shape,
+                                       std::vector<long> w2_shape) {
+  TORCH_CHECK(w2_shape.size() == 4 && w1_shape.size() == 4 &&
+              w2_shape[3] == w1_shape[0],
+              "conv stack: w2's channels are w1's outputs");
+  return stack_gate(stack_shapes(x_shape, w1_shape, w2_shape))
+             ? "halo_stack"
+             : "two_call";
+}
+
+long halo_stack_group_images_query(std::vector<long> x_shape,
+                                   std::vector<long> w1_shape,
+                                   std::vector<long> w2_shape) {
+  const StackShapes s = stack_shapes(x_shape, w1_shape, w2_shape);
+  return halo_stack_group_images(s.sh1, s.sh2);
+}
+
+torch::Tensor conv_relu_pool_stack_fwd(torch::Tensor x, torch::Tensor w1,
+                                       torch::Tensor b1, torch::Tensor w2,
+                                       torch::Tensor b2, long max_blocks,
+                                       std::string impl) {
+  CHECK_GPU(x); CHECK_CONTIG(x); CHECK_CONTIG(w1); CHECK_CONTIG(w2);
+  TORCH_CHECK(x.scalar_type() == at::kBFloat16 &&
+              w1.scalar_type() == at::kBFloat16 &&
+              w2.scalar_type() == at::kBFloat16 &&
+              b1.scalar_type() == at::kBFloat16 &&
+              b2.scalar_type() == at::kBFloat16, "conv: bf16 only");
+  TORCH_CHECK(impl.empty() || impl == "two_call" || impl == "halo_stack",
+              "conv_relu_pool_stack: impl is '' | two_call | halo_stack");
+  TORCH_CHECK(x.dim() == 4 && w1.dim() == 4 && w2.dim() == 4 &&
+              w2.size(3) == w1.size(0),
+              "conv stack: NHWC x, KRSC weights, w2's channels w1's outputs");
+  const StackShapes s = stack_shapes(x.sizes().vec(), w1.sizes().vec(),
+                                     w2.sizes().vec());
+  const bool pinned = impl == "halo_stack";
+  TORCH_CHECK(!pinned || halo_stack_geometry_ok(s.sh1, s.sh2),
+              "conv_relu_pool_stack: shape outside the stack kernel's "
+              "geometry");
+  if (pinned || (impl.empty() && stack_gate(s))) {
+    auto b1c = b1.contiguous(), b2c = b2.contiguous();
+    auto y = torch::empty({(long)s.sh2.N, (long)s.sh2.OH / 2,
+                           (long)s.sh2.OW / 2, (long)s.sh2.Kout},
+                          x.options());
+    halo_stack_launch(x, w1, b1c, w2, b2c, y, s.sh1, s.sh2, (int)max_blocks);
+    return y;
+  }
+  auto h = std::get<0>(relu_pool_fwd_impl(x, w1, b1, 1, 1, false));
+  return std::get<0>(
+      relu_pool_fwd_impl(h, w2, b2, 1, 1, false, max_blocks, ""));
 }
 
 std::tuple<torch::Tensor, torch::Tensor> conv2d_relu_pool_fwd_idx(
diff --git a/csrc/hip/gemm_api.h b/csrc/hip/gemm_api.h
--- a/csrc/hip/gemm_api.h
+++ b/csrc/hip/gemm_api.h
@@ -70,6 +70,14 @@
                                const torch::Tensor& w2, torch::Tensor& y,
                                const ConvShape& sh, const torch::Tensor* bias,
                                bool relu, uint8_t* idx, int max_blocks);
+bool halo_stack_geometry_ok(const ConvShape& sh1, const ConvShape& sh2);
+int halo_stack_group_images(const ConvShape& sh1, const ConvShape& sh2);
+bool halo_stack_gate(const ConvShape& sh1, const ConvShape& sh2);
+void halo_stack_launch(const torch::Tensor& x, const torch::Tensor& w1,
+                       const torch::Tensor& b1, const torch::Tensor& w2,
+                       const torch::Tensor& b2, torch::Tensor& y,
+                       const ConvShape& sh1, const ConvShape& sh2,
+                       int max_blocks);
 bool halo_dgrad_geometry_ok(const ConvShape& sh);
 int halo_dgrad_group_images(const ConvShape& sh);
 bool halo_dgrad_gate(const ConvShape& sh);
@@ -79,9 +87,9 @@
                             const torch::Tensor& dy_pooled,
                             torch::Tensor* dyf, torch::Tensor& dx,
                             const ConvShape& sh, int max_blocks);
-bool gemm_thin_conv_pool_eligible(const ConvShape& sh, long KT);
+bool gemm_thin_conv_pool_eligible(const ConvShape& sh);
 bool gemm_thin_conv_pool_raw(const torch::Tensor& x,
-                             const torch::Tensor& w2p, torch::Tensor& y,
+                             const torch::Tensor& w2, torch::Tensor& y,
                              const ConvShape& sh, const torch::Tensor* bias,
                              bool relu, uint8_t* idx = nullptr);
 
diff --git a/csrc/hip/gemm_bf16.hip b/csrc/hip/gemm_bf16.hip
--- a/csrc/hip/gemm_bf16.hip
+++ b/csrc/hip/gemm_bf16.hip
@@ -1,6 +1,7 @@
 
 #include "common.h"
 #include "gemm_api.h"
+#include "thin_pool_chain.h"
 
 namespace bflc {
 
@@ -1450,15 +1451,15 @@
   }
 }
 
-template <int KT, bool IDX>
+template <bool IDX>
 __global__ __launch_bounds__(256) void gemm_thin_conv_pool_kernel(
     const bf16* __restrict__ X, const bf16* __restrict__ B,
     bf16* __restrict__ C, uint8_t* __restrict__ idx,
     const bf16* __restrict__ bias, ConvShape sh, long MP, int N, int relu) {
-  __shared__ float Bl[32 * 64];
-  __shared__ float bl[64];
-  for (int i = threadIdx.x; i < N * KT; i += blockDim.x)
-    Bl[(i % KT) * 64 + i / KT] = b2f(B[i]);
+  __shared__ __align__(32) float Bl[9 * 64];
+  __shared__ __align__(32) float bl[64];
+  for (int i = threadIdx.x; i < N * 9; i += blockDim.x)
+    Bl[(i % 9) * 64 + i / 9] = b2f(B[i]);
   for (int i = threadIdx.x; i < N; i += blockDim.x)
     bl[i] = bias ? b2f(bias[i]) : 0.f;
   __syncthreads();
@@ -1470,7 +1471,7 @@
     const int rem = (int)(mp % PHW);
     const int ih0 = (rem / PW) * 2 - sh.pad;
     const int iw0 = (rem % PW) * 2 - sh.pad;
-    f32x2v_t pd[4][4];
+    thin::f32x2 pd[4][4];
 #pragma unroll
     for (int r = 0; r < 4; ++r) {
       const int ih = ih0 + r;
@@ -1481,56 +1482,15 @@
         const bool ok = okh && iw >= 0 && iw < sh.W;
         const float f =
             ok ? b2f(X[((long)n * sh.H + ih) * sh.W + iw]) : 0.f;
-        pd[r][s] = f32x2v_t{f, f};
-      }
-    }
-    const f32x2v_t zero2 = {0.f, 0.f};
+        pd[r][s] = thin::f32x2{f, f};
+      }
+    }
     for (int n8 = 0; n8 < N; n8 += 8) {
-      f32x8v_t acc[4];
-#pragma unroll
-      for (int q = 0; q < 4; ++q)
-        acc[q] = *reinterpret_cast<const f32x8v_t*>(&bl[n8]);
-#pragma unroll
-      for (int k = 0; k < KT; ++k) {
-        const f32x8v_t bv =
-            *reinterpret_cast<const f32x8v_t*>(&Bl[k * 64 + n8]);
-        const f32x2v_t* bv2 = reinterpret_cast<const f32x2v_t*>(&bv);
-#pragma unroll
-        for (int q = 0; q < 4; ++q) {
-          const f32x2v_t a =
-              k < 9 ? pd[(q >> 1) + k / 3][(q & 1) + k % 3] : zero2;
-          f32x2v_t* acc2 = reinterpret_cast<f32x2v_t*>(&acc[q]);
-#pragma unroll
-          for (int p = 0; p < 4; ++p) acc2[p] += bv2[p] * a;
-        }
-      }
-      float best[8];
-      int bi[8];
-#pragma unroll
-      for (int j = 0; j < 8; ++j) { best[j] = -INFINITY; bi[j] = 0; }
-#pragma unroll
-      for (int q = 0; q < 4; ++q) {
-#pragma unroll
-        for (int j = 0; j < 8; ++j) {
-          float v = acc[q][j];
-          if (relu && v < 0.f) v = 0.f;
-          const float f = b2f(f2b(v));
-          if (f > best[j]) {
-            best[j] = f;
-            if (IDX) bi[j] = q;
-          }
-        }
-      }
-      bf16x8_t out;
-#pragma unroll
-      for (int j = 0; j < 8; ++j) out[j] = f2b(best[j]);
-      *reinterpret_cast<bf16x8_t*>(&C[mp * N + n8]) = out;
-      if (IDX) {
-        u8x8_t oidx;
-#pragma unroll
-        for (int j = 0; j < 8; ++j) oidx[j] = (uint8_t)bi[j];
-        *reinterpret_cast<u8x8_t*>(&idx[mp * N + n8]) = oidx;
-      }
+      thin::bf16x8 out;
+      thin::u8x8 oidx;
+      thin::conv_pool_chain<IDX>(pd, &Bl[n8], 64, &bl[n8], relu, out, oidx);
+      *reinterpret_cast<thin::bf16x8*>(&C[mp * N + n8]) = out;
+      if (IDX) *reinterpret_cast<thin::u8x8*>(&idx[mp * N + n8]) = oidx;
     }
   }
 }
@@ -1664,26 +1624,25 @@
 
 }
 
-bool gemm_thin_conv_pool_eligible(const ConvShape& sh, long KT) {
-  return sh.R == 3 && sh.S == 3 && sh.C == 1 && sh.stride == 1 &&
-         sh.OH % 2 == 0 && sh.OW % 2 == 0 && KT == 16 &&
+bool gemm_thin_conv_pool_eligible(const ConvShape& sh) {
+  return sh.R == 3 && sh.S == 3 && sh.C == 1 && sh.RSC() == 9 &&
+         sh.stride == 1 && sh.OH % 2 == 0 && sh.OW % 2 == 0 &&
          sh.Kout <= 64 && sh.Kout % 8 == 0 && sh.M() >= 65536;
 }
 
 bool gemm_thin_conv_pool_raw(const torch::Tensor& x,
-                             const torch::Tensor& w2p, torch::Tensor& y,
+                             const torch::Tensor& w2, torch::Tensor& y,
                              const ConvShape& sh, const torch::Tensor* bias,
                              bool relu, uint8_t* idx) {
-  const long KT = w2p.size(1);
-  if (!gemm_thin_conv_pool_eligible(sh, KT)) return false;
+  if (!gemm_thin_conv_pool_eligible(sh) || w2.size(1) != 9) return false;
   const long MP = sh.M() / 4;
   const bf16* bs = bias ? (const bf16*)bias->data_ptr() : nullptr;
   const int blocks = (int)std::min<long>((MP + 255) / 256, 16384);
   dispatch_bool(idx != nullptr, [&](auto want_idx) {
     hipLaunchKernelGGL(
-        (gemm_thin_conv_pool_kernel<16, decltype(want_idx)::value>),
+        (gemm_thin_conv_pool_kernel<decltype(want_idx)::value>),
         dim3(blocks), dim3(256), 0, cur_stream(), (const bf16*)x.data_ptr(),
-        (const bf16*)w2p.data_ptr(), (bf16*)y.data_ptr(), idx, bs, sh, MP,
+        (const bf16*)w2.data_ptr(), (bf16*)y.data_ptr(), idx, bs, sh, MP,
         (int)sh.Kout, relu ? 1 : 0);
   });
   HIP_CHECK(hipGetLastError());
diff --git a/csrc/hip/halo_conv.hip b/csrc/hip/halo_conv.hip
--- a/csrc/hip/halo_conv.hip
+++ b/csrc/hip/halo_conv.hip
@@ -1,5 +1,6 @@
 #include "common.h"
 #include "gemm_api.h"
+#include "thin_pool_chain.h"
 
 #include <cstdlib>
 
@@ -9,6 +10,7 @@
 
 typedef __attribute__((ext_vector_type(8))) __bf16 bf16x8_t;
 typedef __attribute__((ext_vector_type(4))) unsigned int u32x4_t;
+typedef __attribute__((ext_vector_type(2))) unsigned int u32x2_t;
 typedef __attribute__((ext_vector_type(4))) float f32x4_t;
 
 constexpr int kHaloThreads = 256;
@@ -33,14 +35,26 @@
   Magic m_hw4, m_w, m_phw, m_pw;
 };
 
-template <int POOLV>
-__launch_bounds__(kHaloThreads, kHaloMinBlocks * (kHaloThreads / 256))
-__global__ void halo_conv_pool_kernel(const unsigned char* __restrict__ x,
-                                      const bf16* __restrict__ w2,
-                                      const bf16* __restrict__ bias,
-                                      bf16* __restrict__ y,
-                                      uint8_t* __restrict__ pool_idx,
-                                      int relu, HaloParams p) {
+struct StackParams {
+  const bf16* w1;
+  const bf16* b1;
+  int W1;
+  int rpitch;
+  int rimg;
+  int rgr;
+  int raw_off;
+  int w_off;
+  Magic m_w1;
+};
+constexpr int kStackKout1 = 32;
+constexpr int kStackWBytes = (9 + 1) * kStackKout1 * 4;
+
+template <int POOLV, bool STACK>
+__device__ __forceinline__ void halo_conv_pool_body(
+    const unsigned char* __restrict__ x, const bf16* __restrict__ w2,
+    const bf16* __restrict__ bias, bf16* __restrict__ y,
+    uint8_t* __restrict__ pool_idx, int relu, const HaloParams& p,
+    const StackParams& sp) {
   extern __shared__ __align__(16) unsigned char smem[];
   constexpr int WR = kHaloThreads / 64 / kHaloWC;
   constexpr int FN = 4 / kHaloWC;
@@ -58,8 +72,15 @@
 
   {
     const u32x4_t z = {0u, 0u, 0u, 0u};
-    for (int o = tid * 16; o < 2 * buf_bytes; o += kHaloThreads * 16)
+    const int zbytes = STACK ? sp.w_off : 2 * buf_bytes;
+    for (int o = tid * 16; o < zbytes; o += kHaloThreads * 16)
       *reinterpret_cast<u32x4_t*>(smem + o) = z;
+  }
+  float* w1l = reinterpret_cast<float*>(smem + (STACK ? sp.w_off : 0));
+  if constexpr (STACK) {
+    for (int i = tid; i < kStackKout1 * 9; i += kHaloThreads)
+      w1l[(i % 9) * kStackKout1 + i / 9] = b2f(sp.w1[i]);
+    if (tid < kStackKout1) w1l[9 * kStackKout1 + tid] = b2f(sp.b1[tid]);
   }
 
   bf16x8_t bfr[9][FN];
@@ -86,17 +107,81 @@
                       ch * 16);
   }
   u32x4_t pf[kHaloPF];
+  int rst[2] = {0, 0};
+  if constexpr (STACK) {
+#pragma unroll
+    for (int h = 0; h < 2; ++h) {
+      const unsigned e = tid * 8 + h * 4;
+      const unsigned img = mdiv(e, p.m_hw4);
+      const unsigned rem = e - img * p.hw4;
+      const unsigned iy = mdiv(rem, sp.m_w1), ix = rem - iy * sp.W1;
+      rst[h] = (int)(sp.raw_off + img * sp.rimg +
+                     ((iy + 1) * sp.rpitch + ix + 4) * 2);
+    }
+  }
+  u32x4_t rpf;
   auto fetch = [&](int g) __attribute__((always_inline)) {
     const int gc = min(p.G, p.N - g * p.G);
-    const int ngr = gc * p.hw4;
-    const unsigned char* src = x + (long)g * p.G * p.hw4 * 16;
-#pragma unroll
-    for (int i = 0; i < kHaloPF; ++i) {
-      const int gi = tid + i * kHaloThreads;
-      if (gi < ngr)
-        pf[i] = *reinterpret_cast<const u32x4_t*>(src + (long)gi * 16);
-    }
-    return ngr;
+    if constexpr (STACK) {
+      const int ngr = gc * sp.rgr;
+      const unsigned char* src = x + (long)g * p.G * sp.rgr * 16;
+      if (tid < ngr)
+        rpf = *reinterpret_cast<const u32x4_t*>(src + (long)tid * 16);
+      return ngr;
+    } else {
+      const int ngr = gc * p.hw4;
+      const unsigned char* src = x + (long)g * p.G * p.hw4 * 16;
+#pragma unroll
+      for (int i = 0; i < kHaloPF; ++i) {
+        const int gi = tid + i * kHaloThreads;
+        if (gi < ngr)
+          pf[i] = *reinterpret_cast<const u32x4_t*>(src + (long)gi * 16);
+      }
+      return ngr;
+    }
+  };
+  auto raw_put = [&](int ngr) __attribute__((always_inline)) {
+    if (tid < ngr) {
+      *reinterpret_cast<u32x2_t*>(smem + rst[0]) = u32x2_t{rpf.x, rpf.y};
+      *reinterpret_cast<u32x2_t*>(smem + rst[1]) = u32x2_t{rpf.z, rpf.w};
+    }
+  };
+  auto conv1_item = [&](int buf, int npix, int item)
+      __attribute__((always_inline)) {
+    if (item < 4 * npix) {
+      const int hw = p.hw4 >> 2;
+      const int oct =
+          (item >= npix) + (item >= 2 * npix) + (item >= 3 * npix);
+      const unsigned pix = item - oct * npix;
+      const unsigned img = mdiv(pix * 4, p.m_hw4);
+      const unsigned rem = pix - img * hw;
+      const unsigned py = mdiv(rem, p.m_w), px = rem - py * p.W;
+      const unsigned char* rp = smem + sp.raw_off + img * sp.rimg +
+                                ((2 * py) * sp.rpitch + 2 * px + 2) * 2;
+      thin::f32x2 pd[4][4];
+#pragma unroll
+      for (int r = 0; r < 4; ++r) {
+        const unsigned* rw =
+            reinterpret_cast<const unsigned*>(rp + r * sp.rpitch * 2);
+        const unsigned a = rw[0], b = rw[1], c = rw[2];
+        const float f0 = __uint_as_float(a & 0xffff0000u);
+        const float f1 = __uint_as_float(b << 16);
+        const float f2 = __uint_as_float(b & 0xffff0000u);
+        const float f3 = __uint_as_float(c << 16);
+        pd[r][0] = thin::f32x2{f0, f0};
+        pd[r][1] = thin::f32x2{f1, f1};
+        pd[r][2] = thin::f32x2{f2, f2};
+        pd[r][3] = thin::f32x2{f3, f3};
+      }
+      thin::bf16x8 out;
+      thin::u8x8 oidx;
+      thin::conv_pool_chain<false>(pd, w1l + oct * 8, kStackKout1,
+                                   w1l + 9 * kStackKout1 + oct * 8, 1, out,
+                                   oidx);
+      *reinterpret_cast<thin::bf16x8*>(
+          smem + buf * buf_bytes + img * p.img_lds + (py + 1) * p.pitch +
+          (px + 1) * 64 + oct * 16) = out;
+    }
   };
   auto stage = [&](int buf, int ngr) __attribute__((always_inline)) {
 #pragma unroll
@@ -110,10 +195,20 @@
 
   int g = blockIdx.x;
   if (g >= ngroups) return;
+  int ngr_ahead = 0;
   {
     const int ngr = fetch(g);
     __syncthreads();
-    stage(0, ngr);
+    if constexpr (STACK) {
+      raw_put(ngr);
+      __syncthreads();
+      const int npix = ngr * 2;
+      for (int item = tid; item < 4 * npix; item += kHaloThreads)
+        conv1_item(0, npix, item);
+      if (g + (int)gridDim.x < ngroups) ngr_ahead = fetch(g + gridDim.x);
+    } else {
+      stage(0, ngr);
+    }
   }
   __syncthreads();
 
@@ -122,7 +217,16 @@
     const int gnext = g + gridDim.x;
     const bool has_next = gnext < ngroups;
     int ngr_next = 0;
-    if (has_next) ngr_next = fetch(gnext);
+    if constexpr (STACK) {
+      ngr_next = ngr_ahead;
+      raw_put(ngr_next);
+      __syncthreads();
+      ngr_ahead = 0;
+      if (gnext + (int)gridDim.x < ngroups)
+        ngr_ahead = fetch(gnext + gridDim.x);
+    } else {
+      if (has_next) ngr_next = fetch(gnext);
+    }
 
     const int gc = min(p.G, p.N - g * p.G);
     const int npp = gc * p.phw;
@@ -130,7 +234,15 @@
     const long pp0 = (long)g * p.G * p.phw;
     const unsigned char* lbuf = smem + cur * buf_bytes;
 
-    for (int mt = wr; mt < ntiles; mt += WR) {
+    const int npix_next = ngr_next * 2;
+    const int npass = STACK ? (4 * npix_next + 63) >> 6 : 0;
+    const int nloop = STACK ? max(ntiles, npass) : ntiles;
+
+    for (int mt = wr; mt < nloop; mt += WR) {
+      if constexpr (STACK) {
+        if (mt < npass) conv1_item(cur ^ 1, npix_next, mt * 64 + lane);
+        if (mt >= ntiles) continue;
+      }
       const int pp = mt * 4 + (l15 >> 2);
       const int q = l15 & 3;
       const unsigned ppc = pp < npp ? pp : 0;
@@ -187,10 +299,33 @@
       }
     }
 
-    if (has_next) stage(cur ^ 1, ngr_next);
+    if constexpr (!STACK) {
+      if (has_next) stage(cur ^ 1, ngr_next);
+    }
     __syncthreads();
     cur ^= 1;
   }
+}
+
+template <int POOLV>
+__launch_bounds__(kHaloThreads, kHaloMinBlocks * (kHaloThreads / 256))
+__global__ void halo_conv_pool_kernel(const unsigned char* __restrict__ x,
+                                      const bf16* __restrict__ w2,
+                                      const bf16* __restrict__ bias,
+                                      bf16* __restrict__ y,
+                                      uint8_t* __restrict__ pool_idx,
+                                      int relu, HaloParams p) {
+  halo_conv_pool_body<POOLV, false>(x, w2, bias, y, pool_idx, relu, p,
+                                    StackParams{});
+}
+
+__launch_bounds__(kHaloThreads, kHaloMinBlocks * (kHaloThreads / 256))
+__global__ void halo_conv_stack_kernel(const unsigned char* __restrict__ x,
+                                       const bf16* __restrict__ w2,
+                                       const bf16* __restrict__ bias,
+                                       bf16* __restrict__ y, HaloParams p,
+                                       StackParams sp) {
+  halo_conv_pool_body<1, true>(x, w2, bias, y, nullptr, 1, p, sp);
 }
 
 bool halo_conv_env_gate() {
@@ -225,6 +360,48 @@
   return g;
 }
 
+bool halo_stack_env_gate() {
+  static const bool v = [] {
+    const char* e = getenv("BFLC_HALO_STACK");
+    return (e ? atoi(e) : 1) != 0;
+  }();
+  return v;
+}
+
+struct StackGeom {
+  bool ok = false;
+  int G = 0, pitch = 0, img_lds = 0;
+  int rpitch = 0, rimg = 0, raw_off = 0, w_off = 0;
+  long lds = 0;
+};
+
+StackGeom stack_geom(const ConvShape& sh1, const ConvShape& sh2) {
+  StackGeom s;
+  if (sh1.C != 1 || sh1.R != 3 || sh1.S != 3 || sh1.stride != 1 ||
+      sh1.pad != 1 || sh1.Kout != kStackKout1 || sh1.N <= 0 ||
+      sh1.H <= 0 || sh1.W <= 0 || sh1.H % 4 != 0 || sh1.W % 4 != 0 ||
+      sh2.N != sh1.N || sh2.H != sh1.H / 2 || sh2.W != sh1.W / 2)
+    return s;
+  const HaloGeom h = halo_geom(sh2);
+  if (!h.ok) return s;
+  s.pitch = h.pitch;
+  s.img_lds = h.img_lds;
+  s.rpitch = sh1.W + 8;
+  s.rimg = (sh1.H + 2) * s.rpitch * 2;
+  for (int G = h.G; G >= 1; --G) {
+    const long raw_off = 2L * G * h.img_lds;
+    const long w_off = (raw_off + (long)G * s.rimg + 63) / 64 * 64;
+    if (w_off + kStackWBytes > kHaloLdsBudget) continue;
+    s.G = G;
+    s.raw_off = (int)raw_off;
+    s.w_off = (int)w_off;
+    s.lds = w_off + kStackWBytes;
+    s.ok = (long)G * sh1.H * sh1.W / 8 <= kHaloThreads;
+    break;
+  }
+  return s;
+}
+
 constexpr int kDgPF = 2;
 constexpr int kDgWPitch = 72;
 constexpr long kDgWBytes = 9L * 32 * kDgWPitch * 2;
@@ -240,7 +417,6 @@
 };
 
 typedef __attribute__((ext_vector_type(8))) unsigned short u16x8_t;
-typedef __attribute__((ext_vector_type(2))) unsigned int u32x2_t;
 
 __device__ __forceinline__ int dg_lds_off(int pix, int slot) {
   return pix * 128 + ((slot ^ ((pix >> 1) & 7)) << 4);
@@ -571,4 +747,66 @@
   HIP_CHECK(hipGetLastError());
 }
 
-}
+bool halo_stack_geometry_ok(const ConvShape& sh1, const ConvShape& sh2) {
+  return stack_geom(sh1, sh2).ok;
+}
+
+int halo_stack_group_images(const ConvShape& sh1, const ConvShape& sh2) {
+  return stack_geom(sh1, sh2).G;
+}
+
+bool halo_stack_gate(const ConvShape& sh1, const ConvShape& sh2) {
+  return halo_stack_env_gate() && stack_geom(sh1, sh2).ok &&
+         halo_conv_gate(sh2);
+}
+
+void halo_stack_launch(const torch::Tensor& x, const torch::Tensor& w1,
+                       const torch::Tensor& b1, const torch::Tensor& w2,
+                       const torch::Tensor& b2, torch::Tensor& y,
+                       const ConvShape& sh1, const ConvShape& sh2,
+                       int max_blocks) {
+  const StackGeom g = stack_geom(sh1, sh2);
+  TORCH_CHECK(g.ok, "halo stack: shape outside the kernel's geometry");
+  TORCH_CHECK((long)sh2.N * sh2.H * sh2.W * 64 < (1L << 40), "halo stack: N");
+  TORCH_CHECK(w1.numel() == kStackKout1 * 9 && b1.numel() == kStackKout1 &&
+              w2.numel() == 64 * 9 * 32 && b2.numel() == 64,
+              "halo stack: parameter sizes");
+  HaloParams p;
+  p.N = sh2.N; p.H = sh2.H; p.W = sh2.W;
+  p.PH = sh2.OH / 2; p.PW = sh2.OW / 2;
+  p.G = g.G; p.pitch = g.pitch; p.img_lds = g.img_lds;
+  p.hw4 = sh2.H * sh2.W * 4;
+  p.phw = p.PH * p.PW;
+  p.m_hw4 = make_magic((unsigned)p.hw4);
+  p.m_w = make_magic((unsigned)p.W);
+  p.m_phw = make_magic((unsigned)p.phw);
+  p.m_pw = make_magic((unsigned)p.PW);
+  StackParams sp;
+  sp.w1 = (const bf16*)w1.data_ptr();
+  sp.b1 = (const bf16*)b1.data_ptr();
+  sp.W1 = sh1.W;
+  sp.rpitch = g.rpitch;
+  sp.rimg = g.rimg;
+  sp.rgr = sh1.H * sh1.W / 8;
+  sp.raw_off = g.raw_off;
+  sp.w_off = g.w_off;
+  sp.m_w1 = make_magic((unsigned)sh1.W);
+  const int groups = (sh2.N + g.G - 1) / g.G;
+  int blocks = std::min(groups, kHaloMinBlocks * kNumCU);
+  if (max_blocks > 0) blocks = std::min(blocks, max_blocks);
+  static const bool attr_set = [] {
+    HIP_CHECK(hipFuncSetAttribute(
+        (const void*)halo_conv_stack_kernel,
+        hipFuncAttributeMaxDynamicSharedMemorySize, (int)kHaloLdsBudget));
+    return true;
+  }();
+  (void)attr_set;
+  hipLaunchKernelGGL(halo_conv_stack_kernel, dim3((unsigned)blocks),
+                     dim3(kHaloThreads), (size_t)g.lds, cur_stream(),
+                     (const unsigned char*)x.data_ptr(),
+                     (const bf16*)w2.data_ptr(), (const bf16*)b2.data_ptr(),
+                     (bf16*)y.data_ptr(), p, sp);
+  HIP_CHECK(hipGetLastError());
+}
+
+}
diff --git a/csrc/hip/thin_pool_chain.h b/csrc/hip/thin_pool_chain.h
--- /dev/null
+++ b/csrc/hip/thin_pool_chain.h
@@ -0,0 +1,71 @@
+#pragma once
+
+#include "common.h"
+
+namespace bflc {
+namespace thin {
+
+typedef __attribute__((ext_vector_type(8))) float f32x8;
+typedef __attribute__((ext_vector_type(2))) float f32x2;
+typedef __attribute__((ext_vector_type(8))) __bf16 bf16x8;
+typedef uint8_t u8x8 __attribute__((ext_vector_type(8)));
+
+template <bool IDX>
+__device__ __forceinline__ void conv_pool_chain(const f32x2 (&pd)[4][4],
+                                                const float* wl, int wstride,
+                                                const float* bl, int relu,
+                                                bf16x8& out, u8x8& oidx) {
+  f32x8 acc[4];
+#pragma unroll
+  for (int q = 0; q < 4; ++q) acc[q] = *reinterpret_cast<const f32x8*>(bl);
+#pragma unroll
+  for (int k = 0; k < 9; ++k) {
+    const f32x8 bv = *reinterpret_cast<const f32x8*>(&wl[k * wstride]);
+    const f32x2* bv2 = reinterpret_cast<const f32x2*>(&bv);
+#pragma unroll
+    for (int q = 0; q < 4; ++q) {
+      const f32x2 a = pd[(q >> 1) + k / 3][(q & 1) + k % 3];
+      f32x2* acc2 = reinterpret_cast<f32x2*>(&acc[q]);
+#pragma unroll
+      for (int p = 0; p < 4; ++p) acc2[p] += bv2[p] * a;
+    }
+  }
+#pragma unroll
+  for (int q = 0; q < 4; ++q) acc[q] = acc[q] + 0.f;
+  if constexpr (!IDX) {
+#pragma unroll
+    for (int j = 0; j < 8; ++j) {
+      float m = fmaxf(fmaxf(acc[0][j], acc[1][j]),
+                      fmaxf(acc[2][j], acc[3][j]));
+      if (relu && m < 0.f) m = 0.f;
+      out[j] = f2b(fmaxf(m, -INFINITY));
+    }
+    return;
+  }
+  float best[8];
+  int bi[8];
+#pragma unroll
+  for (int j = 0; j < 8; ++j) { best[j] = -INFINITY; bi[j] = 0; }
+#pragma unroll
+  for (int q = 0; q < 4; ++q) {
+#pragma unroll
+    for (int j = 0; j < 8; ++j) {
+      float v = acc[q][j];
+      if (relu && v < 0.f) v = 0.f;
+      const float f = b2f(f2b(v));
+      if (f > best[j]) {
+        best[j] = f;
+        if (IDX) bi[j] = q;
+      }
+    }
+  }
+#pragma unroll
+  for (int j = 0; j < 8; ++j) out[j] = f2b(best[j]);
+  if (IDX) {
+#pragma unroll
+    for (int j = 0; j < 8; ++j) oidx[j] = (uint8_t)bi[j];
+  }
+}
+
+}
+}
```

New measurement: 4.717 ms/round, median of 6. -6.9%, faster.
